# killerwhile/kafka-assignment-optimizer

Measured on AMD Instinct MI355X. Metric: candidate assignments/sec (+ time_to_optimal_s), 10k-partition reassign, higher is better.
Workload: dtype int32

## Files before the change

### include/kao.h

```cpp
#ifndef KAO_H
#define KAO_H

#include <stdint.h>

#ifdef __cplusplus
extern "C" {
#endif

#define KAO_VERSION 103
#define KAO_NONE 0xFFFFu
#define KAO_MAX_RF 8
#define KAO_MAX_RACKS 255

enum {
    KAO_OK = 0,
    KAO_ERR_INVALID = -1,
    KAO_ERR_UNSUPPORTED = -2,
    KAO_ERR_NO_DEVICE = -3,
    KAO_ERR_HIP = -4,
    KAO_ERR_NOMEM = -5,
    KAO_ERR_NOT_INIT = -6
};

enum {
    KAO_STATUS_OPTIMAL_PROVEN = 0,
    KAO_STATUS_FEASIBLE_BOUND_GAP = 1,
    KAO_STATUS_NO_FEASIBLE = 2,
    KAO_STATUS_TIME_LIMIT = 3,
    KAO_STATUS_INFEASIBLE_PROVEN = 4
};

typedef struct kao_topic {
    int32_t n_brokers;
    int32_t n_racks;
    int32_t n_partitions;
    int32_t rf;
    int32_t rf_cur;
    const uint8_t *rack_of;
    const uint16_t *current;
    int32_t w[2][2];
    int32_t rep_lo, rep_hi;
    int32_t lead_lo, lead_hi;
    int32_t rack_lo, rack_hi;
    int32_t prack_lo, prack_hi;
    const int32_t *broker_w;
    const int32_t *broker_wl;
} kao_topic;

typedef struct kao_opts {
    uint64_t seed;
    double time_limit_s;
    int32_t restarts;
    int32_t iters_per_launch;
    int32_t max_launches;
    int32_t obj_scale;
    int32_t lam_min, lam_max;
    int32_t period_log2;
    int32_t stop_at_bound;
    int32_t profile;
    int32_t dual_iters;
    int32_t elite_period;
    int32_t use_prices;
    int32_t use_cycles;
    int32_t islands;
    int32_t schedule;
    int32_t team;
    const int64_t *target_objective;
} kao_opts;

typedef struct kao_result {
    int32_t status;
    int32_t best_restart;
    int64_t objective;
    int64_t upper_bound;
    int32_t violations[8];
    double seconds_to_best;
    uint16_t *assignment;
} kao_result;

typedef struct kao_stats {
    uint64_t launches;
    uint64_t delta_candidates;
    uint64_t full_candidates;
    double ms_search;
    double ms_eval;
    uint64_t search_bytes_algo;
    uint64_t eval_bytes_algo;
    int32_t n_restarts_total;
    int32_t lds_bytes_search;
    int32_t blocks_search;
    int32_t drift;
    int32_t launch_groups;
    int32_t search_rf3_launches;
} kao_stats;

typedef struct kao_session kao_session;
typedef struct kao_eval_plan kao_eval_plan;

int kao_init(int device);
void kao_shutdown(void);
int kao_version(void);
const char *kao_strerror(int code);
const char *kao_last_error(void);
int kao_device_name(char *buf, int len);

int kao_derive_bounds(const kao_topic *t, int32_t out[8]);
int kao_upper_bound(const kao_topic *t, int64_t *ub);
int kao_check_infeasible(const kao_topic *t, char *why, int why_len);
int kao_canonicalize(const kao_topic *t, uint16_t *assignment);

int kao_evaluate(const kao_topic *t, const uint16_t *assignment, int64_t *objective, int32_t violations[8]);
int kao_evaluate_batch(const kao_topic *t, const uint16_t *candidates, int64_t n, int32_t *objective,
                       int32_t *violations);
int kao_eval_plan_create(const kao_topic *t, kao_eval_plan **out);
int kao_eval_plan_run(kao_eval_plan *p, const void *d_candidates, int64_t n, void *d_objective ,
                      void *d_violations , void *d_best_key );
int kao_eval_plan_sync(kao_eval_plan *p, double *ms_last );
void kao_eval_plan_destroy(kao_eval_plan *p);

int kao_session_create(const kao_topic *topics, int32_t n_topics, const kao_opts *opts, kao_session **out);
int kao_session_step(kao_session *s);
int kao_session_sync(kao_session *s);
int kao_session_new_generation(kao_session *s);
int kao_session_best(kao_session *s, kao_result *results);
int kao_session_best_keys(kao_session *s, uint64_t *keys);
int kao_session_device_keys(kao_session *s, void **d_keys);
int kao_session_stats(kao_session *s, kao_stats *out);
int kao_session_small_launches(kao_session *s, int64_t *out);
int kao_session_bound_step(kao_session *s, const int64_t *target, int32_t iters);
int kao_session_set_prices(kao_session *s, int32_t topic, const int32_t *a, const int32_t *l, const int32_t *g);
int kao_session_adopt_prices(kao_session *s);
int kao_session_prices(kao_session *s, int32_t topic, int32_t *a, int32_t *l, int32_t *g);
int kao_session_bound_busy(kao_session *s);
int kao_session_bounds(kao_session *s, int64_t *upper_bound, int32_t *flags, int32_t *iters);
int kao_session_dual_state(kao_session *s, int32_t topic, int32_t *a, int32_t *l, int32_t *g, int64_t *best_dual);
int kao_session_set_dual_state(kao_session *s, int32_t topic, const int32_t *a, const int32_t *l, const int32_t *g);
int kao_lp_bound(const kao_topic *t, double tol, int32_t max_iters, int64_t *bound, int64_t *best_dual, int32_t *multipliers, double stats[8]);
int kao_lp_trace(const kao_topic *t, double tol, int32_t max_iters, double *trace, double stats[8], int32_t *multipliers);
int kao_lp_round(const kao_topic *t, double pert, uint32_t salt, double tol, int32_t max_iters, int32_t use_fallback, uint16_t *assignment,
                 int64_t *objective, int32_t violations[8], double stats[8]);
int kao_lp_round_host(const kao_topic *t, const uint8_t *q, const int32_t *zq, int32_t use_fallback, uint16_t *assignment, int32_t rep[4]);
int kao_dense_spd_test(const double *A, int32_t n, const double *rhs, double *factor, double *linv, double *x, double ms[2]);
int kao_search_band_row(int32_t lo, int32_t hi, int32_t c, int32_t force_plain, int32_t *fits);
int kao_search_rack_delta(int32_t lo, int32_t hi, int32_t c, int32_t dec);
int kao_lp_sharded_test(const kao_topic *t, const int32_t *devices, int32_t n_dev, double pert, uint32_t salt, double tol, int32_t max_iters,
                        int64_t *bound, uint16_t *assignment, int64_t *objective, int32_t violations[8], double stats[8]);
int kao_dual_bound(const kao_topic *t, int64_t target, int32_t iters, int32_t launches, int64_t *bound,
                   int64_t *best_dual, int32_t *iters_done, int32_t *flags, int32_t *multipliers);
int kao_session_restart_state(kao_session *s, int32_t topic, int32_t restart, uint16_t *final_state,
                              uint16_t *best_state, int32_t info[4]);
void kao_session_destroy(kao_session *s);

int kao_solve(const kao_topic *topics, int32_t n_topics, const kao_opts *opts, kao_result *results);
int kao_solve_multi(const kao_topic *topics, int32_t n_topics, const int32_t *devices, int32_t n_dev, const kao_opts *opts,
                    kao_result *results);
int kao_solve_capped(const kao_topic *topics, int32_t n_topics, const int32_t *replica_cap, const int32_t *devices, int32_t n_dev,
                     const kao_opts *opts, int32_t max_rounds, kao_result *results, int64_t *lagrangian_bound);
int kao_improve_cycles(const kao_topic *t, uint16_t *assignment, int32_t max_rounds, int64_t *objective, int32_t stats[8]);
int kao_cycle_matrices(const kao_topic *t, const uint16_t *assignment, int32_t layer, int32_t level, int32_t *dist, int32_t *mid,
                       uint32_t *slot);
int kao_cycle_square_plan(int32_t n, int32_t out[3]);
int kao_cycle_seeds(const kao_topic *t, const uint16_t *assignment, int32_t *table, int32_t *n_cfg);
int kao_cycle_pair_edges(const kao_topic *t, const uint16_t *assignment, int32_t gmin, int32_t *cost, int64_t stats[4]);

int kao_plan_waves(int32_t n_brokers, int32_t n_partitions, int32_t width, const uint16_t *current, const uint16_t *target,
                   int32_t max_per_broker, uint64_t seed, int32_t *wave , int32_t *n_waves, int32_t *lower_bound);

int kao_plan_waves_sized(int32_t n_brokers, int32_t n_partitions, int32_t width, const uint16_t *current, const uint16_t *target,
                         const uint64_t *size , uint64_t max_bytes_per_broker, int32_t max_per_broker,
                         uint64_t seed, int32_t *wave , int32_t *n_waves, int32_t *lower_bound);

int kao_balance_leaders(const kao_topic *t, uint16_t *assignment , int32_t *n_changed,
                        int64_t *objective ,
                        int32_t *status, int32_t stats[8] );

#define KAO_FAILOVER_MAX_BROKERS 8000
int kao_failover_order(int32_t n_brokers, int32_t n_racks, const uint8_t *rack_of ,
                       int32_t n_partitions, int32_t width, uint16_t *rows ,
                       int32_t scope , int32_t dry_run,
                       int32_t *scen , int32_t *n_reordered, int32_t stats[8] );

int kao_balance_leaders_cluster(int32_t n_brokers, int32_t n_partitions, int32_t width,
                                uint16_t *rows ,
                                const int32_t *topic_of , int32_t n_topics,
                                const int32_t *topic_lo, const int32_t *topic_hi ,
                                int32_t cluster_lo, int32_t cluster_hi , int32_t dry_run,
                                int32_t *n_changed, int32_t *peak_before, int32_t *peak_after, int32_t *status,
                                int32_t stats[8] );

int kao_balance_leaders_weighted(int32_t n_brokers, int32_t n_partitions, int32_t width,
                                 uint16_t *rows , const uint64_t *weight ,
                                 uint64_t min_gain, int32_t max_rounds , int32_t dry_run,
                                 int32_t *n_changed, uint64_t *peak_before, uint64_t *peak_after, uint64_t *lower_bound,
                                 int32_t *status, int64_t stats[8] );
int kao_wleaders_test_path(int32_t path);

int kao_failover_order_weighted(int32_t n_brokers, int32_t n_racks, const uint8_t *rack_of, int32_t n_partitions, int32_t width,
                                uint16_t *rows , const uint64_t *weight ,
                                int32_t scope, uint64_t min_gain, int32_t max_rounds , int32_t dry_run,
                                uint64_t *scen , int32_t *n_reordered, int32_t *status,
                                int64_t stats[8] );

#define KAO_DISK_MAX_BROKERS 8000
int kao_balance_disk(int32_t n_brokers, int32_t n_racks, const uint8_t *rack_of, int32_t n_partitions, int32_t width,
                     uint16_t *rows , const uint64_t *size ,
                     int32_t max_per_rack , int32_t move_leaders, uint64_t min_gain,
                     int32_t max_rounds , int32_t dry_run, int32_t *n_moved, uint64_t *bytes_moved,
                     uint64_t *peak_before, uint64_t *peak_after, uint64_t *lower_bound, int32_t *status,
                     int64_t stats[8] );

int kao_balance_disk_budget(int32_t n_brokers, int32_t n_racks, const uint8_t *rack_of, int32_t n_partitions, int32_t width,
                            uint16_t *rows , const uint64_t *size ,
                            int32_t max_per_rack , int32_t move_leaders, uint64_t min_gain,
                            uint64_t max_bytes , int32_t max_rounds , int32_t dry_run,
                            int32_t *n_moved, uint64_t *bytes_moved, uint64_t *peak_before, uint64_t *peak_after,
                            uint64_t *lower_bound, int32_t *status, int64_t stats[10] );

#define KAO_LOGDIRS_MAX_DIRS 64
int kao_balance_logdirs(int32_t n_brokers, const int32_t *dir_start , const uint64_t *base ,
                        int32_t n_replicas, int32_t *dir , const uint64_t *size ,
                        uint64_t min_gain, int32_t max_rounds , int32_t dry_run,
                        int32_t *n_moved, uint64_t *bytes_moved, uint64_t *peak_before, uint64_t *peak_after,
                        uint64_t *per_broker , int32_t *status, int64_t stats[8] );

int kao_rccl_selftest(const int32_t *devices, int32_t n_dev);
int kao_rccl_loopback_counts(uint64_t out[2]);
int kao_last_solve_timing(double out[16]);
int kao_last_solve_lp(double out[8]);
int kao_last_solve_profile(double out[8]);

#ifdef __cplusplus
}
#endif
#endif
```

### kafka_assignment_optimizer_amd/__init__.py

```python
from .model import DEFAULT_WEIGHTS, NONE, Topic, assignment_to_json, topics_from_json
from .solver import (EvalPlan, KaoError, Result, Session, canonicalize, check_infeasible, derive_bounds, device_name, dual_bound, evaluate,
                     cycle_matrices, cycle_pair_edges, cycle_seeds, cycle_square_plan, dense_spd_test, evaluate_batch, improve_cycles, init, last_solve_lp, last_solve_profile, last_solve_timing, library_path, lp_bound, lp_repair_host, lp_round, lp_round_host, lp_sharded, lp_trace, rccl_loopback_counts, rccl_selftest, solve, solve_capped, solve_multi, upper_bound)

__version__ = "0.1.0"
```

### kafka_assignment_optimizer_amd/_ffi.py

```python
from __future__ import annotations

import ctypes as C
import os

_HERE = os.path.dirname(os.path.abspath(__file__))
LIB_PATH = os.path.join(_HERE, "libkao.so")


class KaoTopic(C.Structure):
    _fields_ = [("n_brokers", C.c_int32), ("n_racks", C.c_int32), ("n_partitions", C.c_int32),
                ("rf", C.c_int32), ("rf_cur", C.c_int32),
                ("rack_of", C.POINTER(C.c_uint8)), ("current", C.POINTER(C.c_uint16)),
                ("w", (C.c_int32 * 2) * 2),
                ("rep_lo", C.c_int32), ("rep_hi", C.c_int32), ("lead_lo", C.c_int32), ("lead_hi", C.c_int32),
                ("rack_lo", C.c_int32), ("rack_hi", C.c_int32), ("prack_lo", C.c_int32), ("prack_hi", C.c_int32),
                ("broker_w", C.POINTER(C.c_int32)), ("broker_wl", C.POINTER(C.c_int32))]


class KaoOpts(C.Structure):
    _fields_ = [("seed", C.c_uint64), ("time_limit_s", C.c_double), ("restarts", C.c_int32),
                ("iters_per_launch", C.c_int32), ("max_launches", C.c_int32), ("obj_scale", C.c_int32),
                ("lam_min", C.c_int32), ("lam_max", C.c_int32), ("period_log2", C.c_int32),
                ("stop_at_bound", C.c_int32), ("profile", C.c_int32), ("dual_iters", C.c_int32),
                ("elite_period", C.c_int32), ("use_prices", C.c_int32), ("use_cycles", C.c_int32), ("islands", C.c_int32),
                ("schedule", C.c_int32), ("team", C.c_int32),
                ("target_objective", C.POINTER(C.c_int64))]


class KaoResult(C.Structure):
    _fields_ = [("status", C.c_int32), ("best_restart", C.c_int32), ("objective", C.c_int64),
                ("upper_bound", C.c_int64), ("violations", C.c_int32 * 8), ("seconds_to_best", C.c_double),
                ("assignment", C.POINTER(C.c_uint16))]


class KaoStats(C.Structure):
    _fields_ = [("launches", C.c_uint64), ("delta_candidates", C.c_uint64), ("full_candidates", C.c_uint64),
                ("ms_search", C.c_double), ("ms_eval", C.c_double), ("search_bytes_algo", C.c_uint64),
                ("eval_bytes_algo", C.c_uint64), ("n_restarts_total", C.c_int32), ("lds_bytes_search", C.c_int32),
                ("blocks_search", C.c_int32), ("drift", C.c_int32), ("launch_groups", C.c_int32),
                ("search_rf3_launches", C.c_int32)]


_P = C.POINTER
SIGNATURES = {
    "kao_init": (C.c_int, [C.c_int]),
    "kao_shutdown": (None, []),
    "kao_version": (C.c_int, []),
    "kao_strerror": (C.c_char_p, [C.c_int]),
    "kao_last_error": (C.c_char_p, []),
    "kao_device_name": (C.c_int, [C.c_char_p, C.c_int]),
    "kao_derive_bounds": (C.c_int, [_P(KaoTopic), _P(C.c_int32)]),
    "kao_upper_bound": (C.c_int, [_P(KaoTopic), _P(C.c_int64)]),
    "kao_canonicalize": (C.c_int, [_P(KaoTopic), _P(C.c_uint16)]),
    "kao_check_infeasible": (C.c_int, [_P(KaoTopic), C.c_char_p, C.c_int]),
    "kao_evaluate": (C.c_int, [_P(KaoTopic), _P(C.c_uint16), _P(C.c_int64), _P(C.c_int32)]),
    "kao_evaluate_batch": (C.c_int, [_P(KaoTopic), _P(C.c_uint16), C.c_int64, _P(C.c_int32), _P(C.c_int32)]),
    "kao_eval_plan_create": (C.c_int, [_P(KaoTopic), _P(C.c_void_p)]),
    "kao_eval_plan_run": (C.c_int, [C.c_void_p, C.c_void_p, C.c_int64, C.c_void_p, C.c_void_p, C.c_void_p]),
    "kao_eval_plan_sync": (C.c_int, [C.c_void_p, _P(C.c_double)]),
    "kao_eval_plan_destroy": (None, [C.c_void_p]),
    "kao_session_create": (C.c_int, [_P(KaoTopic), C.c_int32, _P(KaoOpts), _P(C.c_void_p)]),
    "kao_session_step": (C.c_int, [C.c_void_p]),
    "kao_session_sync": (C.c_int, [C.c_void_p]),
    "kao_session_new_generation": (C.c_int, [C.c_void_p]),
    "kao_session_best": (C.c_int, [C.c_void_p, _P(KaoResult)]),
    "kao_session_best_keys": (C.c_int, [C.c_void_p, _P(C.c_uint64)]),
    "kao_session_device_keys": (C.c_int, [C.c_void_p, _P(C.c_void_p)]),
    "kao_session_stats": (C.c_int, [C.c_void_p, _P(KaoStats)]),
    "kao_session_small_launches": (C.c_int, [C.c_void_p, _P(C.c_int64)]),
    "kao_session_restart_state": (C.c_int, [C.c_void_p, C.c_int32, C.c_int32, _P(C.c_uint16), _P(C.c_uint16),
                                            _P(C.c_int32)]),
    "kao_session_bound_step": (C.c_int, [C.c_void_p, _P(C.c_int64), C.c_int32]),
    "kao_session_set_prices": (C.c_int, [C.c_void_p, C.c_int32, _P(C.c_int32), _P(C.c_int32), _P(C.c_int32)]),
    "kao_session_adopt_prices": (C.c_int, [C.c_void_p]),
    "kao_session_prices": (C.c_int, [C.c_void_p, C.c_int32, _P(C.c_int32), _P(C.c_int32), _P(C.c_int32)]),
    "kao_session_bound_busy": (C.c_int, [C.c_void_p]),
    "kao_session_bounds": (C.c_int, [C.c_void_p, _P(C.c_int64), _P(C.c_int32), _P(C.c_int32)]),
    "kao_session_dual_state": (C.c_int, [C.c_void_p, C.c_int32, _P(C.c_int32), _P(C.c_int32), _P(C.c_int32), _P(C.c_int64)]),
    "kao_session_set_dual_state": (C.c_int, [C.c_void_p, C.c_int32, _P(C.c_int32), _P(C.c_int32), _P(C.c_int32)]),
    "kao_lp_bound": (C.c_int, [_P(KaoTopic), C.c_double, C.c_int32, _P(C.c_int64), _P(C.c_int64), _P(C.c_int32), _P(C.c_double)]),
    "kao_lp_round": (C.c_int, [_P(KaoTopic), C.c_double, C.c_uint32, C.c_double, C.c_int32, C.c_int32, _P(C.c_uint16), _P(C.c_int64), _P(C.c_int32), _P(C.c_double)]),
    "kao_lp_round_host": (C.c_int, [_P(KaoTopic), _P(C.c_uint8), _P(C.c_int32), C.c_int32, _P(C.c_uint16), _P(C.c_int32)]),
    "kao_dense_spd_test": (C.c_int, [_P(C.c_double), C.c_int32, _P(C.c_double), _P(C.c_double), _P(C.c_double), _P(C.c_double), _P(C.c_double)]),
    "kao_search_band_row": (C.c_int, [C.c_int32, C.c_int32, C.c_int32, C.c_int32, _P(C.c_int32)]),
    "kao_search_rack_delta": (C.c_int, [C.c_int32, C.c_int32, C.c_int32, C.c_int32]),
    "kao_lp_sharded_test": (C.c_int, [_P(KaoTopic), _P(C.c_int32), C.c_int32, C.c_double, C.c_uint32, C.c_double, C.c_int32, _P(C.c_int64), _P(C.c_uint16),
                                      _P(C.c_int64), _P(C.c_int32), _P(C.c_double)]),
    "kao_lp_trace": (C.c_int, [_P(KaoTopic), C.c_double, C.c_int32, _P(C.c_double), _P(C.c_double), _P(C.c_int32)]),
    "kao_dual_bound": (C.c_int, [_P(KaoTopic), C.c_int64, C.c_int32, C.c_int32, _P(C.c_int64), _P(C.c_int64), _P(C.c_int32),
                                 _P(C.c_int32), _P(C.c_int32)]),
    "kao_session_destroy": (None, [C.c_void_p]),
    "kao_solve": (C.c_int, [_P(KaoTopic), C.c_int32, _P(KaoOpts), _P(KaoResult)]),
    "kao_solve_multi": (C.c_int, [_P(KaoTopic), C.c_int32, _P(C.c_int32), C.c_int32, _P(KaoOpts), _P(KaoResult)]),
    "kao_solve_capped": (C.c_int, [_P(KaoTopic), C.c_int32, _P(C.c_int32), _P(C.c_int32), C.c_int32, _P(KaoOpts), C.c_int32,
                                  _P(KaoResult), _P(C.c_int64)]),
    "kao_rccl_selftest": (C.c_int, [_P(C.c_int32), C.c_int32]),
    "kao_rccl_loopback_counts": (C.c_int, [_P(C.c_uint64)]),
    "kao_improve_cycles": (C.c_int, [_P(KaoTopic), _P(C.c_uint16), C.c_int32, _P(C.c_int64), _P(C.c_int32)]),
    "kao_cycle_matrices": (C.c_int, [_P(KaoTopic), _P(C.c_uint16), C.c_int32, C.c_int32, _P(C.c_int32), _P(C.c_int32), _P(C.c_uint32)]),
    "kao_cycle_square_plan": (C.c_int, [C.c_int32, _P(C.c_int32)]),
    "kao_cycle_seeds": (C.c_int, [_P(KaoTopic), _P(C.c_uint16), _P(C.c_int32), _P(C.c_int32)]),
    "kao_cycle_pair_edges": (C.c_int, [_P(KaoTopic), _P(C.c_uint16), C.c_int32, _P(C.c_int32), _P(C.c_int64)]),
    "kao_plan_waves": (C.c_int, [C.c_int32, C.c_int32, C.c_int32, _P(C.c_uint16), _P(C.c_uint16), C.c_int32, C.c_uint64,
                                 _P(C.c_int32), _P(C.c_int32), _P(C.c_int32)]),
    "kao_plan_waves_sized": (C.c_int, [C.c_int32, C.c_int32, C.c_int32, _P(C.c_uint16), _P(C.c_uint16), _P(C.c_uint64), C.c_uint64,
                                       C.c_int32, C.c_uint64, _P(C.c_int32), _P(C.c_int32), _P(C.c_int32)]),
    "kao_balance_leaders": (C.c_int, [_P(KaoTopic), _P(C.c_uint16), _P(C.c_int32), _P(C.c_int64), _P(C.c_int32), _P(C.c_int32)]),
    "kao_failover_order": (C.c_int, [C.c_int32, C.c_int32, _P(C.c_uint8), C.c_int32, C.c_int32, _P(C.c_uint16), C.c_int32, C.c_int32,
                                     _P(C.c_int32), _P(C.c_int32), _P(C.c_int32)]),
    "kao_balance_leaders_cluster": (C.c_int, [C.c_int32, C.c_int32, C.c_int32, _P(C.c_uint16), _P(C.c_int32), C.c_int32, _P(C.c_int32),
                                              _P(C.c_int32), C.c_int32, C.c_int32, C.c_int32, _P(C.c_int32), _P(C.c_int32), _P(C.c_int32),
                                              _P(C.c_int32), _P(C.c_int32)]),
    "kao_balance_leaders_weighted": (C.c_int, [C.c_int32, C.c_int32, C.c_int32, _P(C.c_uint16), _P(C.c_uint64), C.c_uint64, C.c_int32, C.c_int32,
                                               _P(C.c_int32), _P(C.c_uint64), _P(C.c_uint64), _P(C.c_uint64), _P(C.c_int32), _P(C.c_int64)]),
    "kao_wleaders_test_path": (C.c_int, [C.c_int32]),
    "kao_failover_order_weighted": (C.c_int, [C.c_int32, C.c_int32, _P(C.c_uint8), C.c_int32, C.c_int32, _P(C.c_uint16), _P(C.c_uint64), C.c_int32,
                                              C.c_uint64, C.c_int32, C.c_int32, _P(C.c_uint64), _P(C.c_int32), _P(C.c_int32), _P(C.c_int64)]),
    "kao_balance_disk": (C.c_int, [C.c_int32, C.c_int32, _P(C.c_uint8), C.c_int32, C.c_int32, _P(C.c_uint16), _P(C.c_uint64), C.c_int32, C.c_int32,
                                   C.c_uint64, C.c_int32, C.c_int32, _P(C.c_int32), _P(C.c_uint64), _P(C.c_uint64), _P(C.c_uint64), _P(C.c_uint64),
                                   _P(C.c_int32), _P(C.c_int64)]),
    "kao_balance_disk_budget": (C.c_int, [C.c_int32, C.c_int32, _P(C.c_uint8), C.c_int32, C.c_int32, _P(C.c_uint16), _P(C.c_uint64), C.c_int32,
                                          C.c_int32, C.c_uint64, C.c_uint64, C.c_int32, C.c_int32, _P(C.c_int32), _P(C.c_uint64), _P(C.c_uint64),
                                          _P(C.c_uint64), _P(C.c_uint64), _P(C.c_int32), _P(C.c_int64)]),
    "kao_balance_logdirs": (C.c_int, [C.c_int32, _P(C.c_int32), _P(C.c_uint64), C.c_int32, _P(C.c_int32), _P(C.c_uint64), C.c_uint64, C.c_int32, C.c_int32,
                                      _P(C.c_int32), _P(C.c_uint64), _P(C.c_uint64), _P(C.c_uint64), _P(C.c_uint64), _P(C.c_int32), _P(C.c_int64)]),
    "kao_last_solve_timing":(C.c_int, [_P(C.c_double)]),
    "kao_last_solve_profile": (C.c_int, [_P(C.c_double)]),
    "kao_last_solve_lp": (C.c_int, [_P(C.c_double)]),
}

_lib = None


def load():
    global _lib
    if _lib is None:
        if not os.path.exists(LIB_PATH):
            raise OSError(f"{LIB_PATH} not built: the HIP library is required (no CPU fallback); "
                          "run `make -C kafka_assignment_optimizer_amd/csrc`")
        lib = C.CDLL(LIB_PATH)
        for name, (res, args) in SIGNATURES.items():
            fn = getattr(lib, name)
            fn.restype = res
            fn.argtypes = args
        _lib = lib
    return _lib
```

### kafka_assignment_optimizer_amd/csrc/kao_host.h

```cpp
#pragma once
#include <hip/hip_runtime.h>

#include <algorithm>
#include <cstdint>
#include <cstdlib>
#include <memory>
#include <string>
#include <vector>

#include "../../include/kao.h"
#include "kao_internal.h"

namespace kao {

int fail(int code, const std::string &msg);
#define HIP_TRY(expr)                                                                          \
    do {                                                                                       \
        hipError_t e_ = (expr);                                                                \
        if (e_ != hipSuccess)                                                                  \
            return ::kao::fail(KAO_ERR_HIP, std::string(#expr) + ": " + hipGetErrorString(e_)); \
    } while (0)
double now_s();
int cur_device();
constexpr int kMaxDevices = 64;
int num_cu(int device);
int require_init();
bool is_init();
extern thread_local int t_device;
struct DeviceScope {
    const int saved = t_device;
    int rc = KAO_OK;
    DeviceScope() = default;
    explicit DeviceScope(int device) { to(device); }
    DeviceScope(const DeviceScope &) = delete;
    DeviceScope &operator=(const DeviceScope &) = delete;
    int to(int device);
    ~DeviceScope();
};
struct SolveTiming {
    double session_ready, time_to_best, results_read_back, returned, launches, delta_candidates, bound_launches, elite_exchanges,
           bound_iters, cx_calls, cx_gains, search_iters, generations, cx_further_starts, lp_solves, lp_iters;
};
struct SolveLp { double solves, iterations, rounded, adopted, fractional_partitions; };
struct SolveProfile {
    double ms_search, ms_eval, search_launches, restarts, search_bytes_algo, delta_candidates, lds_bytes_search, blocks_search;
};
struct SolveCounters { SolveTiming timing; SolveLp lp; SolveProfile profile; };
extern thread_local SolveCounters g_last;
inline const char *env_str(const char *name) { const char *e = std::getenv(name); return e && *e ? e : nullptr; }
inline int64_t env_int(const char *name, int64_t dflt) { const char *e = env_str(name); return e ? (int64_t)std::atoll(e) : dflt; }
inline double env_real(const char *name, double dflt) { const char *e = env_str(name); return e ? std::atof(e) : dflt; }
int arena_get(size_t bytes, void **out, size_t *cap);
void arena_put(void *p, size_t bytes, int device);
int stream_get(hipStream_t *out);
void stream_put(hipStream_t st, int device);
void arena_drop_all();
inline size_t align_up(size_t x, size_t a = 256) { return (x + a - 1) / a * a; }
inline uint32_t replica_word(uint16_t x, int m) { return x == KAO_NONE ? kNoneW : ((uint32_t)x | ((uint32_t)(x / m) << 16)); }

struct CallBufs {
    void *arena = nullptr;
    size_t cap = 0;
    hipStream_t stream = nullptr;
    CallBufs() = default;
    CallBufs(const CallBufs &) = delete;
    CallBufs &operator=(const CallBufs &) = delete;
    int open(size_t bytes);
    template <class T> T *at(size_t off) const { return reinterpret_cast<T *>(static_cast<unsigned char *>(arena) + off); }
    ~CallBufs();
};
struct Carve {
    size_t next = 0;
    template <class T> size_t take(size_t count) { const size_t o = next; next += align_up(count * sizeof(T)); return o; }
    size_t end() const { return next; }
};
inline unsigned grid_for(int64_t n, int threads) { return (unsigned)((std::max<int64_t>(n, 1) + threads - 1) / threads); }
int check_dims(const std::string &fn, int32_t B, int32_t P, int32_t W, int32_t R = 1);
int check_slot_cap(const std::string &fn, int32_t P, int32_t W);
int check_row(const std::string &fn, int32_t B, int32_t W, int64_t p, const uint16_t *row);
int check_rows(const std::string &fn, int32_t B, int32_t P, int32_t W, const uint16_t *rows);
int check_weight_sum(const std::string &fn, int32_t P, const uint64_t *weight);
constexpr int kSettleBatch = 8;
template <class Launch>
int settle_rounds(const char *fn, hipStream_t st, int N, int32_t *d_flags, int32_t &rounds, int32_t &launches, Launch launch) {
    int32_t flags[kSettleBatch];
    for (int r = 0, settled = 0; !settled;) {
        if (r > N + kSettleBatch) return fail(KAO_ERR_HIP, std::string(fn) + "relaxation did not settle");
        if (r) { HIP_TRY(hipMemsetAsync(d_flags, 0, sizeof flags, st)); }
        for (int i = 0; i < kSettleBatch; ++i, ++r) launch(r, d_flags + i);
        launches += kSettleBatch;
        HIP_TRY(hipGetLastError());
        HIP_TRY(hipMemcpyAsync(flags, d_flags, sizeof flags, hipMemcpyDeviceToHost, st));
        HIP_TRY(hipStreamSynchronize(st));
        for (int i = 0; i < kSettleBatch && !settled; ++i) {
            ++rounds;
            settled = flags[i] == 0;
        }
    }
    return KAO_OK;
}

int validate(const kao_topic *t);
void derive_bounds(const kao_topic *t, int32_t o[8]);
struct PreparedTopic {
    TopicDev d{};
    std::vector<uint16_t> int_of;
    std::vector<uint16_t> ext_of;
    std::vector<int32_t> rack_size;
    std::vector<uint16_t> cur_int;
    std::vector<uint8_t> rack_of;
    std::vector<uint16_t> cur_dense;
    std::vector<uint32_t> bw_int, bw_dense;
};
int prepare(const kao_topic *t, uint64_t seed, PreparedTopic &pt);
std::string infeasible_reason(const kao_topic *t);
int64_t upper_bound(const kao_topic *t);
int64_t upper_bound_w(const kao_topic *t);
uint64_t neighbours_in_range(uint32_t it0, uint32_t iters, int rf, int n_brokers, int n_partitions, int scan2_max = kScanTwoSlots);
int auto_period_log2(int P, int RF);
bool dual_supported(const kao_topic *t, bool session_bw = false);

}

using namespace kao;

struct kao_eval_plan {
    PreparedTopic pt;
    TopicDev *d_topic = nullptr;
    uint8_t *d_rackof = nullptr;
    uint16_t *d_curd = nullptr;
    int4 *d_map = nullptr;
    uint32_t *d_bwd = nullptr;
    int32_t *d_overflow = nullptr;
    int64_t map_n = -1;
    int map_blocks = 0;
    hipStream_t stream = nullptr;
    hipEvent_t ev0 = nullptr, ev1 = nullptr;
    bool timed = false;
    int cands_per_block = 32;
    bool cur_in_lds = true;
    bool coop = false;
    int device = 0;
};

struct kao_session {
    int device = 0;
    int n_topics = 0;
    kao_opts opts{};
    std::vector<PreparedTopic> pts;
    std::vector<kao_topic> topics;
    std::vector<int64_t> ub;
    std::vector<char> topic_global;
    std::vector<char> topic_curg;
    std::vector<char> topic_infeasible;
    std::vector<char> dual_ok;
    std::vector<int64_t> h_dual_target;
    std::vector<int32_t> h_dual_ids;
    bool multi_off = false;
    std::vector<int2> h_wide_map;
    uint64_t wide_ctl_i32 = 0, wide_map_i32 = 0;
    std::vector<int32_t> dual_flags, dual_iters;
    int total_restarts = 0;
    struct LaunchGroup {
        int maxP = 0, maxBx = 0, maxB = 0, maxR = 0;
        bool wide = false;
        int waves = kWaves;
        int nw = kRFP;
        int rf_uniform = -1;
        int w_abs_max = 0;
        bool band_tabs = true;
        bool rf3 = true;
        bool global_a = false;
        bool cur_global = false;
        int team = 0;
        bool cur_in_lds = true;
        bool eval_coop = false;
        int smap_off = 0, smap_n = 0, emap_off = 0, emap_n = 0;
    };
    std::vector<LaunchGroup> groups;
    int blocks_search = 0, blocks_eval = 0;
    void *arena_ro = nullptr, *arena_rw = nullptr;
    size_t arena_ro_bytes = 0, arena_rw_bytes = 0;
    TopicDev *d_topics = nullptr;
    int2 *d_smap = nullptr;
    int4 *d_emap = nullptr;
    uint32_t *d_cur = nullptr;
    uint16_t *d_ext = nullptr;
    int32_t *d_rsz = nullptr;
    uint8_t *d_rackof = nullptr;
    uint16_t *d_curd = nullptr;
    unsigned char *d_state = nullptr;
    uint16_t *d_best = nullptr;
    int32_t *d_info = nullptr;
    int32_t *d_obj = nullptr;
    int32_t *d_viol = nullptr;
    unsigned char *d_readback = nullptr;
    size_t readback_bytes = 0, rb_viol_off = 0, rb_assign_off = 0;
    int32_t *d_dual = nullptr;
    int32_t *d_price = nullptr;
    size_t price_half_i32 = 0;
    int price_read = 0;
    int price_write_last = -1;
    bool priced = false;
    bool any_bw = false;
    uint16_t *d_int = nullptr;
    uint32_t *d_bw = nullptr, *d_bwd = nullptr;
    long long *d_dual_target = nullptr;
    int32_t *d_dual_ids = nullptr;
    unsigned char *d_dual_rb = nullptr;
    size_t dual_rb_bytes = 0;
    uint64_t bound_launches = 0;
    bool dual_state_init = false;
    size_t dual_bytes = 0;
    hipStream_t stream_bound = nullptr;
    hipEvent_t ev_bound0 = nullptr, ev_bound1 = nullptr, ev_search = nullptr;
    bool bound_inflight = false;
    bool bound_no_wait = false;
    int bound_iters_last = 0;
    double bound_ms_last = 0;
    unsigned long long *d_keys = nullptr;
    unsigned long long *d_keys_glob = nullptr;
    int32_t *d_drift = nullptr;
    int32_t *d_win_viol = nullptr;
    uint16_t *d_win_assign = nullptr;
    std::vector<unsigned char> h_readback;
    hipStream_t stream = nullptr;
    uint32_t launch = 0;
    uint32_t gen = 0;
    bool reinit = false;
    size_t best_bytes = 0;
    std::vector<hipEvent_t> ev;
    int ev_pending = 0;
    double ms_search = 0, ms_eval = 0;
    uint64_t eval_bytes_per_launch = 0;
    uint64_t delta_total = 0, search_bytes_total = 0;
    uint64_t search_rf3_launches = 0;
    uint64_t search_small_launches = 0;
    bool small_on = true;
};

namespace kao {
constexpr int64_t kDualNone = 0x7F7F7F7F7F7F7F7Fll;
inline int64_t dual_floor(int64_t best_dual) { return best_dual >= 0 ? best_dual / kDualScale : -((-best_dual + kDualScale - 1) / kDualScale); }
inline int64_t dual_bound_value(int32_t flags, int32_t iters, int64_t best_dual) { return (flags & 4) || iters == 0 ? INT64_MAX : dual_floor(best_dual); }
struct SessionDeleter { void operator()(kao_session *s) const { kao_session_destroy(s); } };
using SessionPtr = std::unique_ptr<kao_session, SessionDeleter>;
int bound_only_session(const kao_topic *t, SessionPtr &out);
int session_topic_best(kao_session *s, int i, uint16_t *out);
int session_restart_objs(kao_session *s, int i, std::vector<int32_t> &objs);
int session_restart_best(kao_session *s, int i, int restart, uint16_t *out);
int session_adopt_external(kao_session *s, int i, const uint16_t *assign, int64_t objective, uint64_t *key_out);
}
```

### kafka_assignment_optimizer_amd/csrc/kao_internal.h

```cpp
#pragma once
#include <stdint.h>

#include <unordered_map>

#include "../../include/kao.h"

namespace kao {

constexpr int kRFP = 4;
constexpr int kMaxRF = 8;
constexpr int kWaves = 4;
constexpr int kTeamMax = 8;
constexpr int kMaxRacks = 255;
constexpr int kLdsLimit = 160 * 1024;
constexpr int kRackTab = 256;
constexpr uint32_t kNoneW = 0xFFFFFFFFu;
constexpr uint32_t kKeyNull = 0xFFFFFFFFu;
constexpr int kDBias = 32768;
constexpr int kDualLog2 = 16;
constexpr int kDualScale = 1 << kDualLog2;
constexpr int kDualStage = 100;
constexpr int kDualDeflP = 2048;
constexpr int kScanTwoSlots = 24576;
constexpr int kDualClamp = 1 << 26;
constexpr int kDualQuarterLog2 = kDualLog2 - 2;
constexpr int kDualProbes = 2;
constexpr uint32_t kExternalRestart = 0xFFFFFu;
constexpr uint32_t kObjCap = 0xFFFFFFu;

struct TopicDev {
    int32_t P, RF, R, m, Bx;
    uint32_t magic;
    int32_t rep_lo, rep_hi, lead_lo, lead_hi, rack_lo, rack_hi, prack_lo, prack_hi;
    int32_t w00, w01, w10, w11;
    uint32_t seed_lo, seed_hi;
    int32_t n_restarts;
    int32_t restart_base;
    uint32_t cur_off;
    uint32_t ext_off;
    uint32_t rsz_off;
    uint64_t state_off;
    uint64_t best_off;
    int32_t B, rf_cur;
    uint32_t rackof_off;
    uint32_t curd_off;
    uint32_t win_off;
    uint32_t dual_off;
    int32_t period_log2;
    uint32_t price_off;
    uint32_t int_off;
    int32_t nw;
    int32_t has_bw;
    uint32_t bw_off;
    uint32_t bwd_off;
    uint32_t cnt_off;
    uint32_t hole_off;
    int32_t pad_[1];
};

struct SearchParams {
    int32_t obj_scale, lam_min, lam_max;
    int32_t maxR;
    int32_t wide;
    uint32_t launch;
    uint32_t iters;
    int32_t init;
    int32_t maxP, maxBx;
    int32_t bw;
    uint32_t gen;
    int32_t scan2_max;
    int32_t cur_global;
    int32_t elite;
};

struct SearchPools {
    const TopicDev *topics;
    const int2 *block_map;
    const uint32_t *cur_pool;
    const uint16_t *ext_pool;
    const int32_t *rsz_pool;
    unsigned char *state_pool;
    uint16_t *best_pool;
    int32_t *restart_info;
    int32_t *drift;
    const int32_t *price_pool;
    const uint32_t *bw_pool;
    const uint16_t *int_pool;
    const uint16_t *elite_assign;
    const unsigned long long *elite_key;
};

struct EvalPools {
    const TopicDev *topics;
    const int4 *block_map;
    const uint8_t *rackof_pool;
    const uint16_t *curd_pool;
    const uint16_t *cand;
    int32_t *objective;
    int32_t *violations;
    unsigned long long *best_key;
    int32_t maxP, maxB;
    int32_t cur_in_lds;
    int32_t coop;
    const uint32_t *bwd_pool;
    int32_t *overflow;
    int32_t rf_uniform;
};

struct BoundPools {
    const TopicDev *topics;
    const int32_t *ids;
    const uint8_t *rackof_pool;
    const uint16_t *curd_pool;
    const uint16_t *ext_pool;
    const int32_t *rsz_pool;
    int32_t *dual_pool;
    const long long *target;
    long long *best_L;
    int32_t *info;
    int32_t iters;
    int32_t maxB, maxP, maxR;
    int32_t cur_in_lds;
    int32_t *price_pool;
    int32_t export_prices;
    int32_t ne;
    const uint32_t *bwd_pool;
};

struct BoundWide {
    const int2 *map;
    int32_t *cnt_pool;
    long long *ctl;
    int32_t chunk;
};

constexpr int search_rack_tab(int maxR) { return ((maxR < 1 ? 1 : maxR) + 1 + 63) & ~63; }
size_t search_lds_bytes(int maxP, int maxBx, int waves, bool global_a, bool priced = false, int nw = 4, bool bw = false, int maxR = kRackTab - 1, int team = 0, bool cur_global = false);
size_t eval_lds_bytes(int maxP, int maxB, bool cur_in_lds, int ne = 4);
bool search_rf3_eligible(bool global_a, bool cur_global, bool priced, int nw, int team);
constexpr int kSmallCostMax = 16384;
bool search_small_cost(int lam_min, int lam_max, int obj_scale, int w_abs_max, bool priced);
bool search_band_tabs(int rep_lo, int rep_hi, int lead_lo, int lead_hi);
void launch_search(const SearchPools &pools, const SearchParams &prm, int n_blocks, int waves, bool global_a, bool priced, int nw, void *stream, int team = 0, int rft = 0, bool small = false);
bool launch_init(const SearchPools &pools, const SearchParams &prm, int n_blocks, int per_block, bool priced, int nw, int waves, void *stream);
void launch_eval(const EvalPools &pools, int n_blocks, int ne, void *stream);
void launch_gather(const TopicDev *topics, int n_topics, const unsigned long long *keys, const uint16_t *best_pool,
                   const int32_t *viol, uint16_t *win_assign, int32_t *win_viol, void *stream);

void launch_adopt_global(unsigned long long *keys, const unsigned long long *glob, int n, void *stream);

size_t bound_lds_bytes(int maxB, int maxP, int maxR, bool cur_in_lds, int ne = 4, bool hbw = false, bool dirs = false);
void launch_bound_center(const BoundPools &pools, int n_topics, void *stream);
void launch_bound(const BoundPools &pools, int n_blocks, int waves, void *stream);
void launch_bound_wide(const BoundPools &pools, const BoundWide &wide, int n_topics, int n_blocks, int waves, void *stream);
bool launch_bound_multi(const BoundPools &pools, const BoundWide &wide, int n_topics, int n_blocks, int waves, void *stream);

size_t canon_lds_bytes(int maxBx);
void launch_canon(const TopicDev *topic, const uint32_t *cur_words, const uint16_t *ext, const int32_t *rsz, uint32_t *A, int maxBx,
                  int nw, int32_t *status, void *stream);


struct LpCtx;
struct LpColl {
    virtual int allreduce(int rank, double *buf, size_t n, bool is_min, void *stream) = 0;
    virtual ~LpColl() {}
};
struct LpShard { int p0, p1, rank; LpColl *coll; };
struct LpFan {
    virtual int begin(double tol, int maxit, double pert, uint32_t salt) = 0;
    virtual int enqueue_mark(int k, int slot) = 0;
    virtual int poll_mark(int slot, int *status, int *iterations, double deadline) = 0;
    virtual int finish(int32_t *multipliers, double stats[8], double *trace) = 0;
    virtual int primal(uint8_t *q, int32_t *zq) = 0;
    virtual void abort() = 0;
    virtual void close() = 0;
    virtual ~LpFan() {}
};
extern thread_local bool t_lp_inner;
void lp_set_fan(LpCtx *c, LpFan *fan);
int lp_open_fan(const kao_topic *t, const int *devices, int n_dev, LpCtx **out);
int lp_open(const kao_topic *t, LpCtx **out, const LpShard *shard = nullptr);
int lp_solve(LpCtx *c, double tol, int maxit, int32_t *multipliers, double stats[8], double *trace, double pert = 0.0, uint32_t salt = 0);
int lp_begin(LpCtx *c, double tol, int maxit, double pert = 0.0, uint32_t salt = 0);
int lp_enqueue(LpCtx *c, int k);
int lp_poll(LpCtx *c, int *status, int *iterations);
int lp_enqueue_mark(LpCtx *c, int k, int slot);
int lp_poll_mark(LpCtx *c, int slot, int *status, int *iterations, double deadline = 0);
int lp_finish(LpCtx *c, int32_t *multipliers, double stats[8], double *trace);
inline double lp_default_pert(const kao_topic *t) { const double e = 100.0 / ((double)t->n_partitions * t->rf); return e < 1e-2 ? e : 1e-2; }
int lp_primal(LpCtx *c, uint8_t *q, int32_t *zq);
int lp_round_assignment(const kao_topic *t, const uint8_t *q, const int32_t *zq, const uint16_t *fallback, uint16_t *out, int32_t rep[4], int max_free = 1 << 30);
void lp_abort(LpCtx *c);
void lp_close(LpCtx *c);
void chol_enqueue(void *stream, const double *stop, double *S, int n, const double *diag0, double *Linv);
void trsv_enqueue(void *stream, double *stop, const double *gate, const double *S, int n, double *r, const double *Linv, double *xz);

bool cycle_supported(const kao_topic *t);
int cycle_improve(const kao_topic *t, uint16_t *assign, int32_t max_rounds, double deadline, int64_t *objective, int32_t stats[8]);
struct CycleCtx;
CycleCtx *cycle_open(const kao_topic *t, int *rc_out);
int cycle_run(CycleCtx *c, uint16_t *assign, int32_t max_rounds, double deadline, int64_t *objective, int32_t stats[8],
              int (*poll)(void *) = nullptr, void *poll_arg = nullptr, bool pairs = true);
void cycle_close(CycleCtx *c);
struct PairEdge { int32_t cost; int32_t set; int32_t p, q; uint16_t rowp[8], rowq[8]; };
int pair_edges(const kao_topic *t, const uint16_t *assignment, int gmin, std::unordered_map<uint32_t, PairEdge> &edges, int64_t stats[4]);
int api_fail(int code, const char *msg);
int api_require_init();
double api_now_s();

}
```

### kafka_assignment_optimizer_amd/csrc/kao_search.hip

```cpp
#include "kao_search_dev.h"

namespace kao {

template <bool kGlobalA, bool kPriced, int NW, bool kWide, bool kTeam, bool kCurG = false, int RFT = 0, bool kSmall = false>
__device__ __forceinline__ void search_body(unsigned char *smem, const SearchPools &pl, const SearchParams &prm) {
    static_assert(!kTeam || kGlobalA, "teams run topics that live in global memory");
    static_assert(!kCurG || !kGlobalA, "kCurG: the working assignment is in LDS");
    static_assert(RFT == 0 || (RFT == 3 && NW == 4 && !kGlobalA && !kTeam), "RFT = 3: LDS-resident topics of four words per partition");
    static_assert(!kSmall || (RFT == 3 && !kPriced && !kCurG), "kSmall: the unpriced RF-3 instantiation");
    constexpr int NS = RFT ? RFT : NW;
    const int lane = threadIdx.x & 63;
    const int wave = __builtin_amdgcn_readfirstlane(threadIdx.x >> 6);
    const int n_waves = kTeam ? __builtin_amdgcn_readfirstlane((int)(blockDim.x >> 6)) : 1;
    const int tid = kTeam ? (int)threadIdx.x : lane, nthr = kTeam ? (int)blockDim.x : 64;
    const int2 bm = pl.block_map[blockIdx.x];
    const TopicDev *TD = pl.topics + bm.x;

    TopicRegs T = topic_regs<RFT>(TD);
    {
        uint32_t v0 = T.c7_inc, v1 = T.c7_dec;
        asm volatile("" : "+v"(v0), "+v"(v1));
        T.c7_inc = (uint32_t)__builtin_amdgcn_readfirstlane((int)v0); T.c7_dec = (uint32_t)__builtin_amdgcn_readfirstlane((int)v1);
    }
    constexpr bool kBandTabs = kSmall;
    int bq_r0 = kBandTabs ? band_tab_bias(T.rep_lo) : T.rep_lo, bq_r1 = kBandTabs ? (int)band_tab(T.rep_lo, T.rep_hi) : T.rep_hi;
    int bq_l0 = kBandTabs ? band_tab_bias(T.lead_lo) : T.lead_lo, bq_l1 = kBandTabs ? (int)band_tab(T.lead_lo, T.lead_hi) : T.lead_hi;
    asm volatile("" : "+v"(bq_r0), "+v"(bq_r1), "+v"(bq_l0), "+v"(bq_l1));

    const int a_bytes = kGlobalA ? 0 : prm.maxP * NW * 4;
    const int cur_bytes = (kGlobalA || kCurG) ? 0 : prm.maxP * NW * 4;
    const int bx64 = (prm.maxBx + 63) & ~63;
    const int c_bytes = bx64 * 4;
    const int krt = search_rack_tab(prm.maxR);
    int *RSZ = reinterpret_cast<int *>(smem + cur_bytes);
    uint8_t *XR = smem + cur_bytes + krt * 4;
    const uint32_t inv = (uint32_t)krt - 1u;
    uint32_t *PR = reinterpret_cast<uint32_t *>(smem + cur_bytes + krt * 4 + bx64);
    const bool hbw = kPriced && prm.bw != 0;
    const int pr_bytes = kPriced ? (hbw ? 2 : 1) * c_bytes + krt * 4 : 0;
    int *PG = reinterpret_cast<int *>(smem + cur_bytes + krt * 4 + bx64 + c_bytes);
    uint32_t *BW = reinterpret_cast<uint32_t *>(smem + cur_bytes + krt * 4 + bx64 + c_bytes + krt * 4);
    unsigned char *wb = smem + cur_bytes + krt * 4 + bx64 + pr_bytes + (kTeam ? 0 : wave * (a_bytes + c_bytes + c_bytes / 2 + krt * 8));
    const Part<NW> *cur_words = reinterpret_cast<const Part<NW> *>(pl.cur_pool + TD->cur_off);
    const Part<NW> *CUR;
    if (kGlobalA || kCurG) CUR = cur_words; else CUR = reinterpret_cast<const Part<NW> *>(smem);
    WaveLds<NW> L;
    L.C = reinterpret_cast<uint32_t *>(wb + a_bytes);
    L.W = reinterpret_cast<uint16_t *>(wb + a_bytes + c_bytes);
    L.K = reinterpret_cast<int *>(wb + a_bytes + c_bytes + c_bytes / 2);
    L.RT = L.K + krt + (kTeam ? wave * krt : 0);
    int *TR = L.K + krt + n_waves * krt;
    int *TS = TR + 2 * 16 * kTeamRec;

    if (!kGlobalA && !kCurG) {
        Part<NW> *cur_lds = reinterpret_cast<Part<NW> *>(smem);
        for (int p = threadIdx.x; p < T.P; p += blockDim.x) cur_lds[p] = cur_words[p];
    }
    for (int r = threadIdx.x; r < krt; r += blockDim.x) {
        RSZ[r] = r < T.R ? pl.rsz_pool[TD->rsz_off + r] : 0;
        if (kPriced) PG[r] = r < T.R ? price_units(pl.price_pool[TD->price_off + 2 * TD->B + r], prm.obj_scale) : 0;
    }
    __syncthreads();
    for (int x = threadIdx.x; x < ((T.Bx + 63) & ~63); x += blockDim.x) {
        const uint32_t r = mulhi((uint32_t)x, T.magic);
        const bool valid = x < T.Bx && (int)((uint32_t)x - r * (uint32_t)T.m) < RSZ[r < (uint32_t)krt ? r : 0];
        XR[x] = valid ? (uint8_t)r : (uint8_t)inv;
        if (kPriced) {
            uint32_t pr = 0;
            if (valid) {
                const int32_t *pp = pl.price_pool + TD->price_off;
                const int b = pl.ext_pool[TD->ext_off + x];
                pr = ((uint32_t)price_units(pp[b], prm.obj_scale) & 0xFFFFu) | ((uint32_t)price_units(pp[TD->B + b], prm.obj_scale) << 16);
            }
            PR[x] = pr;
            if (hbw) BW[x] = (valid && TD->has_bw) ? pl.bw_pool[TD->bw_off + x] : 0u;
        }
    }
    __syncthreads();

    const int rho = bm.y + (kTeam ? 0 : wave);
    if (rho >= TD->n_restarts) return;
    const int g = TD->restart_base + rho;
    unsigned char *state_packed = pl.state_pool + TD->state_off + (uint64_t)rho * T.P * (NW * 2);
    if (kGlobalA) L.A = reinterpret_cast<Part<NW> *>(pl.state_pool + TD->state_off) + (uint64_t)rho * T.P;
    else L.A = reinterpret_cast<Part<NW> *>(wb);
    uint16_t *best = pl.best_pool + TD->best_off + (uint64_t)rho * T.P * T.RF;
    const uint16_t *ext = pl.ext_pool + TD->ext_off;
    const uint32_t slo = TD->seed_lo, shi = TD->seed_hi;
    const int S = prm.obj_scale;

    int best_obj, accepted;
    if (prm.init) {
        if (prm.init == 1)
        for (int p = tid; p < T.P; p += nthr) {
            Part<NW> c = CUR[p];
#pragma unroll
            for (int k = 1; k < NW; ++k)
                if (k >= T.RF) c.w[k] = kNoneW;
            L.A[p] = c;
        }
        best_obj = -1; accepted = 0;
    } else {
        best_obj = pl.restart_info[g * 4 + 0];
        accepted = pl.restart_info[g * 4 + 3];
        bool reseed = false;
        if (prm.elite) {
            const unsigned long long ek = pl.elite_key[bm.x];
            const int e_obj = (int)kObjCap - (int)((ek >> 20) & 0xFFFFFFull);
            reseed = ek != ~0ull && (ek >> 44) == 0 && (int)(ek & 0xFFFFFull) != rho && best_obj < e_obj &&
                     (fmix32(slo ^ ((uint32_t)rho * 0x9E3779B1u) ^ (prm.launch * 0x85EBCA77u) ^ 0xE117Eu) & 1u);
        }
        if (reseed) {
            const uint16_t *ea = pl.elite_assign + TD->win_off;
            const uint16_t *io = pl.int_pool + TD->int_off;
            for (int p = tid; p < T.P; p += nthr) {
                Part<NW> w;
#pragma unroll
                for (int k = 0; k < NW; ++k) w.w[k] = k < T.RF ? to_word(T, io[ea[p * T.RF + k]]) : kNoneW;
                L.A[p] = w;
            }
        } else if (!kGlobalA) {
            for (int p = lane; p < T.P; p += 64) L.A[p] = load_packed<NW>(T, state_packed, p);
        }
    }
    if (kGlobalA) __builtin_amdgcn_fence(__ATOMIC_SEQ_CST, "workgroup");
    if (kTeam) __syncthreads();
    recount(T, L, tid, nthr, krt);
    if (kTeam) __syncthreads();

    rebuild_band_state(T, L, XR, inv, tid, nthr);
    if (lane == 0) L.RT[krt - 1] = 0;
    if (kTeam) __syncthreads();

    if (prm.init == 1) {
        constexpr bool kFillWeights = RFT != 3;
        const uint32_t *HL = pl.cur_pool + TD->hole_off;
        const FillTabs F{L.W, XR, L.K, L.RT, PR, PG, hbw ? BW : nullptr};
        if (!kTeam || wave == 0)
        for (int pass = 0; pass < 2; ++pass) {
            const uint32_t n_holes = HL[pass], *hl = HL + 2 + (pass ? HL[0] : 0u);
            int p_n = n_holes ? (int)hl[0] : 0;
            Part<NW> a_n = L.A[p_n], c_n = CUR[p_n];
            for (uint32_t hi = 0; hi < n_holes; ++hi) {
                const int p = p_n;
                Part<NW> a = a_n;
                const Part<NW> c = c_n;
                if (hi + 1 < n_holes) { p_n = (int)hl[hi + 1]; a_n = L.A[p_n]; c_n = CUR[p_n]; }
                fill_mark<NS>(L.W, a, lane);
#pragma nounroll
                for (int k = pass; k < (pass ? T.RF : 1); ++k) {
                    if ((uint32_t)__builtin_amdgcn_readfirstlane((int)sel_slot<NS>(a, k)) != kNoneW) continue;
                    const uint32_t hmix = slo ^ fmix32(shi + (uint32_t)rho * 0x9E3779B1u + (uint32_t)(p * NW + k) * 0x27D4EB2Fu + 0x5BD1E995u + prm.gen * 0x632BE5ABu);
                    const uint32_t xw_win = fill_hole<NS, kPriced, !kSmall, kFillWeights>(T, F, a, c, k == 0, hmix, prm.lam_max, S, lane);
                    if (xw_win == kNoneW) continue;
                    set_slot(a, k, xw_win);
                    if (lane == 0) {
                        const uint32_t xs = xw_win & 0xFFFFu;
                        reinterpret_cast<uint32_t *>(&L.A[p])[k] = xw_win;
                        const uint32_t cx = L.C[xs] + ((k == 0) ? 0x10001u : 1u);
                        L.C[xs] = cx;
                        L.K[xw_win >> 16] += 1;
                        uint32_t wx = band_row<kBandTabs>((int)(cx & 0xFFFFu), bq_r0, bq_r1);
                        if (k == 0) wx |= band_row<kBandTabs>((int)(cx >> 16), bq_l0, bq_l1) << 6;
                        else wx |= L.W[xs] & kWRowL;
                        L.W[xs] = (uint16_t)(wx | kWNoCand);
                    }
                }
                fill_unmark<NS>(L.W, a, lane);
            }
        }
        if (kGlobalA) __builtin_amdgcn_fence(__ATOMIC_SEQ_CST, "workgroup");
        if (kTeam) __syncthreads();
    }

    int V, obj;
    full_cost<NW, kTeam>(T, L, CUR, RSZ, tid, nthr, V, obj, hbw ? BW : nullptr, TS, wave, n_waves);
    if (V == 0 && obj > best_obj) { best_obj = obj; snapshot(T, L, ext, best, tid, nthr); }
    if (kTeam) __syncthreads();

    uint32_t rng = fmix32(slo ^ fmix32(shi + (uint32_t)rho * 0x9E3779B1u + prm.launch * 0x85EBCA77u + (uint32_t)tid * 0xC2B2AE3Du));

    const int plog = TD->period_log2 + (rho & 3);
    const uint32_t pmask = (1u << plog) - 1u;
    const uint32_t lrange = (uint32_t)(prm.lam_max - prm.lam_min + 1);
    const uint32_t RF8 = (uint32_t)T.RF << 8, R8 = (uint32_t)T.R << 8, m8 = (uint32_t)T.m << 8;

    const int T_tour = min(64, max(4, (T.P * T.RF) >> 2));
    uint32_t tour_off = lane < T_tour ? 0u : kKeyNull;
    asm volatile("" : "+v"(tour_off));
    const int GA = min(16, max(1, (T.P * T.RF) >> 8));
    const int x_rounds_full = (T.P + 63) >> 6;
    const bool x_windowed = x_rounds_full > 8;

    int lam_lo = prm.lam_min, lam_hi = prm.lam_max;
    uint32_t n_iters = prm.iters, it_base = prm.launch * prm.iters;
    constexpr uint32_t kLpScanTwo = 1u << 29;
    uint32_t loop_pack = TD->P * TD->RF <= prm.scan2_max ? kLpScanTwo : 0u;
    if (kSmall) loop_pack |= ((uint32_t)prm.lam_min & 0xFFFu) | (((uint32_t)prm.lam_max & 0xFFFu) << 12) | (((uint32_t)plog & 31u) << 24);
    {
        uint32_t v0 = (uint32_t)lam_lo, v1 = (uint32_t)lam_hi, v2 = n_iters, v3 = it_base, v4 = loop_pack;
        asm volatile("" : "+v"(v2), "+v"(v3), "+v"(v4));
        if constexpr (!kSmall) {
            asm volatile("" : "+v"(v0), "+v"(v1));
            lam_lo = (int)__builtin_amdgcn_readfirstlane(v0); lam_hi = (int)__builtin_amdgcn_readfirstlane(v1);
        }
        n_iters = __builtin_amdgcn_readfirstlane(v2); it_base = __builtin_amdgcn_readfirstlane(v3);
        loop_pack = __builtin_amdgcn_readfirstlane(v4);
    }
    auto loop_flag = [&](uint32_t bit) { uint32_t lp = loop_pack; asm volatile("" : "+s"(lp)); return (lp & bit) != 0u; };
    constexpr bool kFuse = !kGlobalA && !kTeam && !kPriced;
    const bool fuse_ok = kFuse && T.Bx <= 16384;
    uint32_t jmp_a = 1u, jmp_c = 0u;
    if (fuse_ok)
        for (int n = (T.Bx + 63) >> 6; n > 0; --n) { jmp_a = (jmp_a * 0x6D2B79u) & 0xFFFFFFu; jmp_c = (jmp_c * 0x6D2B79u + 0x3C6EF3u) & 0xFFFFFFu; }
    best_obj = __builtin_amdgcn_readfirstlane(best_obj);
    for (uint32_t i = 0; i < n_iters; ++i) {
        const uint32_t it = it_base + i;
        const int type = (int)((0x1210u >> ((it & 7u) * 2u)) & 3u);
        int lam;
        if constexpr (kSmall) {
            uint32_t lp = loop_pack;
            asm volatile("" : "+s"(lp));
            const uint32_t plg = (lp >> 24) & 31u;
            const int lo_ = (int)(lp & 0xFFFu), hi_ = (int)((lp >> 12) & 0xFFFu);
            const uint32_t ph = it & ((1u << plg) - 1u);
            lam = best_obj < 0 ? hi_ : min(hi_, lo_ + (int)((2u * ph * (uint32_t)(hi_ - lo_ + 1)) >> plg));
        } else {
            const uint32_t ph = it & pmask;
            lam = best_obj < 0 ? lam_hi : min(lam_hi, lam_lo + (int)((2u * ph * lrange) >> plog));
        }
        const bool sampled = (type == 2) || (type == 0 && ((it >> 3) & 1u));

        auto finish = [&](auto ty, auto uni, uint32_t kmin, int win, int p, int k, int q, int j, uint32_t uw, uint32_t vw, int dV, int dObj) {
            constexpr int TY = decltype(ty)::value;
            auto of_win = [&](int v) { return decltype(uni)::value ? v : __builtin_amdgcn_readlane(v, win); };
            if (!kTeam) {
                if (kmin == kKeyNull) return;
                if ((int)(kmin >> 8) - kDBias > 0) return;
            }
            bool mine = true;
            int *rec = TR + ((i & 1u) * 16 + (uint32_t)wave) * kTeamRec;
            if (kTeam) {
                const bool ok = kmin != kKeyNull && (int)(kmin >> 8) - kDBias <= 0;
                if (lane == win) {
                    const uint32_t ro_ = uw >> 16, rn_ = vw >> 16;
                    const bool racks = ok && TY == 0 && ro_ != rn_;
                    rec[0] = ok ? 1 : 0; rec[1] = p; rec[2] = TY == 1 ? q : p;
                    rec[3] = (int)(uw & 0xFFFFu); rec[4] = (int)(vw & 0xFFFFu);
                    rec[5] = racks ? (int)ro_ : 0xFFFF; rec[6] = racks ? (int)rn_ : 0xFFFF;
                    rec[7] = dV; rec[8] = dObj;
                }
                __syncthreads();
                bool clash = false;
                if (lane < wave) {
                    const int *o = TR + ((i & 1u) * 16 + (uint32_t)lane) * kTeamRec;
                    if (o[0]) {
                        const int mp = rec[1], mq = rec[2], mb0 = rec[3], mb1 = rec[4], mr0 = rec[5], mr1 = rec[6];
                        clash = (o[1] == mp) | (o[1] == mq) | (o[2] == mp) | (o[2] == mq) | (o[3] == mb0) | (o[3] == mb1) | (o[4] == mb0) | (o[4] == mb1);
                        if (o[5] != 0xFFFF && mr0 != 0xFFFF) clash |= (o[5] == mr0) | (o[5] == mr1) | (o[6] == mr0) | (o[6] == mr1);
                    }
                }
                mine = ok && __ballot(clash) == 0ull;
            }

            constexpr bool kOneTrip = !kTeam && kSmall;
            if constexpr (kOneTrip) {
                if (lane == win) {
                    uint32_t *ap = reinterpret_cast<uint32_t *>(&L.A[p]);
                    if (TY == 0) ap[k] = vw;
                    else if (TY == 1) { ap[k] = vw; reinterpret_cast<uint32_t *>(&L.A[q])[j] = uw; }
                    else { ap[0] = vw; ap[k] = uw; }
                }
                const int kw = of_win(k);
                int rows;
                if (TY == 0) rows = 1 | (kw == 0 ? 2 : 0);
                else if (TY == 1) rows = (kw == 0 ? 2 : 0) ^ (of_win(j) == 0 ? 2 : 0);
                else rows = 2;
                if (rows != 0) {
                    const uint32_t uws = (uint32_t)of_win((int)uw);
                    const uint32_t vws = decltype(uni)::value ? (uint32_t)__builtin_amdgcn_readfirstlane((int)vw) : (uint32_t)of_win((int)vw);
                    const uint32_t xo = uws & 0xFFFFu, xn = vws & 0xFFFFu;
                    uint32_t xx = xo;
                    asm("v_writelane_b32 %0, %1, 1" : "+v"(xx) : "s"(xn));
                    uint32_t xi = xx;
                    const uint32_t d0 = TY == 0 ? (kw == 0 ? 0x10001u : 1u) : (TY == 1 ? (kw == 0 ? 0x10000u : 0u - 0x10000u) : 0x10000u);
                    int n_own = 2;
                    if (TY == 0) {
                        const uint32_t ro_ = uws >> 16, rn_ = vws >> 16;
                        asm("v_writelane_b32 %0, %1, 2\n\tv_writelane_b32 %0, %2, 3" : "+v"(xi) : "s"(ro_), "s"(rn_));
                        n_own = ro_ != rn_ ? 4 : 2;
                    }
                    int lane_w = lane;
                    asm volatile("" : "+v"(lane_w));
                    if (lane_w < n_own) {
                        uint32_t *cp = (lane_w < 2 ? L.C : reinterpret_cast<uint32_t *>(L.K)) + xi;
                        const uint32_t c_old = *cp;
                        const uint32_t w_old = L.W[xx];
                        const uint32_t dl = lane_w < 2 ? d0 : 1u;
                        const uint32_t cx = (lane_w & 1) ? c_old + dl : c_old - dl;
                        *cp = cx;
                        if (lane_w < 2) {
                            uint32_t wx;
                            if (rows == 3) wx = band_row<kBandTabs>((int)(cx & 0xFFFFu), bq_r0, bq_r1) | (band_row<kBandTabs>((int)(cx >> 16), bq_l0, bq_l1) << 6);
                            else if (rows == 1) wx = (w_old & ~kWRowR) | band_row<kBandTabs>((int)(cx & 0xFFFFu), bq_r0, bq_r1);
                            else wx = (w_old & ~kWRowL) | (band_row<kBandTabs>((int)(cx >> 16), bq_l0, bq_l1) << 6);
                            L.W[xx] = (uint16_t)wx;
                        }
                    }
                }
            } else {
            if (lane == win && mine) {
                uint32_t *ap = reinterpret_cast<uint32_t *>(&L.A[p]);
                if (TY == 0) {
                    const uint32_t d = (k == 0) ? 0x10001u : 1u;
                    L.C[uw & 0xFFFFu] -= d;
                    L.C[vw & 0xFFFFu] += d;
                    if (!kTeam || (uw >> 16) != (vw >> 16)) {
                        L.K[uw >> 16] -= 1;
                        L.K[vw >> 16] += 1;
                    }
                    ap[k] = vw;
                } else if (TY == 1) {
                    uint32_t *bp = reinterpret_cast<uint32_t *>(&L.A[q]);
                    if ((k == 0) != (j == 0)) {
                        const uint32_t lose = (k == 0) ? uw : vw, gain = (k == 0) ? vw : uw;
                        L.C[lose & 0xFFFFu] -= 0x10000u;
                        L.C[gain & 0xFFFFu] += 0x10000u;
                    }
                    ap[k] = vw;
                    bp[j] = uw;
                } else {
                    L.C[uw & 0xFFFFu] -= 0x10000u;
                    L.C[vw & 0xFFFFu] += 0x10000u;
                    ap[0] = vw;
                    ap[k] = uw;
                }
            }
            if (mine) {
                int rows;
                if (TY == 0) rows = 1 | (of_win(k) == 0 ? 2 : 0);
                else if (TY == 1) rows = (of_win(k) == 0 ? 2 : 0) ^ (of_win(j) == 0 ? 2 : 0);
                else rows = 2;
                if (rows != 0) {
                    const uint32_t xo = (uint32_t)of_win((int)uw) & 0xFFFFu, xn = decltype(uni)::value ? (uint32_t)__builtin_amdgcn_readfirstlane((int)(vw & 0xFFFFu)) : (uint32_t)of_win((int)vw) & 0xFFFFu;
                    uint32_t xx = xo;
                    asm("v_writelane_b32 %0, %1, 1" : "+v"(xx) : "s"(xn));
                    int lane_w = lane;
                    asm volatile("" : "+v"(lane_w));
                    if (lane_w < 2) {
                        const uint32_t cx = L.C[xx];
                        uint32_t wx;
                        if (rows == 3) wx = band_row<kBandTabs>((int)(cx & 0xFFFFu), bq_r0, bq_r1) | (band_row<kBandTabs>((int)(cx >> 16), bq_l0, bq_l1) << 6);
                        else if (rows == 1) wx = (L.W[xx] & ~kWRowR) | band_row<kBandTabs>((int)(cx & 0xFFFFu), bq_r0, bq_r1);
                        else wx = (L.W[xx] & ~kWRowL) | (band_row<kBandTabs>((int)(cx >> 16), bq_l0, bq_l1) << 6);
                        L.W[xx] = (uint16_t)wx;
                    }
                }
            }
            }
            if (kGlobalA) __builtin_amdgcn_fence(__ATOMIC_SEQ_CST, "workgroup");
            if (kTeam) {
                if (lane == 0) rec[9] = mine ? 1 : 0;
                __syncthreads();
                int dVs = 0, dOs = 0, na = 0;
                if (lane < n_waves) {
                    const int *o = TR + ((i & 1u) * 16 + (uint32_t)lane) * kTeamRec;
                    if (o[9]) { dVs = o[7]; dOs = o[8]; na = 1; }
                }
                V += wave_sum(dVs);
                obj += wave_sum(dOs);
                accepted += wave_sum(na);
            } else {
                V += of_win(dV);
                obj += of_win(dObj);
                accepted++;
            }
        };
        constexpr std::integral_constant<int, 0> kReplace{};
        constexpr std::integral_constant<int, 1> kExchange{};
        constexpr std::integral_constant<int, 2> kLeaderSwap{};

        if (sampled) {
            const int p = (int)rnd24_wide(rng, (uint32_t)T.P);
            const Part<NW> a = L.A[p];
            const Part<NW> c = CUR[p];
            uint32_t key = kKeyNull, vw = 0;
            int dV = 0, dObj = 0;
            if (type == 0) {
                const int k = (int)rnd24(rng, RF8);
                const uint32_t uw = sel_slot<NS>(a, k);
                const uint32_t ro = uw >> 16;
                const bool lead = k == 0;
                const uint32_t lw = lead ? 2u : 0u;
                const int wl = lead ? T.w00 : T.w01, wf = lead ? T.w10 : T.w11;
                const int g_old = role_w2<NS>(c, uw, wl, wf) + (hbw ? bw_of(BW[uw & 0xFFFFu], lead) : 0);
                const uint32_t wo = L.W[uw & 0xFFFFu];
                const int dV_old = wfld(wo, kWDecR) + wfldw(wo, kWDecL, lw);
                const int dV_rack_old = ddec(L.K[ro], T.rack_lo, T.rack_hi) + c7_delta(T.c7_dec, cnt4x2<NS>(a, ro));
                const int rsz_ro = RSZ[ro];
                int dP_old = 0, dP_rack_old = 0;
                if (kPriced) {
                    const uint32_t pro = PR[uw & 0xFFFFu];
                    dP_old = -(wflag(wo, kWPoutR) & price_rep(pro));
                    if (lead) dP_old -= wflag(wo, kWPoutL) & price_lead(pro);
                    dP_rack_old = p_out(L.K[ro], T.rack_lo, T.rack_hi, PG[ro]);
                }
                const int base_s = kSmall ? mad24s(S, g_old, kDBias) : 0;
#pragma unroll
                for (int g = 0; g < 4; ++g) {
                    uint32_t r, jj;
                    bool okg;
                    if (g < 2) {
                        r = rnd24(rng, R8);
                        jj = rnd24(rng, m8);
                        okg = (int)jj < RSZ[r];
                    } else {
                        r = ro;
                        jj = rnd24(rng, (uint32_t)rsz_ro << 8);
                        okg = true;
                    }
                    const uint32_t x = __umul24(r, (uint32_t)T.m) + jj;
                    const uint32_t xw = x | (r << 16);
                    okg = okg && !in4<NS>(a, xw);
                    const uint32_t wn = L.W[x];
                    int dVg = dV_old + wfld(wn, kWIncR) + wfldw(wn, kWIncL, lw);
                    if (g < 2) {
                        if (r != ro)
                            dVg += dV_rack_old + dinc(L.K[r], T.rack_lo, T.rack_hi) + c7_delta(T.c7_inc, cnt4x2<NS>(a, r));
                    }
                    const int dObjg = role_w2<NS>(c, xw, wl, wf) + (hbw ? bw_of(BW[x], lead) : 0) - (kSmall ? 0 : g_old);
                    uint32_t keyg;
                    if constexpr (kSmall) keyg = okg ? key_small(mad24s(-S, dObjg, mad24s(lam, dVg, base_s)), (uint32_t)lane) : kKeyNull;
                    else if (kPriced) {
                        const uint32_t prx = PR[x];
                        int dPg = dP_old + (wflag(wn, kWPinR) & price_rep(prx));
                        if (lead) dPg += wflag(wn, kWPinL) & price_lead(prx);
                        if (g < 2 && r != ro) dPg += dP_rack_old + p_in(L.K[r], T.rack_lo, T.rack_hi, PG[r]);
                        keyg = okg ? make_key_p(lam, S, dVg, dObjg, dPg, lane) : kKeyNull;
                    }
                    else keyg = okg ? make_key(lam, S, dVg, dObjg, lane) : kKeyNull;
                    if (keyg < key) { key = keyg; vw = xw; dV = dVg; dObj = dObjg; }
                }
                if constexpr (kSmall) dObj -= g_old;
                const uint32_t kmin = wave_umin(key);
                finish(kReplace, std::false_type{}, kmin, (int)(kmin & 63u), p, k, 0, 0, uw, vw, dV, dObj);
            } else {
                const uint32_t uw = a.w[0];
                int k = 0;
                const int u_lead = role_w2<NS>(c, uw, T.w00, T.w10), u_fol = role_w2<NS>(c, uw, T.w01, T.w11);
                const uint32_t wu = L.W[uw & 0xFFFFu];
                const int dV_u = wfld(wu, kWDecL);
                const int dP_u = kPriced ? -(wflag(wu, kWPoutL) & price_lead(PR[uw & 0xFFFFu])) : 0;
#pragma unroll
                for (int kk = 1; kk < NS; ++kk) {
                    if (!RFT && kk >= T.RF) break;
                    const uint32_t xw = a.w[kk];
                    const int dObjg = role_w2<NS>(c, xw, T.w00, T.w10) + u_fol - u_lead - role_w2<NS>(c, xw, T.w01, T.w11) +
                                      (hbw ? (int)(BW[xw & 0xFFFFu] >> 16) - (int)(BW[uw & 0xFFFFu] >> 16) : 0);
                    const uint32_t wx = L.W[xw & 0xFFFFu];
                    const int dVg = dV_u + wfld(wx, kWIncL);
                    uint32_t keyg;
                    if constexpr (kSmall) keyg = key_small(mad24s(lam, dVg, mad24s(-S, dObjg, kDBias)), (uint32_t)lane);
                    else if (kPriced) keyg = make_key_p(lam, S, dVg, dObjg, dP_u + (wflag(wx, kWPinL) & price_lead(PR[xw & 0xFFFFu])), lane);
                    else keyg = make_key(lam, S, dVg, dObjg, lane);
                    if (keyg < key) { key = keyg; vw = xw; k = kk; dV = dVg; dObj = dObjg; }
                }
                const uint32_t kmin = wave_umin(key);
                finish(kLeaderSwap, std::false_type{}, kmin, (int)(kmin & 63u), p, k, 0, 0, uw, vw, dV, dObj);
            }
        } else {
            uint32_t keyA, oldw_l;
            int pl_, kl_, g_old_l, dvo_l = 0, dvr_l = 0;
            auto score_words = [&](auto ty, uint32_t &key_o, const Part<NW> &al, const Part<NW> &cl, int k_o, uint32_t &oldw_o, int &g_o, int &dvo_o, int &dvr_o) {
                constexpr int TY = decltype(ty)::value;
                oldw_o = sel_slot<NS>(al, k_o);
                const uint32_t rol = oldw_o >> 16;
                const bool leadl = k_o == 0;
                g_o = role_w2<NS>(cl, oldw_o, leadl ? T.w00 : T.w01, leadl ? T.w10 : T.w11);
                if (hbw && TY == 0) g_o += bw_of(BW[oldw_o & 0xFFFFu], leadl);
                const uint32_t wo = L.W[oldw_o & 0xFFFFu];
                const int dv7 = c7_delta(T.c7_dec, cnt4x2<NS>(al, rol));
                int sc;
                if (TY == 0) {
                    dvo_o = wfld(wo, kWDecR) + wfldw(wo, kWDecL, leadl ? 2u : 0u);
                    dvr_o = ddec(L.K[rol], T.rack_lo, T.rack_hi) + dv7;
                    sc = dvo_o + min(dvr_o, 0);
                } else {
                    const int dvl = wfld(wo, leadl ? kWDecL : kWIncL);
                    sc = min(dv7, 0) + min(dvl, 0);
                }
                if constexpr (kSmall) key_o = key_small(mad24s(lam, sc, mad24s(S, g_o, kDBias)), (uint32_t)lane) | tour_off;
                else if (kPriced) {
                    int dPs = 0;
                    if (TY == 0) {
                        const uint32_t pro = PR[oldw_o & 0xFFFFu];
                        dPs = -(wflag(wo, kWPoutR) & price_rep(pro));
                        dPs -= wflagw(wo, kWPoutL, leadl ? 1u : 0u) & price_lead(pro);
                    }
// ... 174 lines not shown
                const int n_rd = (T.Bx + 63) >> 6;
                int rd = 0, base = 0;
                while (rd < n_rd) {
                    int nxt = n_rd;
#pragma unroll
                    for (int i2 = 0; i2 < 2 * NW; ++i2)
                        if (mr[i2] >= rd) nxt = min(nxt, mr[i2]);
                    uint32_t k1a, k2a, k1b, k2b;
                    for (; rd + 1 < nxt; rd += 2, base += 128) {
                        const int wa = Ws[base + lane], wb = Ws[base + 64 + lane];
                        const uint32_t ra = XR[base + lane], rb = XR[base + 64 + lane];
                        const int rta = L.RT[ra], rtb = L.RT[rb];
                        scan_round2(std::false_type{}, base, rd, wa, rta, k1a, k2a);
                        scan_round2(std::false_type{}, base + 64, rd + 1, wb, rtb, k1b, k2b);
                        best1 = min(best1, min(k1a, k1b));
                        best2 = min(best2, min(k2a, k2b));
                    }
                    if (rd < nxt) { const int wa = Ws[base + lane]; scan_round2(std::false_type{}, base, rd, wa, L.RT[XR[base + lane]], k1a, k2a); best1 = min(best1, k1a); best2 = min(best2, k2a); ++rd; base += 64; }
                    if (rd < n_rd) { const int wa = Ws[base + lane]; scan_round2(std::true_type{}, base, rd, wa, L.RT[XR[base + lane]], k1a, k2a); best1 = min(best1, k1a); best2 = min(best2, k2a); ++rd; base += 64; }
                }
                asm("v_mad_u32_u24 %0, %0, %1, %2" : "+v"(rng) : "s"(jmp_a), "v"(jc));
                if (holds) L.W[ai & 0xFFFFu] = (uint16_t)w_keep;
                const uint32_t kw = wave_umin(min(((best1 >> 1) & ~127u) | (uint32_t)lane, ((best2 >> 1) & ~127u) | 64u | (uint32_t)lane));
                const bool two = (kw & 64u) != 0u;
                const uint32_t kmin = kw >> 7;
                const int win = (int)(kw & 63u);
                const int p = two ? ps[1] : ps[0], k = two ? ks[1] : ks[0];
                const uint32_t uw = two ? us[1] : us[0];
                if ((int)(kmin >> 8) - kDBias <= 0) {
                    const bool lead = k == 0;
                    const uint32_t bw_ = (uint32_t)__builtin_amdgcn_readlane((int)(two ? best2 : best1), win);
                    const uint32_t xs = ((bw_ & 255u) << 6) + (uint32_t)win;
                    const uint32_t rs = XR[xs];
                    const uint32_t ws = L.W[xs];
                    const int rts = L.RT[rs];
                    const uint32_t vw = xs | (rs << 16);
                    const int dV = wfld(ws, kWIncR) + wfldw(ws, kWIncL, lead ? 2u : 0u) + (two ? dvos[1] : dvos[0]) + ((two != kSmall) ? (rts >> 16) : wfldw(rts, 0, 16u));
                    int mx1 = -1, mx2 = -1;
#pragma unroll
                    for (int i2 = 0; i2 < NW; ++i2) { mx1 = max(mx1, mr[i2]); mx2 = max(mx2, mr[NW + i2]); }
                    const bool has_missing = (two ? mx2 : mx1) >= 0;
                    const int dObj = -(two ? gs[1] : gs[0]) + (has_missing ? (two ? role_w2<NS>(c2, vw, wl2, wf2) : role_w2<NS>(c1, vw, wl1, wf1)) : 0);
                    finish(kReplace, std::true_type{}, kmin, win, p, k, 0, 0, uw, vw, dV, dObj);
                }
            } else {
            auto slot_of = [&](int wA, int &p, int &k, uint32_t &uw, int &g_old, int &dV_old, int &dV_rack_old, Part<NW> &a, Part<NW> &c) {
                p = __builtin_amdgcn_readlane(pl_, wA);
                k = __builtin_amdgcn_readlane(kl_, wA);
                uw = (uint32_t)__builtin_amdgcn_readlane((int)oldw_l, wA);
                g_old = __builtin_amdgcn_readlane(g_old_l, wA);
                dV_old = __builtin_amdgcn_readlane(dvo_l, wA);
                dV_rack_old = __builtin_amdgcn_readlane(dvr_l, wA);
                if constexpr (kGlobalA) {
#pragma unroll
                    for (int i2 = 0; i2 < NW; ++i2) { a.w[i2] = (uint32_t)__builtin_amdgcn_readlane((int)a_l.w[i2], wA); c.w[i2] = (uint32_t)__builtin_amdgcn_readlane((int)c_l.w[i2], wA); }
                } else {
                    a = L.A[p];
                    c = CUR[p];
                }
            };
            if (type == 0) {
            uint32_t b_kmin = kKeyNull, b_uw = 0, b_vw = 0;
            int b_win = 0, b_p = 0, b_k = 0, b_dV = 0, b_dObj = 0;
#pragma nounroll
            for (int si = 0; si < (wA2 >= 0 ? 2 : 1); ++si) {
                int p, k, g_old, dV_old, dV_rack_old;
                uint32_t uw;
                Part<NW> a, c;
                slot_of(si == 0 ? wA1 : wA2, p, k, uw, g_old, dV_old, dV_rack_old, a, c);
                const bool lead = k == 0;
                const uint32_t ro = uw >> 16;
                uint32_t vw = 0;
                int dV = 0, dObj = 0;
                {
                    const int dP_rack_old = kPriced ? p_out(L.K[ro], T.rack_lo, T.rack_hi, PG[ro]) : 0;
                    for (int r = lane; r < T.R; r += 64) {
                        int v = ((uint32_t)r != ro) ? dV_rack_old + dinc(L.K[r], T.rack_lo, T.rack_hi) + c7_delta(T.c7_inc, cnt4x2<NS>(a, (uint32_t)r)) : 0;
                        if (kPriced)
                            v = (v & 0xFF) | ((((uint32_t)r != ro) ? dP_rack_old + p_in(L.K[r], T.rack_lo, T.rack_hi, PG[r]) : 0) * 256);
                        L.RT[r] = v;
                    }
                }
                const int wl = lead ? T.w00 : T.w01, wf = lead ? T.w10 : T.w11;
                const int li = lane & (NW - 1);
                const uint32_t ai = sel_slot<NS>(a, li), ci = sel_slot<NS>(c, li);
                const bool holds = (lane < NS) & (ai != kNoneW);
                uint32_t w_keep = 0;
                if (!kTeam && holds) {
                    w_keep = L.W[ai & 0xFFFFu];
                    L.W[ai & 0xFFFFu] = (uint16_t)(w_keep | kWNoCand);
                }
                int ar[NS];
                {
                    const int ar_l = (kTeam && holds) ? (int)((ai & 0xFFFFu) >> 6) : -1;
#pragma unroll
                    for (int i2 = 0; i2 < NS; ++i2) ar[i2] = __builtin_amdgcn_readlane(ar_l, i2);
                }
                const bool hm_l = (lane < NS) & (ci != kNoneW) & !in4<NS>(a, ci);
                const int mr_l = hm_l ? (int)((ci & 0xFFFFu) >> 6) : -1;
                int mr[NS];
#pragma unroll
                for (int i2 = 0; i2 < NS; ++i2) mr[i2] = __builtin_amdgcn_readlane(mr_l, i2);
                bool has_missing = false;
#pragma unroll
                for (int i2 = 0; i2 < NS; ++i2) has_missing |= mr[i2] >= 0;
                int K0 = __mul24(S, g_old) + kDBias + __mul24(lam, dV_old);
                if (kPriced) {
                    const uint32_t pro = PR[uw & 0xFFFFu];
                    const uint32_t wo = L.W[uw & 0xFFFFu];
                    K0 -= wflag(wo, kWPoutR) & price_rep(pro);
                    if (lead) K0 -= wflag(wo, kWPoutL) & price_lead(pro);
                }
                const uint32_t lw = lead ? 2u : 0u, lf = lead ? 1u : 0u;
                uint32_t bestA = kKeyNull;
                int chunkA = 0;
                const short *Ws = reinterpret_cast<const short *>(L.W);
                auto scan_round_on = [&](auto with_w, int base, int rd, int w, int rt) -> uint32_t {
                    const uint32_t st = lcg24(rng);
                    int dsc;
                    if (kPriced) {
                        const uint32_t prx = PR[base + lane];
                        const int dVx = wfld(w, kWIncR) + wfldw(w, kWIncL, lw) + (int)(signed char)(rt & 0xFF);
                        dsc = __mul24(lam, dVx) + K0 + (rt >> 8) + (wflag(w, kWPinR) & price_rep(prx)) + (wflagw(w, kWPinL, lf) & price_lead(prx));
                        if (hbw) dsc -= __mul24(S, bw_of(BW[base + lane], lead));
                    } else {
                        const int dVx = wfld(w, kWIncR) + wfldw(w, kWIncL, lw) + rt;
                        dsc = __mul24(lam, dVx) + K0;
                    }
                    uint32_t member = 0;
                    if (decltype(with_w)::value) {
                        const uint32_t x = (uint32_t)(base + lane);
                        const uint32_t xw = x | ((uint32_t)XR[x] << 16);
                        dsc -= __mul24(S, role_w2<NS>(c, xw, wl, wf));
                        if (kTeam && in4<NS>(a, xw)) member = 0xFFFF0000u;
                    }
                    dsc = min(max(dsc, 0), 2 * kDBias - 2);
                    return ((uint32_t)dsc << 16) | (st & 0xFF00u) | (uint32_t)rd | ((uint32_t)w & 0xFFFF0000u) | member;
                };
                auto scan_round = [&](auto with_w, int base, int rd) -> uint32_t {
                    const int w = Ws[base + lane];
                    return scan_round_on(with_w, base, rd, w, L.RT[XR[base + lane]]);
                };
                auto scan_pair = [&](int base, int rd) -> uint32_t {
                    const int wa = Ws[base + lane], wb = Ws[base + 64 + lane];
                    const uint32_t ra = XR[base + lane], rb = XR[base + 64 + lane];
                    const int rta = L.RT[ra], rtb = L.RT[rb];
                    const uint32_t k0 = scan_round_on(std::false_type{}, base, rd, wa, rta);
                    const uint32_t k1 = scan_round_on(std::false_type{}, base + 64, rd + 1, wb, rtb);
                    return min(k0, k1);
                };
                auto is_weighted = [&](int rdg) {
                    bool wgt = false;
#pragma unroll
                    for (int i2 = 0; i2 < NS; ++i2) wgt |= (mr[i2] == rdg) | (kTeam && ar[i2] == rdg);
                    return wgt;
                };
                for (int cb = 0; cb < T.Bx; cb += 16384) {
                    uint32_t bestc = kKeyNull;
                    const int cend = min(T.Bx, cb + 16384);
                    int rd = 0, base = cb;
                    if (kWide) {
                        for (; base + 64 < cend; base += 128, rd += 2) {
                            const int rdg = (cb >> 6) + rd;
                            if (is_weighted(rdg) || is_weighted(rdg + 1)) {
                                bestc = min(bestc, is_weighted(rdg) ? scan_round(std::true_type{}, base, rd) : scan_round(std::false_type{}, base, rd));
                                bestc = min(bestc, is_weighted(rdg + 1) ? scan_round(std::true_type{}, base + 64, rd + 1) : scan_round(std::false_type{}, base + 64, rd + 1));
                            } else bestc = min(bestc, scan_pair(base, rd));
                        }
                    }
                    if (kWide || kTeam) {
                        for (; base < cend; base += 64, ++rd)
                            bestc = min(bestc, is_weighted((cb >> 6) + rd) ? scan_round(std::true_type{}, base, rd) : scan_round(std::false_type{}, base, rd));
                    } else {
                        const int n_rd = (cend - cb + 63) >> 6, rd0 = cb >> 6;
                        while (rd < n_rd) {
                            int nxt = n_rd;
#pragma unroll
                            for (int i2 = 0; i2 < NS; ++i2) {
                                const int m = mr[i2] - rd0;
                                if (m >= rd) nxt = min(nxt, m);
                            }
                            for (; rd + 1 < nxt; rd += 2, base += 128) bestc = min(bestc, scan_pair(base, rd));
                            if (rd < nxt) { bestc = min(bestc, scan_round(std::false_type{}, base, rd)); ++rd; base += 64; }
                            if (rd < n_rd) { bestc = min(bestc, scan_round(std::true_type{}, base, rd)); ++rd; base += 64; }
                        }
                    }
                    if ((bestc >> 8) < (bestA >> 8)) { bestA = bestc; chunkA = cb; }
                }
                if (!kTeam && holds) L.W[ai & 0xFFFFu] = (uint16_t)w_keep;
                const uint32_t key = bestA >> 8;
                const uint32_t kmin = wave_umin(key);
                const unsigned long long bal = __ballot(key == kmin);
                const int win = __ffsll((long long)bal) - 1;
                if ((int)(kmin >> 8) - kDBias <= 0) {
                    const uint32_t bw_ = (uint32_t)__builtin_amdgcn_readlane((int)bestA, win);
                    const uint32_t xs = (uint32_t)__builtin_amdgcn_readlane(chunkA, win) + ((bw_ & 255u) << 6) + (uint32_t)win;
                    const uint32_t rs = XR[xs];
                    const uint32_t ws = L.W[xs];
                    const int rts = L.RT[rs];
                    vw = xs | (rs << 16);
                    dV = wfld(ws, kWIncR) + wfldw(ws, kWIncL, lw) + dV_old + (kPriced ? (int)(signed char)(rts & 0xFF) : rts);
                    dObj = -g_old + (has_missing ? role_w2<NS>(c, vw, wl, wf) : 0) + (hbw ? bw_of(BW[xs], lead) : 0);
                }
                if (si == 0 || kmin < b_kmin) { b_kmin = kmin; b_win = win; b_p = p; b_k = k; b_uw = uw; b_vw = vw; b_dV = dV; b_dObj = dObj; }
            }
            finish(kReplace, std::true_type{}, b_kmin, b_win, b_p, b_k, 0, 0, b_uw, b_vw, b_dV, b_dObj);
            } else {
                int p, k, g_old, dV_old, dV_rack_old;
                uint32_t uw;
                Part<NW> a, c;
                slot_of(wA1, p, k, uw, g_old, dV_old, dV_rack_old, a, c);
                const bool lead = k == 0;
                const uint32_t ro = uw >> 16;
                uint32_t key = kKeyNull, vw = 0;
                int dV = 0, dObj = 0, q = 0, j = 0;
                const int nrp = lead ? 0 : 1;
                const int cnt_a_ru2 = cnt4x2<NS>(a, ro);
                const uint32_t wu = L.W[uw & 0xFFFFu];
                const int pl_u = kPriced ? price_lead(PR[uw & 0xFFFFu]) : 0;
                const int bwl_u = hbw ? (int)(BW[uw & 0xFFFFu] >> 16) : 0;
                if (!kGlobalA) {
                    const int q_draw = (int)rnd24_wide(rng, (uint32_t)T.P);
                    q0 = x_windowed ? __builtin_amdgcn_readfirstlane(q_draw) : 0;
                }
                const int x_rounds = x_windowed ? 8 : x_rounds_full;
                auto x_round = [&](int rd, const Part<NW> &b, const Part<NW> &cb) {
                    const uint32_t tie0 = lcg24(rng) >> 8;
                    int qq; bool okq;
                    x_partner(rd, qq, okq);
                    okq = okq & (qq != p);
                    const bool u_in_b = in4<NS>(b, uw);
                    const int u_in_q_lead = role_w2<NS>(cb, uw, T.w00, T.w10), u_in_q_fol = role_w2<NS>(cb, uw, T.w01, T.w11);
                    const int dv_ro = c7_delta(T.c7_dec, cnt_a_ru2) + c7_delta(T.c7_inc, cnt4x2<NS>(b, ro));
                    int cnt_b_rv[3] = {0, 0, 0};
                    if constexpr (RFT == 3) {
                        const int e01 = (int)((b.w[0] >> 16) == (b.w[1] >> 16)), e02 = (int)((b.w[0] >> 16) == (b.w[2] >> 16)), e12 = (int)((b.w[1] >> 16) == (b.w[2] >> 16));
                        cnt_b_rv[0] = (1 + e01 + e02) << 1; cnt_b_rv[1] = (1 + e01 + e12) << 1; cnt_b_rv[2] = (1 + e02 + e12) << 1;
                    }
#pragma unroll
                    for (int jj = 0; jj < NS; ++jj) {
                        if (!RFT && jj >= T.RF) break;
                        const uint32_t v = b.w[jj];
                        const bool ok = okq & (v != uw) & !in4<NS>(a, v) & !u_in_b;
                        const int nrq = jj != 0;
                        int dObjx = role_w<NS>(T, c, v, nrp) + (jj == 0 ? u_in_q_lead : u_in_q_fol) - g_old - role_w<NS>(T, cb, v, nrq);
                        int dVx = 0, dPx = 0;
                        if (lead != (jj == 0)) {
                            const uint32_t wv = L.W[v & 0xFFFFu];
                            dVx += lead ? (wfld(wu, kWDecL) + wfld(wv, kWIncL)) : (wfld(wv, kWDecL) + wfld(wu, kWIncL));
                            if (kPriced) {
                                if (hbw) { const int dbl = (int)(BW[v & 0xFFFFu] >> 16) - bwl_u; dObjx += lead ? dbl : -dbl; }
                                const int plv = price_lead(PR[v & 0xFFFFu]);
                                dPx = lead ? ((wflag(wv, kWPinL) & plv) - (wflag(wu, kWPoutL) & pl_u))
                                           : ((wflag(wu, kWPinL) & pl_u) - (wflag(wv, kWPoutL) & plv));
                            }
                        }
                        const uint32_t rv = v >> 16;
                        if (rv != ro)
                            dVx += dv_ro + c7_delta(T.c7_inc, cnt4x2<NS>(a, rv)) + c7_delta(T.c7_dec, RFT == 3 ? cnt_b_rv[jj < 3 ? jj : 0] : cnt4x2<NS>(b, rv));
                        uint32_t keyx;
                        if constexpr (kSmall) keyx = ok ? key_small(mad24s(lam, dVx, mad24s(-S, dObjx, kDBias)), (tie0 + (uint32_t)jj * 0x55u) & 0xFFu) : kKeyNull;
                        else if (kPriced) keyx = ok ? make_key_tie_p(lam, S, dVx, dObjx, dPx, tie0 + (uint32_t)jj * 0x55u) : kKeyNull;
                        else keyx = ok ? make_key_tie(lam, S, dVx, dObjx, tie0 + (uint32_t)jj * 0x55u) : kKeyNull;
                        if (keyx < key) { key = keyx; vw = v; q = qq; j = jj; dV = dVx; dObj = dObjx; }
                    }
                };
                if constexpr (kGlobalA) {
#pragma unroll
                    for (int r2 = 0; r2 < XB; ++r2)
                        if (r2 < x_rounds) x_round(r2, xb[r2], xcb[r2]);
                    for (int rb = XB; rb < x_rounds; rb += XB) {
                        Part<NW> yb[XB], ycb[XB];
#pragma unroll
                        for (int r2 = 0; r2 < XB; ++r2) { int qq; bool okq; const int qc = x_partner(rb + r2, qq, okq); yb[r2] = L.A[qc]; ycb[r2] = CUR[qc]; }
#pragma unroll
                        for (int r2 = 0; r2 < XB; ++r2)
                            if (rb + r2 < x_rounds) x_round(rb + r2, yb[r2], ycb[r2]);
                    }
                } else {
                    for (int rd = 0; rd < x_rounds; ++rd) {
                        int qq; bool okq;
                        const int qc = x_partner(rd, qq, okq);
                        const Part<NW> b = L.A[qc];
                        const Part<NW> cb = CUR[qc];
                        x_round(rd, b, cb);
                    }
                }
                const uint32_t kmin = wave_umin(key);
                const unsigned long long bal = __ballot(key == kmin);
                const int win = __ffsll((long long)bal) - 1;
                finish(kExchange, std::false_type{}, kmin, win, p, k, q, j, uw, vw, dV, dObj);
            }
            }
        }
        if (V == 0 && obj > best_obj) { best_obj = obj; snapshot(T, L, ext, best, tid, nthr); }
    }

    if (kTeam) __syncthreads();
    recount(T, L, tid, nthr, krt);
    if (kTeam) __syncthreads();
    int V2, obj2;
    T = topic_regs<RFT>(TD);
    full_cost<NW, kTeam>(T, L, CUR, RSZ, tid, nthr, V2, obj2, hbw ? BW : nullptr, TS, wave, n_waves);
    if ((V2 != V || obj2 != obj) && tid == 0) atomicAdd(pl.drift, 1);
    if (!kGlobalA)
        for (int p = lane; p < T.P; p += 64) store_packed<NW>(state_packed, p, L.A[p]);
    if (tid == 0) {
        pl.restart_info[g * 4 + 0] = best_obj;
        pl.restart_info[g * 4 + 1] = V2;
        pl.restart_info[g * 4 + 2] = obj2;
        pl.restart_info[g * 4 + 3] = accepted;
    }
}

#ifndef KAO_WPE_SMALL
#define KAO_WPE_SMALL 6
#endif
#ifndef KAO_WPE_WIDE
#define KAO_WPE_WIDE 6
#endif
template <bool kGlobalA, bool kPriced, int NW, bool kWide> constexpr int search_min_waves() { return kGlobalA ? 1 : (kWide ? KAO_WPE_WIDE : KAO_WPE_SMALL); }
template <bool kGlobalA, bool kPriced, int NW, bool kWide, int RFT = 0, bool kSmall = false>
__global__ __launch_bounds__(256) __attribute__((amdgpu_waves_per_eu(search_min_waves<kGlobalA, kPriced, NW, kWide>(), 8))) void k_search(SearchPools pl, SearchParams prm) {
    extern __shared__ __attribute__((aligned(16))) unsigned char smem[];
    search_body<kGlobalA, kPriced, NW, kWide, false, false, RFT, kSmall>(smem, pl, prm);
}
template <bool kPriced, int NW>
__global__ __launch_bounds__(256) void k_search_curg(SearchPools pl, SearchParams prm) {
    extern __shared__ __attribute__((aligned(16))) unsigned char smem[];
    search_body<false, kPriced, NW, true, false, true>(smem, pl, prm);
}
template <bool kPriced, int NW>
__global__ __launch_bounds__(NW == 8 ? 256 : 512) void k_team(SearchPools pl, SearchParams prm) {
    extern __shared__ __attribute__((aligned(16))) unsigned char smem[];
    search_body<true, kPriced, NW, true, true>(smem, pl, prm);
}

constexpr int kInitWaves = 16;
constexpr size_t init_lds_total(size_t maxBx, int maxR, bool priced, bool bw) {
    const size_t bx64 = (maxBx + 63) & ~(size_t)63, krt = (size_t)search_rack_tab(maxR);
    return krt * 4 + bx64 + (priced ? (bw ? 2 : 1) * bx64 * 4 + krt * 4 : 0) + bx64 * 4 + krt * 4 + (size_t)kInitWaves * krt * 4 + 3 * 8;
}
size_t init_lds_bytes(int maxBx, int maxR, bool priced, bool bw) { return init_lds_total((size_t)maxBx, maxR, priced, bw); }
static_assert(init_lds_total(500, 255, false, false) == 21016 && init_lds_total(500, 255, true, true) == 26136, "init_lds_total no longer sums the LDS carve of k_init");
template <bool kPriced, int NW>
__global__ __launch_bounds__(64 * kInitWaves) void k_init(SearchPools pl, SearchParams prm, int per_block) {
    extern __shared__ __attribute__((aligned(16))) unsigned char smem[];
    const int lane = threadIdx.x & 63;
    const int wave = __builtin_amdgcn_readfirstlane(threadIdx.x >> 6);
    const int n_waves = __builtin_amdgcn_readfirstlane((int)(blockDim.x >> 6));
    const int tid = (int)threadIdx.x, nthr = (int)blockDim.x;
    const int2 bm = pl.block_map[blockIdx.x / (unsigned)per_block];
    const TopicDev *TD = pl.topics + bm.x;
    const int rho = bm.y + (int)(blockIdx.x % (unsigned)per_block);
    if (rho >= TD->n_restarts) return;

    const TopicRegs T = topic_regs(TD);

    const int bx64 = (prm.maxBx + 63) & ~63, krt = search_rack_tab(prm.maxR);
    const bool hbw = kPriced && prm.bw != 0;
    const uint32_t inv = (uint32_t)krt - 1u;
    unsigned char *q = smem;
    int *RSZ = reinterpret_cast<int *>(q); q += krt * 4;
    uint8_t *XR = q; q += bx64;
    uint32_t *PR = reinterpret_cast<uint32_t *>(q); if (kPriced) q += bx64 * 4;
    int *PG = reinterpret_cast<int *>(q); if (kPriced) q += krt * 4;
    uint32_t *BW = reinterpret_cast<uint32_t *>(q); if (hbw) q += bx64 * 4;
    WaveLds<NW> L;
    L.C = reinterpret_cast<uint32_t *>(q); q += bx64 * 4;
    L.K = reinterpret_cast<int *>(q); q += krt * 4;
    L.W = nullptr; L.RT = nullptr;
    int *KW = reinterpret_cast<int *>(q); q += kInitWaves * krt * 4;
    unsigned long long *BEST = reinterpret_cast<unsigned long long *>(q);

    for (int r = tid; r < krt; r += nthr) {
        RSZ[r] = r < T.R ? pl.rsz_pool[TD->rsz_off + r] : 0;
        if (kPriced) PG[r] = r < T.R ? price_units(pl.price_pool[TD->price_off + 2 * TD->B + r], prm.obj_scale) : 0;
    }
    __syncthreads();
    for (int x = tid; x < ((T.Bx + 63) & ~63); x += nthr) {
        const uint32_t r = mulhi((uint32_t)x, T.magic);
        const bool valid = x < T.Bx && (int)((uint32_t)x - r * (uint32_t)T.m) < RSZ[r < (uint32_t)krt ? r : 0];
        XR[x] = valid ? (uint8_t)r : (uint8_t)inv;
        if (kPriced) {
            uint32_t pr = 0;
            if (valid) {
                const int32_t *pp = pl.price_pool + TD->price_off;
                const int b = pl.ext_pool[TD->ext_off + x];
                pr = ((uint32_t)price_units(pp[b], prm.obj_scale) & 0xFFFFu) | ((uint32_t)price_units(pp[TD->B + b], prm.obj_scale) << 16);
            }
            PR[x] = pr;
            if (hbw) BW[x] = (valid && TD->has_bw) ? pl.bw_pool[TD->bw_off + x] : 0u;
        }
    }
    const Part<NW> *CUR = reinterpret_cast<const Part<NW> *>(pl.cur_pool + TD->cur_off);
    L.A = reinterpret_cast<Part<NW> *>(pl.state_pool + TD->state_off) + (uint64_t)rho * T.P;
    const uint32_t slo = TD->seed_lo, shi = TD->seed_hi;
    const int S = prm.obj_scale;
    for (int p = tid; p < T.P; p += nthr) {
        Part<NW> c = CUR[p];
#pragma unroll
        for (int k = 1; k < NW; ++k)
            if (k >= T.RF) c.w[k] = kNoneW;
        L.A[p] = c;
    }
    __builtin_amdgcn_fence(__ATOMIC_SEQ_CST, "workgroup");
    __syncthreads();
    recount(T, L, tid, nthr, krt);
    __syncthreads();
    if (n_waves > 1) {
        for (int r = lane; r < krt; r += 64) KW[wave * krt + r] = L.K[r];
        L.K = KW + wave * krt;
        if (tid < 3) BEST[tid] = ~0ull;
        __syncthreads();
    }

    const uint32_t *HL = pl.cur_pool + TD->hole_off;
    const int n_rounds = (T.Bx + 63) >> 6;
    int par = 0;
    for (int pass = 0; pass < 2; ++pass) {
        const uint32_t n_holes = HL[pass], *hl = HL + 2 + (pass ? HL[0] : 0u);
        for (uint32_t h0 = 0; h0 < n_holes; h0 += 64) {
          const uint32_t nb = min(64u, n_holes - h0);
          const uint32_t p_l = hl[h0 + ((uint32_t)lane < nb ? (uint32_t)lane : 0u)];
          const Part<NW> a_l = L.A[p_l], c_l = CUR[p_l];
          for (uint32_t hi = 0; hi < nb; ++hi) {
            const int p = __builtin_amdgcn_readlane((int)p_l, (int)hi);
            Part<NW> a, c;
#pragma unroll
            for (int w = 0; w < NW; ++w) {
                a.w[w] = (uint32_t)__builtin_amdgcn_readlane((int)a_l.w[w], (int)hi);
                c.w[w] = (uint32_t)__builtin_amdgcn_readlane((int)c_l.w[w], (int)hi);
            }
#pragma unroll
            for (int k = 0; k < NW; ++k) {
                if (k >= T.RF) break;
                if ((k == 0) != (pass == 0)) continue;
                if (a.w[k] != kNoneW) continue;
                const uint32_t hmix = slo ^ fmix32(shi + (uint32_t)rho * 0x9E3779B1u + (uint32_t)(p * NW + k) * 0x27D4EB2Fu + 0x5BD1E995u + prm.gen * 0x632BE5ABu);
                const int wl = k == 0 ? T.w00 : T.w01, wf = k == 0 ? T.w10 : T.w11;
                uint32_t key = kKeyNull, xw_l = kNoneW;
                for (int j = wave; j < n_rounds; j += n_waves) {
                    const uint32_t x = (uint32_t)(j * 64 + lane);
                    const uint32_t r = XR[x];
                    const uint32_t xw = x | (r << 16);
                    const bool okx = (r != inv) & !in4(a, xw);
                    const uint32_t cn = L.C[x];
                    int dV = dinc((int)(cn & 0xFFFFu), T.rep_lo, T.rep_hi) + dinc(L.K[r], T.rack_lo, T.rack_hi) +
                             dinc(cnt4(a, r), T.prack_lo, T.prack_hi);
                    if (k == 0) dV += dinc((int)(cn >> 16), T.lead_lo, T.lead_hi);
                    const uint32_t tie = fmix32(hmix + x * 0x165667B1u) >> 24;
                    uint32_t keyx;
                    if (kPriced) {
                        const uint32_t prx = PR[x];
                        int dP = p_in((int)(cn & 0xFFFFu), T.rep_lo, T.rep_hi, price_rep(prx)) + p_in(L.K[r], T.rack_lo, T.rack_hi, PG[r]);
                        if (k == 0) dP += p_in((int)(cn >> 16), T.lead_lo, T.lead_hi, price_lead(prx));
                        keyx = okx ? make_key_tie_p(prm.lam_max, S, dV, role_w2(c, xw, wl, wf) + (hbw ? bw_of(BW[x], k == 0) : 0), dP, tie) : kKeyNull;
                    }
                    else keyx = okx ? make_key_tie(prm.lam_max, S, dV, role_w2(c, xw, wl, wf), tie) : kKeyNull;
                    if (keyx < key) { key = keyx; xw_l = xw; }
                }
                uint32_t kmin = wave_umin(key);
                const unsigned long long bal = __ballot(key == kmin);
                const int l_win = __ffsll((long long)bal) - 1;
                uint32_t xw_win = (uint32_t)__builtin_amdgcn_readlane((int)xw_l, l_win);
                if (n_waves > 1) {
                    if (lane == 0) atomicMin(&BEST[par], ((unsigned long long)kmin << 32) | ((unsigned long long)l_win << 24) | ((unsigned long long)((xw_win & 0xFFFFu) >> 6) << 8) | (xw_win >> 16 & 0xFFu));
                    asm volatile("s_waitcnt lgkmcnt(0)\n\ts_barrier" ::: "memory");
                    const unsigned long long bw = BEST[par];
                    const int nxt = par == 2 ? 0 : par + 1;
                    if (tid == 0) BEST[nxt == 2 ? 0 : nxt + 1] = ~0ull;
                    par = nxt;
                    const uint32_t lo = (uint32_t)bw;
                    xw_win = (((lo >> 8) & 0xFFFFu) << 6 | (lo >> 24)) | ((lo & 0xFFu) << 16);
                }
                a.w[k] = xw_win;
                if (lane == 0) {
                    const int owner = (int)(((xw_win & 0xFFFFu) >> 6) & (uint32_t)(n_waves - 1));
                    if (wave == owner) {
                        reinterpret_cast<uint32_t *>(&L.A[p])[k] = xw_win;
                        L.C[xw_win & 0xFFFFu] += (k == 0) ? 0x10001u : 1u;
                    }
                    L.K[xw_win >> 16] += 1;
                }
            }
          }
        }
        __builtin_amdgcn_fence(__ATOMIC_SEQ_CST, "workgroup");
        __syncthreads();
    }
}

constexpr size_t search_lds_total(size_t maxP, size_t maxBx, size_t waves, bool global_a, bool priced, size_t nw, bool bw, int maxR, size_t team, bool cur_global) {
    const size_t a = global_a ? 0 : maxP * 4 * nw, bx64 = (maxBx + 63) & ~(size_t)63, krt = (size_t)search_rack_tab(maxR);
    const size_t shared = (cur_global ? 0 : a) + krt * 4 + bx64 + (priced ? (bw ? 2 : 1) * bx64 * 4 + krt * 4 : 0);
    if (team > 0)
        return shared + bx64 * 6 + krt * 4 + team * krt * 4 + 2 * 16 * kTeamRec * 4 + 16 * 2 * 4;
    return shared + waves * (a + bx64 * 6 + krt * 8);
}
size_t search_lds_bytes(int maxP, int maxBx, int waves, bool global_a, bool priced, int nw, bool bw, int maxR, int team, bool cur_global) {
    return search_lds_total((size_t)maxP, (size_t)maxBx, (size_t)waves, global_a, priced, (size_t)nw, bw, maxR, (size_t)team, cur_global);
}
static_assert(search_lds_total(50, 500, 4, false, false, 4, false, 10, 0, false) == 19104 && search_lds_total(50, 500, 4, false, false, 8, false, 10, 0, false) == 23104 &&
              search_lds_total(50, 500, 4, false, true, 4, false, 10, 0, false) == 21408 && search_lds_total(50, 500, 4, false, true, 4, true, 10, 0, false) == 23456 &&
              search_lds_total(9800, 500, 1, false, false, 4, false, 10, 0, true) == 161152 && search_lds_total(100000, 500, 1, true, false, 4, false, 10, 8, false) == 7808,
              "search_lds_total no longer sums the LDS carve of search_body");

bool search_rf3_eligible(bool global_a, bool cur_global, bool priced, int nw, int team) { return !global_a && !cur_global && !priced && nw == 4 && team == 0; }

bool search_band_tabs(int rep_lo, int rep_hi, int lead_lo, int lead_hi) { return band_tab_fits(rep_lo, rep_hi) && band_tab_fits(lead_lo, lead_hi); }
bool search_small_cost(int lam_min, int lam_max, int obj_scale, int w_abs_max, bool priced) {
    if (priced || lam_min < 0 || lam_max < lam_min || obj_scale < 1 || w_abs_max < 0) return false;
    return 8 * (int64_t)lam_max + 4 * (int64_t)obj_scale * (int64_t)w_abs_max <= (int64_t)kSmallCostMax;
}

void launch_search(const SearchPools &pools, const SearchParams &prm, int n_blocks, int waves, bool global_a, bool priced, int nw, void *stream, int team, int rft, bool small) {
    const bool curg = prm.cur_global != 0 && !global_a, wide = prm.wide != 0;
    const size_t lds = search_lds_bytes(prm.maxP, prm.maxBx, waves, global_a, priced, nw, prm.bw != 0, prm.maxR, team, curg);
    hipStream_t st = static_cast<hipStream_t>(stream);
    const dim3 grid(n_blocks), block(64 * (team > 0 && !curg ? team : waves));
    if (rft == 3 && search_rf3_eligible(global_a, curg, priced, nw, team)) {
        if (small) {
            if (wide) launch_lds<k_search<false, false, 4, true, 3, true>>(grid, block, lds, st, pools, prm);
            else launch_lds<k_search<false, false, 4, false, 3, true>>(grid, block, lds, st, pools, prm);
        }
        else if (wide) launch_lds<k_search<false, false, 4, true, 3>>(grid, block, lds, st, pools, prm);
        else launch_lds<k_search<false, false, 4, false, 3>>(grid, block, lds, st, pools, prm);
        return;
    }
    with_flags(priced, nw == 8, [&](auto p, auto k8) {
        constexpr bool kPriced = decltype(p)::value;
        constexpr int NW = decltype(k8)::value ? 8 : 4;
        if (curg) launch_lds<k_search_curg<kPriced, NW>>(grid, block, lds, st, pools, prm);
        else if (team > 0) launch_lds<k_team<kPriced, NW>>(grid, block, lds, st, pools, prm);
        else if (global_a) launch_lds<k_search<true, kPriced, NW, true>>(grid, block, lds, st, pools, prm);
        else if (wide) launch_lds<k_search<false, kPriced, NW, true>>(grid, block, lds, st, pools, prm);
        else launch_lds<k_search<false, kPriced, NW, false>>(grid, block, lds, st, pools, prm);
    });
}

bool launch_init(const SearchPools &pools, const SearchParams &prm, int n_blocks, int per_block, bool priced, int nw, int waves, void *stream) {
    const size_t lds = init_lds_bytes(prm.maxBx, prm.maxR, priced, prm.bw != 0);
    if (lds > 160 * 1024) return false;
    waves = waves > 0 ? std::min(kInitWaves, waves) : std::min(8, std::max(1, (prm.maxBx + 63) / 64));
    while (waves & (waves - 1)) waves &= waves - 1;
    const dim3 grid((unsigned)(n_blocks * per_block)), block((unsigned)(64 * waves));
    with_flags(priced, nw == 8, [&](auto p, auto k8) {
        launch_lds<k_init<decltype(p)::value, decltype(k8)::value ? 8 : 4>>(grid, block, lds, static_cast<hipStream_t>(stream), pools, prm, per_block);
    });
    return true;
}

}

extern "C" int kao_search_band_row(int32_t lo, int32_t hi, int32_t c, int32_t force_plain, int32_t *fits) {
    using namespace kao;
    const bool tab = band_tab_fits(lo, hi);
    if (fits) *fits = tab ? 1 : 0;
    if (tab && !force_plain) return (int)band_lookup_plain(c, band_tab_bias(lo), band_tab(lo, hi));
    const int a = std::min(std::max(c - lo, -1), 1), b = std::min(std::max(c - hi, -1), 1);
    return (int)((kBandTab >> (uint32_t)(6 * (3 * a + b) + 24)) & 63u);
}
extern "C" int kao_search_rack_delta(int32_t lo, int32_t hi, int32_t c, int32_t dec) {
    const uint32_t tab = kao::c7_tab(dec != 0, lo, hi);
    const uint32_t f = (tab >> ((2u * (uint32_t)c) & 31u)) & 3u;
    return (int)(f ^ 2u) - 2;
}
```

### kafka_assignment_optimizer_amd/csrc/kao_session.cpp

```cpp
#include <cstring>

#include "kao_host.h"

namespace {

constexpr int kEvRing = 32;

template <typename Item>
std::vector<Item> xcd_order(const std::vector<Item> &items, const std::vector<int> &topic_of) {
    const size_t n = items.size();
    std::vector<std::vector<size_t>> q(8);
    for (size_t i = 0; i < n; ++i) q[(size_t)topic_of[i] % 8].push_back(i);
    std::vector<size_t> head(8, 0);
    std::vector<Item> out;
    out.reserve(n);
    for (size_t b = 0; b < n; ++b) {
        size_t x = b % 8;
        if (head[x] >= q[x].size()) {
            size_t bestx = 0, bestlen = 0;
            for (size_t y = 0; y < 8; ++y)
                if (q[y].size() - head[y] > bestlen) { bestlen = q[y].size() - head[y]; bestx = y; }
            x = bestx;
            out.push_back(items[q[x].back()]);
            q[x].pop_back();
            continue;
        }
        out.push_back(items[q[x][head[x]++]]);
    }
    return out;
}

int session_drain_events(kao_session *s) {
    for (int i = 0; i < s->ev_pending; ++i) {
        float a = 0, b = 0;
        HIP_TRY(hipEventSynchronize(s->ev[i * 3 + 2]));
        HIP_TRY(hipEventElapsedTime(&a, s->ev[i * 3 + 0], s->ev[i * 3 + 1]));
        HIP_TRY(hipEventElapsedTime(&b, s->ev[i * 3 + 1], s->ev[i * 3 + 2]));
        s->ms_search += a;
        s->ms_eval += b;
    }
    s->ev_pending = 0;
    return KAO_OK;
}

int resolve_opts(const kao_topic *topics, int n_topics, const kao_opts *opts_in, int n_cu, uint64_t device_bytes, kao_opts &o) {
    o = opts_in ? *opts_in : kao_opts{};
    if (o.team < 0 || o.team > kTeamMax || o.schedule < 0 || o.schedule > 1) return fail(KAO_ERR_INVALID, "kao_opts: team must be 0..8, schedule 0 or 1");
    if (o.iters_per_launch <= 0) o.iters_per_launch = 512;
    if (o.obj_scale <= 0) o.obj_scale = 4;
    if (o.lam_min <= 0) o.lam_min = 1;
    if (o.lam_max <= 0) o.lam_max = 40;
    if (o.lam_max < o.lam_min) o.lam_max = o.lam_min;
    if (o.period_log2 < 0) o.period_log2 = 0;
    if (o.period_log2 > 20) o.period_log2 = 20;
    if (o.time_limit_s <= 0) o.time_limit_s = 10.0;
    if (o.elite_period < 0) o.elite_period = 0;
    if (o.restarts <= 0) {
        const int want = n_cu * 32;
        int r = want / n_topics;
        r = (r / kWaves) * kWaves;
        o.restarts = std::min(std::max(r, 8), 8192);
        int64_t slots = 1;
        for (int t = 0; t < n_topics; ++t) slots = std::max<int64_t>(slots, (int64_t)topics[t].n_partitions * std::max(topics[t].rf, 1));
        const int floor_r = slots >= 32768 ? 4 * n_cu : n_cu;
        const int cap = (int)std::max<int64_t>(floor_r, (((int64_t)1 << 22) / slots) / kWaves * kWaves);
        o.restarts = std::min(o.restarts, cap);
        if (n_topics == 1 && o.restarts > n_cu && o.restarts <= n_cu + n_cu / 4 && o.team <= 1) {
            const kao_topic &t0 = topics[0];
            std::vector<int> rs((size_t)std::max(t0.n_racks, 1), 0);
            for (int b = 0; b < t0.n_brokers; ++b) if (t0.rack_of[b] < rs.size()) rs[t0.rack_of[b]]++;
            const int bx = *std::max_element(rs.begin(), rs.end()) * t0.n_racks, nw0 = (t0.rf > kRFP || t0.rf_cur > kRFP) ? 2 * kRFP : kRFP;
            const bool hbw = t0.broker_w || t0.broker_wl;
            if (search_lds_bytes(t0.n_partitions, bx, 1, false, true, nw0, hbw, t0.n_racks) > kLdsLimit &&
                search_lds_bytes(t0.n_partitions, bx, 1, false, true, nw0, hbw, t0.n_racks, 0, true) <= kLdsLimit)
                o.restarts = n_cu / kWaves * kWaves;
        }
    }
    if (o.restarts > (1 << 20) - 2) o.restarts = (1 << 20) - 2;
    uint64_t per_restart = 0;
    for (int t = 0; t < n_topics; ++t) per_restart += (uint64_t)topics[t].n_partitions * (32 + 2 * (uint64_t)std::max(topics[t].rf, 1));
    uint64_t budget = 8ull << 30;
    if (device_bytes > 0) budget = std::min<uint64_t>(budget, std::max<uint64_t>(device_bytes / 8, 256ull << 20));
    const uint64_t cap = budget / std::max<uint64_t>(per_restart, 1);
    if ((uint64_t)o.restarts > cap) o.restarts = (int)std::max<uint64_t>(cap / kWaves * kWaves, kWaves);
    return KAO_OK;
}

struct SessionPlan {
    std::vector<TopicDev> tds;
    std::vector<int2> smap;
    std::vector<int4> emap;
    std::vector<uint32_t> cur_pool, bw_pool, bwd_pool; std::vector<uint16_t> ext_pool, curd_pool, int_pool; std::vector<int32_t> rsz_pool;
    std::vector<uint8_t> rackof_pool;
    uint64_t state_bytes = 0, best_u16 = 0, win_u16 = 0, dual_i32 = 0, price_i32 = 0, wide_slices = 0;
};
template <typename T>
uint32_t append(std::vector<T> &pool, const std::vector<T> &v) { pool.insert(pool.end(), v.begin(), v.end()); return (uint32_t)(pool.size() - v.size()); }

void plan_topic(kao_session &s, int t, bool curg_on, int n_cu, SessionPlan &pl) {
    const kao_opts &o = s.opts;
    const PreparedTopic &pt = s.pts[(size_t)t];
    TopicDev &d = s.pts[(size_t)t].d;
    d.n_restarts = o.restarts;
    d.period_log2 = o.period_log2 > 0 ? o.period_log2 : auto_period_log2(d.P, d.RF);
    d.restart_base = t * o.restarts;
    std::vector<uint32_t> &cur_pool = pl.cur_pool;
    while (cur_pool.size() % 4) cur_pool.push_back(kNoneW);
    d.cur_off = (uint32_t)cur_pool.size();
    for (size_t i = 0; i < (size_t)d.P * d.nw; ++i) cur_pool.push_back(replica_word(pt.cur_int[i], d.m));
    {
        d.hole_off = (uint32_t)cur_pool.size();
        const size_t w0 = (size_t)d.cur_off;
        std::vector<uint32_t> lead, foll;
        for (int p = 0; p < d.P; ++p) {
            bool fh = false;
            for (int k = 1; k < d.RF; ++k) fh |= cur_pool[w0 + (size_t)p * d.nw + k] == kNoneW;
            if (cur_pool[w0 + (size_t)p * d.nw] == kNoneW) lead.push_back((uint32_t)p);
            if (fh) foll.push_back((uint32_t)p);
        }
        cur_pool.push_back((uint32_t)lead.size()); cur_pool.push_back((uint32_t)foll.size());
        append(cur_pool, lead);
        append(cur_pool, foll);
    }
    const bool both_fit = search_lds_bytes(d.P, d.Bx, 1, false, true, d.nw, s.any_bw, d.R) <= kLdsLimit;
    const bool curg = !both_fit && curg_on && o.team <= 1 && o.restarts <= n_cu &&
                      search_lds_bytes(d.P, d.Bx, 1, false, true, d.nw, s.any_bw, d.R, 0, true) <= kLdsLimit;
    const bool global_a = !both_fit && !curg;
    s.topic_global[(size_t)t] = global_a;
    s.topic_curg[(size_t)t] = curg;
    d.ext_off = append(pl.ext_pool, pt.ext_of);
    d.rsz_off = append(pl.rsz_pool, pt.rack_size);
    d.state_off = pl.state_bytes;
    pl.state_bytes += align_up((uint64_t)o.restarts * d.P * d.nw * (global_a ? 4 : 2));
    d.best_off = pl.best_u16;
    pl.best_u16 += (uint64_t)o.restarts * d.P * d.RF;
    d.win_off = (uint32_t)pl.win_u16;
    pl.win_u16 += (uint64_t)d.P * d.RF;
    d.rackof_off = append(pl.rackof_pool, pt.rack_of);
    d.curd_off = append(pl.curd_pool, pt.cur_dense);
    if (d.has_bw) {
        d.bw_off = append(pl.bw_pool, pt.bw_int);
        d.bwd_off = append(pl.bwd_pool, pt.bw_dense);
        s.priced = true;
        s.any_bw = true;
    }
    d.int_off = append(pl.int_pool, pt.int_of);
    d.price_off = (uint32_t)pl.price_i32;
    pl.price_i32 += 2 * (uint64_t)d.B + kRackTab;
    pl.dual_i32 = (pl.dual_i32 + 1) & ~(uint64_t)1;
    d.dual_off = (uint32_t)pl.dual_i32;
    pl.dual_i32 += 6 * (uint64_t)d.B + 3 * kRackTab + 8;
    d.cnt_off = (uint32_t)pl.dual_i32;
    pl.dual_i32 += 3 * (2 * (uint64_t)d.B + kRackTab) + 4 * (uint64_t)d.B + 2 * kRackTab;
    pl.wide_slices += (uint64_t)(d.P + 63) / 64;
    s.eval_bytes_per_launch += (uint64_t)o.restarts * (uint64_t)(2 * d.RF * d.P + 2 * d.rf_cur * d.P + d.B);
}

int plan_groups(kao_session &s, int n_cu, SessionPlan &pl) {
    const kao_opts &o = s.opts;
    const bool rft_on = env_int("KAO_SEARCH_RFT", 1) != 0;
    s.small_on = env_int("KAO_SEARCH_SMALL", 1) != 0;
    std::vector<int> order((size_t)s.n_topics);
    for (int t = 0; t < s.n_topics; ++t) order[(size_t)t] = t;
    auto need1 = [&](int t) {
        const TopicDev &d = s.pts[(size_t)t].d;
        const bool ga = s.topic_global[(size_t)t] != 0;
        const bool cg = s.topic_curg[(size_t)t] != 0;
        return (ga ? ((size_t)1 << 40) : 0) + (cg ? ((size_t)1 << 39) : 0) + (d.nw > kRFP ? ((size_t)1 << 41) : 0) + search_lds_bytes(d.P, d.Bx, 1, ga, true, d.nw, s.any_bw, d.R, 0, cg);
    };
    std::stable_sort(order.begin(), order.end(), [&](int x, int y) { return need1(x) < need1(y); });
    std::vector<std::vector<int>> members;
    size_t group_base = 0;
    auto kind = [&](int t) { return (s.topic_global[(size_t)t] ? 1 : 0) | (s.pts[(size_t)t].d.nw > kRFP ? 2 : 0) | (s.topic_curg[(size_t)t] ? 4 : 0); };
    int lds_groups = 0, group_kind = -1;
    for (int t : order) {
        const bool new_kind = members.empty() || kind(t) != group_kind;
        if (new_kind || (need1(t) > 2 * group_base && lds_groups < 8)) {
            members.emplace_back(); group_base = need1(t); group_kind = kind(t);
            if (new_kind) lds_groups = 1; else ++lds_groups;
        }
        members.back().push_back(t);
    }
    for (const std::vector<int> &mem : members) {
        kao_session::LaunchGroup g;
        int64_t n_cand = 0;
        for (int t : mem) n_cand += s.pts[(size_t)t].d.n_restarts;
        const int64_t fill = 4 * (int64_t)std::max(n_cu, 1);
        int cpb = 32;
        if (n_cand < fill * 32) cpb = (int)std::min<int64_t>(32, std::max<int64_t>(kWaves, ((n_cand + fill - 1) / fill + kWaves - 1) / kWaves * kWaves));
        for (int t : mem) {
            const TopicDev &d = s.pts[(size_t)t].d;
            g.rf_uniform = g.rf_uniform < 0 ? d.RF : (g.rf_uniform == d.RF ? d.RF : 0);
            for (const int w : {d.w00, d.w01, d.w10, d.w11}) g.w_abs_max = std::max(g.w_abs_max, w < 0 ? (w == INT32_MIN ? INT32_MAX : -w) : w);
            g.band_tabs = g.band_tabs && search_band_tabs(d.rep_lo, d.rep_hi, d.lead_lo, d.lead_hi);
            g.rf3 = g.rf3 && d.RF == 3 && d.rf_cur <= 3;
            g.maxP = std::max(g.maxP, d.P); g.maxBx = std::max(g.maxBx, d.Bx); g.maxB = std::max(g.maxB, d.B); g.maxR = std::max(g.maxR, d.R); g.wide = g.wide || (int64_t)d.P * d.RF >= 512;
        }
        g.rf3 = g.rf3 && rft_on;
        g.global_a = s.topic_global[(size_t)mem[0]] != 0;
        g.cur_global = s.topic_curg[(size_t)mem[0]] != 0;
        g.nw = s.pts[(size_t)mem[0]].d.nw;
        g.eval_coop = n_cand <= fill && g.maxP >= 1024;
        if (g.eval_coop) cpb = 1;
        if (g.global_a) {
            const int tmax = g.nw > kRFP ? kTeamMax / 2 : kTeamMax;
            const int want = o.team == 0 ? 1 : o.team;
            g.team = want <= 1 ? 0 : std::min(want, tmax);
            if (g.team > 0) g.waves = 1;
        }
        auto search_lds = [&] { return search_lds_bytes(g.maxP, g.maxBx, g.waves, g.global_a, true, g.nw, s.any_bw, g.maxR, g.team, g.cur_global); };
        while (g.waves > 1 && search_lds() > kLdsLimit) g.waves /= 2;
        g.cur_in_lds = eval_lds_bytes(g.maxP, g.maxB, true, g.nw) <= kLdsLimit;
        if (search_lds() > kLdsLimit || eval_lds_bytes(g.maxP, g.maxB, g.cur_in_lds, g.nw) > kLdsLimit)
            return fail(KAO_ERR_UNSUPPORTED, "broker tables exceed 160 KiB of LDS (about 30,000 padded brokers)");
        std::vector<int2> gs; std::vector<int> gs_topic;
        std::vector<int4> ge; std::vector<int> ge_topic;
        for (int t : mem) {
            const TopicDev &d = s.pts[(size_t)t].d;
            for (int r = 0; r < d.n_restarts; r += g.waves) { gs.push_back(make_int2(t, r)); gs_topic.push_back(t); }
            for (int r = 0; r < d.n_restarts; r += cpb) {
                ge.push_back(make_int4(t, r, std::min(cpb, d.n_restarts - r), d.restart_base + r));
                ge_topic.push_back(t);
            }
        }
        gs = xcd_order(gs, gs_topic);
        ge = xcd_order(ge, ge_topic);
        g.smap_off = (int)pl.smap.size(); g.smap_n = (int)gs.size();
        g.emap_off = (int)pl.emap.size(); g.emap_n = (int)ge.size();
        pl.smap.insert(pl.smap.end(), gs.begin(), gs.end());
        pl.emap.insert(pl.emap.end(), ge.begin(), ge.end());
        s.groups.push_back(g);
    }
    s.blocks_search = (int)pl.smap.size();
    s.blocks_eval = (int)pl.emap.size();
    return KAO_OK;
}

int plan_session(kao_session &s, const kao_topic *topics, int n_cu, SessionPlan &pl) {
    const int n_topics = s.n_topics;
    s.pts.resize((size_t)n_topics);
    s.topics.assign(topics, topics + n_topics);
    s.ub.resize((size_t)n_topics);
    s.topic_global.assign((size_t)n_topics, 0);
    s.topic_curg.assign((size_t)n_topics, 0);
    for (int t = 0; t < n_topics; ++t) s.any_bw |= topics[t].broker_w || topics[t].broker_wl;
    const bool curg_on = env_int("KAO_CUR_GLOBAL", 1) != 0;
    for (int t = 0; t < n_topics; ++t) {
        const uint64_t seed = s.opts.seed ^ ((uint64_t)(t + 1) * 0x9E3779B97F4A7C15ull);
        const int rc = prepare(&topics[t], seed, s.pts[(size_t)t]);
        if (rc) return rc;
        s.ub[(size_t)t] = upper_bound_w(&topics[t]);
        s.topic_infeasible.push_back(infeasible_reason(&topics[t]).empty() ? 0 : 1);
        plan_topic(s, t, curg_on, n_cu, pl);
        s.dual_ok.push_back(dual_supported(&topics[t], s.any_bw) ? 1 : 0);
    }
    s.dual_flags.assign((size_t)n_topics, 0);
    s.dual_iters.assign((size_t)n_topics, 0);
    for (int t = 0; t < n_topics; ++t) if (!s.dual_ok[(size_t)t]) s.dual_flags[(size_t)t] = 8;
    s.total_restarts = n_topics * s.opts.restarts;
    const int rc = plan_groups(s, n_cu, pl);
    for (const PreparedTopic &pt : s.pts) pl.tds.push_back(pt.d);
    return rc;
}

struct ArenaLayout {
    struct Sec { void *slot; size_t off, bytes; const void *src; };
    std::vector<Sec> secs;
    size_t total = 0;
    template <typename T>
    void add(T *&dev_ptr, size_t bytes, const void *src = nullptr) {
        secs.push_back({&dev_ptr, total, bytes, src});
        total += align_up(bytes);
    }
    template <typename T, typename V>
    void add(T *&dev_ptr, const std::vector<V> &image) { add(dev_ptr, image.size() * sizeof(V), image.data()); }
    void stage(unsigned char *host) const {
        for (const Sec &sec : secs) if (sec.bytes && sec.src) std::memcpy(host + sec.off, sec.src, sec.bytes);
    }
    void bind(void *base) const {
        for (const Sec &sec : secs) { unsigned char *p = static_cast<unsigned char *>(base) + sec.off; std::memcpy(sec.slot, &p, sizeof p); }
    }
};

ArenaLayout layout_ro(kao_session &s, const SessionPlan &pl) {
    ArenaLayout a;
    a.add(s.d_topics, pl.tds);
    a.add(s.d_smap, pl.smap);
    a.add(s.d_emap, pl.emap);
    a.add(s.d_cur, pl.cur_pool);
    a.add(s.d_ext, pl.ext_pool);
    a.add(s.d_rsz, pl.rsz_pool);
    a.add(s.d_rackof, pl.rackof_pool);
    a.add(s.d_curd, pl.curd_pool);
    a.add(s.d_int, pl.int_pool);
    a.add(s.d_bw, pl.bw_pool);
    a.add(s.d_bwd, pl.bwd_pool);
    return a;
}

ArenaLayout layout_rw(kao_session &s, const SessionPlan &pl) {
    const size_t n_topics = (size_t)s.n_topics, n_restarts = (size_t)s.total_restarts;
    s.rb_viol_off = align_up(n_topics * 8 + 16, 16);
    s.rb_assign_off = s.rb_viol_off + n_topics * 32;
    s.readback_bytes = s.rb_assign_off + pl.win_u16 * 2;
    uint64_t dual_i32 = (pl.dual_i32 + 1) & ~(uint64_t)1;
    s.wide_ctl_i32 = dual_i32; dual_i32 += 32 * (uint64_t)n_topics;
    s.wide_map_i32 = dual_i32; dual_i32 += 2 * pl.wide_slices;
    s.dual_bytes = align_up(dual_i32 * 4);
    s.dual_rb_bytes = n_topics * 24;
    s.price_half_i32 = align_up(pl.price_i32 * 4) / 4;
    s.best_bytes = pl.best_u16 * 2 ? pl.best_u16 * 2 : 2;
    ArenaLayout a;
    a.add(s.d_state, pl.state_bytes);
    a.add(s.d_best, pl.best_u16 * 2);
    a.add(s.d_info, n_restarts * 16);
    a.add(s.d_obj, n_restarts * 4);
    a.add(s.d_viol, n_restarts * 32);
    a.add(s.d_readback, s.readback_bytes);
    a.add(s.d_dual, s.dual_bytes);
    a.add(s.d_dual_target, n_topics * 8);
    a.add(s.d_dual_ids, n_topics * 4);
    a.add(s.d_dual_rb, s.dual_rb_bytes);
    a.add(s.d_price, 2 * s.price_half_i32 * 4);
    a.add(s.d_keys_glob, n_topics * 8);
    return a;
}

}

extern "C" {

void kao_session_destroy(kao_session *s) {
    if (!s) return;
    (void)hipSetDevice(s->device);
    if (s->stream) (void)hipStreamSynchronize(s->stream);
    if (s->stream_bound) (void)hipStreamSynchronize(s->stream_bound);
    if (s->ev_bound0) (void)hipEventDestroy(s->ev_bound0);
    if (s->ev_bound1) (void)hipEventDestroy(s->ev_bound1);
    if (s->ev_search) (void)hipEventDestroy(s->ev_search);
    if (s->stream_bound) (void)hipStreamDestroy(s->stream_bound);
    arena_put(s->arena_ro, s->arena_ro_bytes, s->device);
    arena_put(s->arena_rw, s->arena_rw_bytes, s->device);
    for (hipEvent_t e : s->ev) (void)hipEventDestroy(e);
    stream_put(s->stream, s->device);
    delete s;
}

int kao_session_create(const kao_topic *topics, int32_t n_topics, const kao_opts *opts_in, kao_session **out) {
    if (!out) return fail(KAO_ERR_INVALID, "null out");
    *out = nullptr;
    if (!topics || n_topics < 1) return fail(KAO_ERR_INVALID, "no topics");
    int rc = require_init();
    if (rc) return rc;
    SessionPtr s(new kao_session());
    s->device = cur_device();
    s->n_topics = n_topics;
    const int n_cu = num_cu(s->device);
    size_t free_b = 0, total_b = 0;
    if (hipMemGetInfo(&free_b, &total_b) != hipSuccess) total_b = 0;
    if ((rc = resolve_opts(topics, n_topics, opts_in, n_cu, total_b, s->opts))) return rc;
    SessionPlan pl;
    if ((rc = plan_session(*s, topics, n_cu, pl))) return rc;

    const ArenaLayout ro = layout_ro(*s, pl), rw = layout_rw(*s, pl);
    if ((rc = arena_get(ro.total, &s->arena_ro, &s->arena_ro_bytes))) return rc;
    if ((rc = arena_get(rw.total, &s->arena_rw, &s->arena_rw_bytes))) return rc;
    ro.bind(s->arena_ro);
    rw.bind(s->arena_rw);
    s->d_keys = reinterpret_cast<unsigned long long *>(s->d_readback);
    s->d_drift = reinterpret_cast<int32_t *>(s->d_readback + (size_t)n_topics * 8);
    s->d_win_viol = reinterpret_cast<int32_t *>(s->d_readback + s->rb_viol_off);
    s->d_win_assign = reinterpret_cast<uint16_t *>(s->d_readback + s->rb_assign_off);
    s->h_readback.assign(s->readback_bytes, 0);
    std::vector<unsigned char> stage(ro.total);
    ro.stage(stage.data());

    if ((rc = stream_get(&s->stream))) return rc;
    const size_t price_b = 2 * s->price_half_i32 * 4;
    hipError_t e1 = hipMemcpyAsync(s->arena_ro, stage.data(), ro.total, hipMemcpyHostToDevice, s->stream);
    hipError_t e2 = hipMemsetAsync(s->d_best, 0xFF, s->best_bytes, s->stream);
    hipError_t e3 = hipMemsetAsync(s->d_readback, 0xFF, (size_t)n_topics * 8, s->stream);
    hipError_t e4 = hipMemsetAsync(s->d_drift, 0, 16, s->stream);
    if (e4 == hipSuccess) e4 = hipMemsetAsync(s->d_price, 0, price_b ? price_b : 4, s->stream);
    hipError_t e5 = hipStreamSynchronize(s->stream);
    if (e1 != hipSuccess || e2 != hipSuccess || e3 != hipSuccess || e4 != hipSuccess || e5 != hipSuccess) return fail(KAO_ERR_HIP, "session upload failed");
    if (s->opts.profile) {
        s->ev.resize(kEvRing * 3);
        for (auto &e : s->ev) if (hipEventCreate(&e) != hipSuccess) return fail(KAO_ERR_HIP, "hipEventCreate");
    }
    *out = s.release();
    return KAO_OK;
}

int kao_session_step(kao_session *s) {
    if (!s) return fail(KAO_ERR_INVALID, "null session");
    HIP_TRY(hipSetDevice(s->device));
    const bool prof = s->opts.profile != 0;
    if (prof && s->ev_pending == kEvRing) {
        int rc = session_drain_events(s);
        if (rc) return rc;
    }
    SearchPools sp{};
    sp.topics = s->d_topics; sp.block_map = s->d_smap; sp.cur_pool = s->d_cur; sp.ext_pool = s->d_ext; sp.rsz_pool = s->d_rsz;
    sp.state_pool = s->d_state; sp.best_pool = s->d_best; sp.restart_info = s->d_info; sp.drift = s->d_drift;
    SearchParams prm{};
    prm.obj_scale = s->opts.obj_scale; prm.lam_min = s->opts.lam_min; prm.lam_max = s->opts.lam_max;
    prm.launch = s->launch; prm.iters = (uint32_t)s->opts.iters_per_launch; prm.init = (s->launch == 0 || s->reinit) ? 1 : 0;
    prm.gen = s->gen;
    s->reinit = false;
    const int eper = s->opts.elite_period;
    prm.bw = s->any_bw ? 1 : 0;
    prm.scan2_max = kScanTwoSlots;
    prm.elite = (eper > 0 && s->launch > 0 && s->launch % (uint32_t)eper == 0) ? 1 : 0;
    sp.price_pool = s->d_price + (size_t)s->price_read * s->price_half_i32;
    sp.int_pool = s->d_int; sp.elite_assign = s->d_win_assign; sp.elite_key = s->d_keys; sp.bw_pool = s->d_bw;
    EvalPools ep{};
    ep.topics = s->d_topics; ep.rackof_pool = s->d_rackof; ep.curd_pool = s->d_curd;
    ep.cand = s->d_best; ep.objective = s->d_obj; ep.violations = s->d_viol; ep.best_key = s->d_keys; ep.bwd_pool = s->d_bwd;
    hipEvent_t *e = prof ? &s->ev[(size_t)s->ev_pending * 3] : nullptr;
    if (prof) HIP_TRY(hipEventRecord(e[0], s->stream));
    for (const kao_session::LaunchGroup &g : s->groups) {
        sp.block_map = s->d_smap + g.smap_off;
        prm.maxP = g.maxP; prm.maxBx = g.maxBx; prm.maxR = g.maxR; prm.wide = g.wide ? 1 : 0; prm.cur_global = g.cur_global ? 1 : 0;
        SearchParams gp = prm;
        if (gp.init && g.global_a) {
            const int init_waves = (int)env_int("KAO_INIT_WAVES", -1);
            if (init_waves != 0 && launch_init(sp, gp, g.smap_n, g.team > 0 ? 1 : g.waves, s->priced, g.nw, std::max(init_waves, 0), s->stream)) gp.init = 2;
            HIP_TRY(hipGetLastError());
        }
        const int rft = g.rf3 ? 3 : 0;
        const bool rf3_runs = rft && search_rf3_eligible(g.global_a, g.cur_global, s->priced, g.nw, g.team);
        const bool small = rf3_runs && s->small_on && g.band_tabs && search_small_cost(gp.lam_min, gp.lam_max, gp.obj_scale, g.w_abs_max, s->priced);
        launch_search(sp, gp, g.smap_n, g.waves, g.global_a, s->priced, g.nw, s->stream, g.team, rft, small);
        if (rf3_runs) s->search_rf3_launches++;
        if (small) s->search_small_launches++;
        HIP_TRY(hipGetLastError());
    }
    if (prof) HIP_TRY(hipEventRecord(e[1], s->stream));
    for (const kao_session::LaunchGroup &g : s->groups) {
        ep.block_map = s->d_emap + g.emap_off;
        ep.maxP = g.maxP; ep.maxB = g.maxB; ep.cur_in_lds = g.cur_in_lds ? 1 : 0; ep.coop = g.eval_coop ? 1 : 0; ep.rf_uniform = std::max(g.rf_uniform, 0);
        launch_eval(ep, g.emap_n, g.nw, s->stream);
        HIP_TRY(hipGetLastError());
    }
    if (prof) { HIP_TRY(hipEventRecord(e[2], s->stream)); s->ev_pending++; }
    if (eper > 0 && (s->launch + 1) % (uint32_t)eper == 0) {
        launch_gather(s->d_topics, s->n_topics, s->d_keys, s->d_best, s->d_viol, s->d_win_assign, s->d_win_viol, s->stream);
        HIP_TRY(hipGetLastError());
    }
    for (const PreparedTopic &pt : s->pts) {
        const uint64_t n = neighbours_in_range(prm.launch * prm.iters, prm.iters, pt.d.RF, pt.d.B, pt.d.P, prm.scan2_max) * (uint64_t)pt.d.n_restarts;
        s->delta_total += n;
        s->search_bytes_total += n * (uint64_t)(8 * pt.d.RF + 10);
    }
    s->launch++;
    return KAO_OK;
}

int kao_session_new_generation(kao_session *s) {
    if (!s) return fail(KAO_ERR_INVALID, "null session");
    HIP_TRY(hipSetDevice(s->device));
    HIP_TRY(hipMemsetAsync(s->d_best, 0xFF, s->best_bytes, s->stream));
    HIP_TRY(hipMemsetAsync(s->d_readback, 0xFF, (size_t)s->n_topics * 8, s->stream));
    s->gen++;
    s->reinit = true;
    return KAO_OK;
}

int kao_session_sync(kao_session *s) {
    if (!s) return fail(KAO_ERR_INVALID, "null session");
    HIP_TRY(hipSetDevice(s->device));
    HIP_TRY(hipStreamSynchronize(s->stream));
    if (s->opts.profile) return session_drain_events(s);
    return KAO_OK;
}

int kao_session_best_keys(kao_session *s, uint64_t *keys) {
    if (!s || !keys) return fail(KAO_ERR_INVALID, "null argument");
    HIP_TRY(hipSetDevice(s->device));
    HIP_TRY(hipMemcpyAsync(keys, s->d_keys, (size_t)s->n_topics * 8, hipMemcpyDeviceToHost, s->stream));
    HIP_TRY(hipStreamSynchronize(s->stream));
    return KAO_OK;
}

int kao_session_device_keys(kao_session *s, void **d_keys) {
    if (!s || !d_keys) return fail(KAO_ERR_INVALID, "null argument");
    *d_keys = s->d_keys;
    return KAO_OK;
}

int kao_session_best(kao_session *s, kao_result *results) {
    if (!s || !results) return fail(KAO_ERR_INVALID, "null argument");
    HIP_TRY(hipSetDevice(s->device));
    launch_gather(s->d_topics, s->n_topics, s->d_keys, s->d_best, s->d_viol, s->d_win_assign, s->d_win_viol, s->stream);
    HIP_TRY(hipGetLastError());
    HIP_TRY(hipMemcpyAsync(s->h_readback.data(), s->d_readback, s->readback_bytes, hipMemcpyDeviceToHost, s->stream));
    int rc = kao_session_sync(s);
    if (rc) return rc;
    const uint64_t *keys = reinterpret_cast<const uint64_t *>(s->h_readback.data());
    const int32_t *wv = reinterpret_cast<const int32_t *>(s->h_readback.data() + s->rb_viol_off);
    const uint16_t *wa = reinterpret_cast<const uint16_t *>(s->h_readback.data() + s->rb_assign_off);
    for (int t = 0; t < s->n_topics; ++t) {
        const TopicDev &d = s->pts[(size_t)t].d;
        kao_result &r = results[t];
        r.upper_bound = s->ub[(size_t)t];
        const uint64_t key = keys[t];
        if (key == ~0ull) {
            r.status = s->topic_infeasible[(size_t)t] ? KAO_STATUS_INFEASIBLE_PROVEN : KAO_STATUS_NO_FEASIBLE; r.best_restart = -1; r.objective = -1;
            std::memset(r.violations, 0, sizeof r.violations);
            continue;
        }
        r.best_restart = (key & 0xFFFFF) == kExternalRestart ? -1 : (int)(key & 0xFFFFF);
        r.objective = (int64_t)kObjCap - (int64_t)((key >> 20) & 0xFFFFFF);
        std::memcpy(r.violations, wv + (size_t)t * 8, 32);
        if (r.assignment) std::memcpy(r.assignment, wa + d.win_off, (size_t)d.P * d.RF * 2);
        if (r.violations[0] != 0) { r.status = s->topic_infeasible[(size_t)t] ? KAO_STATUS_INFEASIBLE_PROVEN : KAO_STATUS_NO_FEASIBLE; r.objective = -1; }
        else r.status = r.objective >= r.upper_bound ? KAO_STATUS_OPTIMAL_PROVEN : KAO_STATUS_FEASIBLE_BOUND_GAP;
    }
    return KAO_OK;
}

int kao_session_stats(kao_session *s, kao_stats *out) {
    if (!s || !out) return fail(KAO_ERR_INVALID, "null argument");
    int rc = kao_session_sync(s);
    if (rc) return rc;
    std::memset(out, 0, sizeof *out);
    out->launches = s->launch;
    out->delta_candidates = s->delta_total;
    out->full_candidates = (uint64_t)s->launch * (uint64_t)s->total_restarts;
    out->ms_search = s->ms_search; out->ms_eval = s->ms_eval;
    out->search_bytes_algo = s->search_bytes_total;
    out->eval_bytes_algo = s->eval_bytes_per_launch * s->launch;
    out->n_restarts_total = s->total_restarts;
    for (const kao_session::LaunchGroup &g : s->groups)
        out->lds_bytes_search = std::max(out->lds_bytes_search, (int32_t)search_lds_bytes(g.maxP, g.maxBx, g.waves, g.global_a, s->priced, g.nw, s->any_bw, g.maxR, g.team, g.cur_global));
    out->launch_groups = (int32_t)s->groups.size();
    out->blocks_search = s->blocks_search;
    out->search_rf3_launches = (int32_t)std::min<uint64_t>(s->search_rf3_launches, (uint64_t)INT32_MAX);
    HIP_TRY(hipMemcpy(&out->drift, s->d_drift, 4, hipMemcpyDeviceToHost));
    return KAO_OK;
}

int kao_session_small_launches(kao_session *s, int64_t *out) {
    if (!s || !out) return fail(KAO_ERR_INVALID, "null argument");
    *out = (int64_t)s->search_small_launches;
    return KAO_OK;
}

int kao_session_restart_state(kao_session *s, int32_t topic, int32_t restart, uint16_t *final_state, uint16_t *best_state,
                              int32_t info[4]) {
    if (!s || topic < 0 || topic >= s->n_topics) return fail(KAO_ERR_INVALID, "bad topic");
    const PreparedTopic &pt = s->pts[(size_t)topic];
    const TopicDev &d = pt.d;
    if (restart < 0 || restart >= d.n_restarts) return fail(KAO_ERR_INVALID, "bad restart");
    HIP_TRY(hipSetDevice(s->device));
    int rc = kao_session_sync(s);
    if (rc) return rc;
    if (final_state) {
        const bool ga = s->topic_global[(size_t)topic] != 0;
        const int nw = d.nw;
        std::vector<uint16_t> raw((size_t)d.P * nw * (ga ? 2 : 1));
        HIP_TRY(hipMemcpy(raw.data(), s->d_state + d.state_off + (uint64_t)restart * d.P * nw * (ga ? 4 : 2), raw.size() * 2, hipMemcpyDeviceToHost));
        for (int p = 0; p < d.P; ++p)
            for (int k = 0; k < d.RF; ++k) {
                const uint16_t x = ga ? raw[((size_t)p * nw + k) * 2] : raw[(size_t)p * nw + k];
                final_state[(size_t)p * d.RF + k] = x < pt.ext_of.size() ? pt.ext_of[x] : (uint16_t)KAO_NONE;
            }
    }
    if (best_state)
        HIP_TRY(hipMemcpy(best_state, s->d_best + d.best_off + (uint64_t)restart * d.P * d.RF, (size_t)d.P * d.RF * 2, hipMemcpyDeviceToHost));
    if (info) HIP_TRY(hipMemcpy(info, s->d_info + (size_t)(d.restart_base + restart) * 4, 16, hipMemcpyDeviceToHost));
    return KAO_OK;
}

}

namespace kao {

int session_topic_best(kao_session *s, int i, uint16_t *out) {
    HIP_TRY(hipSetDevice(s->device));
    launch_gather(s->d_topics, s->n_topics, s->d_keys, s->d_best, s->d_viol, s->d_win_assign, s->d_win_viol, s->stream);
    HIP_TRY(hipGetLastError());
    const TopicDev &d = s->pts[(size_t)i].d;
    HIP_TRY(hipMemcpyAsync(out, s->d_win_assign + d.win_off, (size_t)d.P * d.RF * 2, hipMemcpyDeviceToHost, s->stream));
    HIP_TRY(hipStreamSynchronize(s->stream));
    return KAO_OK;
}
int session_restart_objs(kao_session *s, int i, std::vector<int32_t> &objs) {
    HIP_TRY(hipSetDevice(s->device));
    const TopicDev &d = s->pts[(size_t)i].d;
    std::vector<int32_t> info((size_t)d.n_restarts * 4);
    HIP_TRY(hipMemcpyAsync(info.data(), s->d_info + (size_t)d.restart_base * 4, info.size() * 4, hipMemcpyDeviceToHost, s->stream));
    HIP_TRY(hipStreamSynchronize(s->stream));
    objs.resize((size_t)d.n_restarts);
    for (int r = 0; r < d.n_restarts; ++r) objs[(size_t)r] = info[(size_t)r * 4];
    return KAO_OK;
}
int session_restart_best(kao_session *s, int i, int restart, uint16_t *out) {
    HIP_TRY(hipSetDevice(s->device));
    const TopicDev &d = s->pts[(size_t)i].d;
    if (restart < 0 || restart >= d.n_restarts) return fail(KAO_ERR_INVALID, "bad restart");
    HIP_TRY(hipMemcpyAsync(out, s->d_best + d.best_off + (uint64_t)restart * d.P * d.RF, (size_t)d.P * d.RF * 2, hipMemcpyDeviceToHost, s->stream));
    HIP_TRY(hipStreamSynchronize(s->stream));
    return KAO_OK;
}
int session_adopt_external(kao_session *s, int i, const uint16_t *assign, int64_t objective, uint64_t *key_out) {
    HIP_TRY(hipSetDevice(s->device));
    const TopicDev &d = s->pts[(size_t)i].d;
    const uint64_t key = ((uint64_t)((int64_t)kObjCap - objective) << 20) | (uint64_t)kExternalRestart;
    HIP_TRY(hipStreamSynchronize(s->stream));
    HIP_TRY(hipMemcpyAsync(s->d_win_assign + d.win_off, assign, (size_t)d.P * d.RF * 2, hipMemcpyHostToDevice, s->stream));
    HIP_TRY(hipMemcpyAsync(s->d_keys + i, &key, 8, hipMemcpyHostToDevice, s->stream));
    HIP_TRY(hipStreamSynchronize(s->stream));
    *key_out = key;
    return KAO_OK;
}

}
```

### kafka_assignment_optimizer_amd/solver.py

```python
from __future__ import annotations

import ctypes as C
from dataclasses import dataclass
from typing import List, Optional, Sequence

import numpy as np

from . import _ffi
from .model import BOUND_KEYS, Topic

STATUS_NAMES = {0: "OPTIMAL_PROVEN", 1: "FEASIBLE_BOUND_GAP", 2: "NO_FEASIBLE", 3: "TIME_LIMIT", 4: "INFEASIBLE_PROVEN"}


class KaoError(RuntimeError):
    def __init__(self, code: int, where: str):
        lib = _ffi.load()
        detail = lib.kao_last_error().decode(errors="replace")
        super().__init__(f"{where}: {lib.kao_strerror(code).decode()} ({code}) {detail}")
        self.code = code


def _check(rc: int, where: str):
    if rc != 0:
        raise KaoError(rc, where)


def library_path() -> str:
    return _ffi.LIB_PATH


def init(device: int = 0):
    _check(_ffi.load().kao_init(int(device)), "kao_init")


def device_name() -> str:
    buf = C.create_string_buffer(256)
    _check(_ffi.load().kao_device_name(buf, 256), "kao_device_name")
    return buf.value.decode()


class _CTopics:

    def __init__(self, topics: Sequence[Topic]):
        self.keep = []
        self.arr = (_ffi.KaoTopic * len(topics))()
        for i, t in enumerate(topics):
            s = self.arr[i]
            rack = np.ascontiguousarray(t.rack_of, dtype=np.uint8)
            cur = np.ascontiguousarray(t.current, dtype=np.uint16)
            self.keep += [rack, cur]
            s.n_brokers, s.n_racks, s.n_partitions = t.n_brokers, int(t.n_racks), int(t.n_partitions)
            s.rf, s.rf_cur = int(t.rf), int(cur.shape[1])
            s.rack_of = rack.ctypes.data_as(C.POINTER(C.c_uint8))
            s.current = cur.ctypes.data_as(C.POINTER(C.c_uint16))
            for a in range(2):
                for b in range(2):
                    s.w[a][b] = int(t.weights[a][b])
            for k in BOUND_KEYS:
                v = t.bounds_override.get(k, -1) if t.bounds_override else -1
                setattr(s, k, -1 if v is None else int(v))
            for name in ("broker_w", "broker_wl"):
                v = getattr(t, name, None)
                if v is not None:
                    arr = np.ascontiguousarray(v, dtype=np.int32)
                    if arr.shape != (t.n_brokers,):
                        raise ValueError(f"{name}: one weight per broker expected")
                    self.keep.append(arr)
                    setattr(s, name, arr.ctypes.data_as(C.POINTER(C.c_int32)))

    def ptr(self, i: int = 0):
        return C.byref(self.arr[i]) if i else self.arr


def derive_bounds(topic: Topic) -> dict:
    ct = _CTopics([topic])
    out = (C.c_int32 * 8)()
    _check(_ffi.load().kao_derive_bounds(ct.arr, out), "kao_derive_bounds")
    return dict(zip(BOUND_KEYS, [int(v) for v in out]))


def upper_bound(topic: Topic) -> int:
    ct = _CTopics([topic])
    ub = C.c_int64()
    _check(_ffi.load().kao_upper_bound(ct.arr, C.byref(ub)), "kao_upper_bound")
    return int(ub.value)


def check_infeasible(topic: Topic) -> str:
    ct = _CTopics([topic])
    buf = C.create_string_buffer(256)
    rc = _ffi.load().kao_check_infeasible(ct.arr, buf, 256)
    if rc < 0:
        raise KaoError(rc, "kao_check_infeasible")
    return buf.value.decode() if rc == 1 else ""


def evaluate(topic: Topic, assign) -> tuple:
    ct = _CTopics([topic])
    a = np.ascontiguousarray(assign, dtype=np.uint16).reshape(-1)
    if a.size != topic.n_partitions * topic.rf:
        raise ValueError("assignment must have P*rf entries")
    obj = C.c_int64()
    viol = (C.c_int32 * 8)()
    _check(_ffi.load().kao_evaluate(ct.arr, a.ctypes.data_as(C.POINTER(C.c_uint16)), C.byref(obj), viol),
           "kao_evaluate")
    return int(obj.value), np.array(list(viol), dtype=np.int64)


def evaluate_batch(topic: Topic, candidates) -> tuple:
    ct = _CTopics([topic])
    c = np.ascontiguousarray(candidates, dtype=np.uint16).reshape(-1, topic.n_partitions * topic.rf)
    n = c.shape[0]
    obj = np.zeros(n, dtype=np.int32)
    viol = np.zeros((n, 8), dtype=np.int32)
    _check(_ffi.load().kao_evaluate_batch(ct.arr, c.ctypes.data_as(C.POINTER(C.c_uint16)), n,
                                          obj.ctypes.data_as(C.POINTER(C.c_int32)),
                                          viol.ctypes.data_as(C.POINTER(C.c_int32))), "kao_evaluate_batch")
    return obj, viol


def canonicalize(topic: Topic, assign) -> np.ndarray:
    ct = _CTopics([topic])
    a = np.ascontiguousarray(assign, dtype=np.uint16).reshape(-1).copy()
    _check(_ffi.load().kao_canonicalize(ct.arr, a.ctypes.data_as(C.POINTER(C.c_uint16))), "kao_canonicalize")
    return a.reshape(topic.n_partitions, topic.rf)


def improve_cycles(topic: Topic, assign, max_rounds: int = 0) -> tuple:
    ct = _CTopics([topic])
    a = np.ascontiguousarray(assign, dtype=np.uint16).reshape(-1).copy()
    if a.size != topic.n_partitions * topic.rf:
        raise ValueError("assignment must have P*rf entries")
    obj = C.c_int64()
    st = (C.c_int32 * 8)()
    _check(_ffi.load().kao_improve_cycles(ct.arr, a.ctypes.data_as(C.POINTER(C.c_uint16)), int(max_rounds), C.byref(obj), st),
           "kao_improve_cycles")
    names = ("rounds", "improving_rounds", "realisations", "improving", "candidates", "merged", "objective_before", "objective_after")
    return a.reshape(topic.n_partitions, topic.rf), int(obj.value), dict(zip(names, (int(v) for v in st)))


def cycle_matrices(topic: Topic, assign, layer: int, level: int) -> tuple:
    ct = _CTopics([topic])
    a = np.ascontiguousarray(assign, dtype=np.uint16).reshape(-1)
    n = len(topic.broker_ids) + int(topic.n_racks) + 1
    dist = np.zeros((n, n), dtype=np.int32)
    mid = np.zeros((n, n), dtype=np.int32)
    slot = np.zeros((n, n), dtype=np.uint32)
    _check(_ffi.load().kao_cycle_matrices(ct.arr, a.ctypes.data_as(C.POINTER(C.c_uint16)), layer, level,
                                          dist.ctypes.data_as(C.POINTER(C.c_int32)), mid.ctypes.data_as(C.POINTER(C.c_int32)),
                                          slot.ctypes.data_as(C.POINTER(C.c_uint32))), "kao_cycle_matrices")
    return dist, mid, slot


def cycle_square_plan(n: int) -> tuple:
    out = (C.c_int32 * 3)()
    _check(_ffi.load().kao_cycle_square_plan(int(n), out), "kao_cycle_square_plan")
    return int(out[0]), int(out[1]), int(out[2])


def cycle_seeds(topic: Topic, assign) -> np.ndarray:
    ct = _CTopics([topic])
    a = np.ascontiguousarray(assign, dtype=np.uint16).reshape(-1)
    ncfg = C.c_int32()
    _check(_ffi.load().kao_cycle_seeds(ct.arr, a.ctypes.data_as(C.POINTER(C.c_uint16)), None, C.byref(ncfg)), "kao_cycle_seeds")
    tab = np.zeros((topic.n_partitions, ncfg.value, 2), dtype=np.int32)
    _check(_ffi.load().kao_cycle_seeds(ct.arr, a.ctypes.data_as(C.POINTER(C.c_uint16)), tab.ctypes.data_as(C.POINTER(C.c_int32)), C.byref(ncfg)),
           "kao_cycle_seeds")
    return tab


def cycle_pair_edges(topic: Topic, assign, gmin: int = -2):
    ct = _CTopics([topic])
    a = np.ascontiguousarray(assign, dtype=np.uint16).reshape(-1)
    B = topic.n_brokers
    cost = np.zeros((B, B), dtype=np.int32)
    st = (C.c_int64 * 4)()
    _check(_ffi.load().kao_cycle_pair_edges(ct.arr, a.ctypes.data_as(C.POINTER(C.c_uint16)), int(gmin), cost.ctypes.data_as(C.POINTER(C.c_int32)), st),
           "kao_cycle_pair_edges")
    return cost, dict(half_moves=int(st[0]), pairs=int(st[1]), edges=int(st[2]), closed_improving=int(st[3]))


class EvalPlan:

    def __init__(self, topic: Topic):
        self.topic = topic
        self._ct = _CTopics([topic])
        self._h = C.c_void_p()
        _check(_ffi.load().kao_eval_plan_create(self._ct.arr, C.byref(self._h)), "kao_eval_plan_create")

    def run(self, d_candidates: int, n: int, d_objective: int, d_violations: int = 0, d_best_key: int = 0):
        _check(_ffi.load().kao_eval_plan_run(self._h, C.c_void_p(d_candidates), int(n), C.c_void_p(d_objective),
                                             C.c_void_p(d_violations or None), C.c_void_p(d_best_key or None)),
               "kao_eval_plan_run")

    def sync(self) -> float:
        ms = C.c_double()
        _check(_ffi.load().kao_eval_plan_sync(self._h, C.byref(ms)), "kao_eval_plan_sync")
        return float(ms.value)

    def close(self):
        if self._h:
            _ffi.load().kao_eval_plan_destroy(self._h)
            self._h = C.c_void_p()

    def __del__(self):
        try:
            self.close()
        except Exception:
            pass


@dataclass
class Result:
    status: str
    objective: int
    upper_bound: int
    violations: np.ndarray
    assignment: np.ndarray
    best_restart: int
    seconds_to_best: float


def _make_opts(**kw) -> _ffi.KaoOpts:
    o = _ffi.KaoOpts()
    for k, v in kw.items():
        if not hasattr(o, k):
            raise TypeError(f"unknown option {k}")
        setattr(o, k, v)
    return o


def _results_buffers(topics: Sequence[Topic]):
    res = (_ffi.KaoResult * len(topics))()
    bufs = []
    for i, t in enumerate(topics):
        b = np.full(t.n_partitions * t.rf, 0xFFFF, dtype=np.uint16)
        bufs.append(b)
        res[i].assignment = b.ctypes.data_as(C.POINTER(C.c_uint16))
    return res, bufs


def _unpack(topics, res, bufs) -> List[Result]:
    out = []
    for i, t in enumerate(topics):
        r = res[i]
        out.append(Result(STATUS_NAMES.get(r.status, str(r.status)), int(r.objective), int(r.upper_bound),
                          np.array(list(r.violations), dtype=np.int64), bufs[i].reshape(t.n_partitions, t.rf).copy(),
                          int(r.best_restart), float(r.seconds_to_best)))
    return out


class Session:

    def __init__(self, topics: Sequence[Topic], **opts):
        self.topics = list(topics)
        self._ct = _CTopics(self.topics)
        self._opts = _make_opts(**opts)
        self._h = C.c_void_p()
        _check(_ffi.load().kao_session_create(self._ct.arr, len(self.topics), C.byref(self._opts), C.byref(self._h)),
               "kao_session_create")

    def step(self, n: int = 1):
        lib = _ffi.load()
        for _ in range(n):
            _check(lib.kao_session_step(self._h), "kao_session_step")

    def sync(self):
        _check(_ffi.load().kao_session_sync(self._h), "kao_session_sync")

    def new_generation(self):
        _check(_ffi.load().kao_session_new_generation(self._h), "kao_session_new_generation")

    def best(self) -> List[Result]:
        res, bufs = _results_buffers(self.topics)
        _check(_ffi.load().kao_session_best(self._h, res), "kao_session_best")
        return _unpack(self.topics, res, bufs)

    def device_keys_ptr(self) -> int:
        p = C.c_void_p()
        _check(_ffi.load().kao_session_device_keys(self._h, C.byref(p)), "kao_session_device_keys")
        return int(p.value)

    def best_keys(self) -> np.ndarray:
        keys = np.zeros(len(self.topics), dtype=np.uint64)
        _check(_ffi.load().kao_session_best_keys(self._h, keys.ctypes.data_as(C.POINTER(C.c_uint64))),
               "kao_session_best_keys")
        return keys

    def stats(self) -> dict:
        st = _ffi.KaoStats()
        _check(_ffi.load().kao_session_stats(self._h, C.byref(st)), "kao_session_stats")
        return {k: getattr(st, k) for k, _ in _ffi.KaoStats._fields_}

    def small_launches(self) -> int:
        n = C.c_int64(0)
        _check(_ffi.load().kao_session_small_launches(self._h, C.byref(n)), "kao_session_small_launches")
        return int(n.value)

    def restart_state(self, topic: int, restart: int) -> dict:
        t = self.topics[topic]
        n = t.n_partitions * t.rf
        fin = np.zeros(n, dtype=np.uint16)
        best = np.zeros(n, dtype=np.uint16)
        info = (C.c_int32 * 4)()
        _check(_ffi.load().kao_session_restart_state(self._h, topic, restart, fin.ctypes.data_as(C.POINTER(C.c_uint16)),
                                                     best.ctypes.data_as(C.POINTER(C.c_uint16)), info),
               "kao_session_restart_state")
        return dict(final=fin.reshape(t.n_partitions, t.rf), best=best.reshape(t.n_partitions, t.rf),
                    best_obj=int(info[0]), V=int(info[1]), obj=int(info[2]), n_accept=int(info[3]))

    def bound_step(self, targets: Sequence[int], iters: int = 512):
        tg = np.ascontiguousarray(targets, dtype=np.int64)
        if tg.shape != (len(self.topics),):
            raise ValueError("one target per topic")
        _check(_ffi.load().kao_session_bound_step(self._h, tg.ctypes.data_as(C.POINTER(C.c_int64)), int(iters)),
               "kao_session_bound_step")

    def set_prices(self, topic: int, a, l, g):
        t = self.topics[topic]
        a = np.ascontiguousarray(a, dtype=np.int32); l = np.ascontiguousarray(l, dtype=np.int32); g = np.ascontiguousarray(g, dtype=np.int32)
        if a.shape != (t.n_brokers,) or l.shape != (t.n_brokers,) or g.shape[0] < t.n_racks:
            raise ValueError("a[n_brokers], l[n_brokers], g[n_racks] expected")
        p32 = C.POINTER(C.c_int32)
        _check(_ffi.load().kao_session_set_prices(self._h, topic, a.ctypes.data_as(p32), l.ctypes.data_as(p32), g.ctypes.data_as(p32)),
               "kao_session_set_prices")

    def prices(self, topic: int) -> tuple:
        t = self.topics[topic]
        a = np.zeros(t.n_brokers, dtype=np.int32); l = np.zeros(t.n_brokers, dtype=np.int32); g = np.zeros(t.n_racks, dtype=np.int32)
        p32 = C.POINTER(C.c_int32)
        _check(_ffi.load().kao_session_prices(self._h, topic, a.ctypes.data_as(p32), l.ctypes.data_as(p32), g.ctypes.data_as(p32)),
               "kao_session_prices")
        return a, l, g

    def adopt_prices(self):
        _check(_ffi.load().kao_session_adopt_prices(self._h), "kao_session_adopt_prices")

    def bounds(self) -> dict:
        n = len(self.topics)
        ub = np.zeros(n, dtype=np.int64)
        fl = np.zeros(n, dtype=np.int32)
        it = np.zeros(n, dtype=np.int32)
        _check(_ffi.load().kao_session_bounds(self._h, ub.ctypes.data_as(C.POINTER(C.c_int64)),
                                              fl.ctypes.data_as(C.POINTER(C.c_int32)), it.ctypes.data_as(C.POINTER(C.c_int32))),
               "kao_session_bounds")
        return dict(upper_bound=ub, flags=fl, iters=it)

    def set_dual_state(self, topic: int, a, l, g):
        a, l, g = (np.ascontiguousarray(v, dtype=np.int32) for v in (a, l, g))
        p32 = C.POINTER(C.c_int32)
        _check(_ffi.load().kao_session_set_dual_state(self._h, topic, a.ctypes.data_as(p32), l.ctypes.data_as(p32), g.ctypes.data_as(p32)),
               "kao_session_set_dual_state")

    def dual_state(self, topic: int) -> dict:
        t = self.topics[topic]
        a = np.zeros(t.n_brokers, dtype=np.int32)
        l = np.zeros(t.n_brokers, dtype=np.int32)
        g = np.zeros(t.n_racks, dtype=np.int32)
        best = C.c_int64()
        p32 = C.POINTER(C.c_int32)
        _check(_ffi.load().kao_session_dual_state(self._h, topic, a.ctypes.data_as(p32), l.ctypes.data_as(p32),
                                                  g.ctypes.data_as(p32), C.byref(best)), "kao_session_dual_state")
        return dict(a=a, l=l, g=g, best_dual=int(best.value))

    def close(self):
        if self._h:
            _ffi.load().kao_session_destroy(self._h)
            self._h = C.c_void_p()

    def __enter__(self):
        return self

    def __exit__(self, *exc):
        self.close()

    def __del__(self):
        try:
            self.close()
        except Exception:
            pass


def dual_bound(topic: Topic, target: int, iters: int = 512, launches: int = 1) -> dict:
    ct = _CTopics([topic])
    bound, best = C.c_int64(), C.c_int64()
    itn, fl = C.c_int32(), C.c_int32()
    mult = np.zeros(2 * topic.n_brokers + topic.n_racks, dtype=np.int32)
    _check(_ffi.load().kao_dual_bound(ct.ptr(0), int(target), int(iters), int(launches), C.byref(bound), C.byref(best),
                                      C.byref(itn), C.byref(fl), mult.ctypes.data_as(C.POINTER(C.c_int32))), "kao_dual_bound")
    B = topic.n_brokers
    return dict(bound=int(bound.value), best_dual=int(best.value), iters=int(itn.value), flags=int(fl.value),
                a=mult[:B].copy(), l=mult[B:2 * B].copy(), g=mult[2 * B:].copy())


def lp_bound(topic: Topic, tol: float = 0.0, max_iters: int = 0) -> dict:
    ct = _CTopics([topic])
    bound, best = C.c_int64(), C.c_int64()
    B = topic.n_brokers
    mult = np.zeros(2 * B + topic.n_racks, dtype=np.int32)
    st = np.zeros(8)
    _check(_ffi.load().kao_lp_bound(ct.ptr(0), float(tol), int(max_iters), C.byref(bound), C.byref(best),
                                    mult.ctypes.data_as(C.POINTER(C.c_int32)), st.ctypes.data_as(C.POINTER(C.c_double))), "kao_lp_bound")
    return dict(bound=int(bound.value), best_dual=int(best.value), a=mult[:B].copy(), l=mult[B:2 * B].copy(), g=mult[2 * B:].copy(),
                iterations=int(st[0]), primal=float(st[1]), dual=float(st[2]), status=int(st[3]), mu=float(st[4]), pinf=float(st[5]),
                dinf=float(st[6]), ms=float(st[7]))


def lp_round(topic: Topic, pert: float = 0.0, salt: int = 0, tol: float = 0.0, max_iters: int = 0, fallback=None) -> dict:
    ct = _CTopics([topic])
    n = topic.n_partitions * topic.rf
    a = np.zeros(n, dtype=np.uint16) if fallback is None else np.ascontiguousarray(np.asarray(fallback).reshape(-1), dtype=np.uint16).copy()
    if a.shape != (n,):
        raise ValueError("fallback: [P, rf] expected")
    obj = C.c_int64()
    viol = (C.c_int32 * 8)()
    st = np.zeros(8)
    _check(_ffi.load().kao_lp_round(ct.ptr(0), float(pert), int(salt) & 0xFFFFFFFF, float(tol), int(max_iters), 0 if fallback is None else 1,
                                    a.ctypes.data_as(C.POINTER(C.c_uint16)), C.byref(obj), viol, st.ctypes.data_as(C.POINTER(C.c_double))), "kao_lp_round")
    return dict(assignment=a.reshape(topic.n_partitions, topic.rf), objective=int(obj.value), violations=[int(v) for v in viol],
                iterations=int(st[0]), status=int(st[1]), fractional=int(st[2]), over_inflow=int(st[3]), from_fallback=int(st[4]),
                ms_lp=float(st[5]), ms_round=float(st[6]), pert=float(st[7]))


def lp_round_host(topic: Topic, q, zq, fallback=None) -> dict:
    ct = _CTopics([topic])
    n = topic.n_partitions * topic.rf
    q = np.ascontiguousarray(q, dtype=np.uint8); zq = np.ascontiguousarray(zq, dtype=np.int32)
    a = np.zeros(n, dtype=np.uint16) if fallback is None else np.ascontiguousarray(np.asarray(fallback).reshape(-1), dtype=np.uint16).copy()
    rep = (C.c_int32 * 4)()
    _check(_ffi.load().kao_lp_round_host(ct.ptr(0), q.ctypes.data_as(C.POINTER(C.c_uint8)), zq.ctypes.data_as(C.POINTER(C.c_int32)),
                                         0 if fallback is None else 1, a.ctypes.data_as(C.POINTER(C.c_uint16)), rep), "kao_lp_round_host")
    return dict(assignment=a.reshape(topic.n_partitions, topic.rf), fractional=int(rep[0]), over_inflow=int(rep[1]), unplaced=int(rep[2]), from_fallback=int(rep[3]))


def lp_repair_host(topic: Topic, assignment) -> np.ndarray:
    ct = _CTopics([topic])
    a = np.ascontiguousarray(np.asarray(assignment).reshape(-1), dtype=np.uint16).copy()
    rep = (C.c_int32 * 4)()
    _check(_ffi.load().kao_lp_round_host(ct.ptr(0), None, None, 2, a.ctypes.data_as(C.POINTER(C.c_uint16)), rep), "kao_lp_round_host")
    return a.reshape(topic.n_partitions, topic.rf)


def lp_trace(topic: Topic, tol: float = 0.0, max_iters: int = 80) -> dict:
    ct = _CTopics([topic])
    B = topic.n_brokers
    mult = np.zeros(2 * B + topic.n_racks, dtype=np.int32)
    st = np.zeros(8)
    max_iters = int(max_iters) if int(max_iters) > 0 else 80
    tr = np.zeros(5 * (max_iters + 2))
    pd = C.POINTER(C.c_double)
    _check(_ffi.load().kao_lp_trace(ct.ptr(0), float(tol), int(max_iters), tr.ctypes.data_as(pd), st.ctypes.data_as(pd),
                                    mult.ctypes.data_as(C.POINTER(C.c_int32))), "kao_lp_trace")
    it = int(st[0])
    return dict(a=mult[:B].copy(), l=mult[B:2 * B].copy(), g=mult[2 * B:].copy(), iterations=it, primal=float(st[1]), dual=float(st[2]),
                status=int(st[3]), ms=float(st[7]), trace=tr[:5 * (it + 1)].reshape(-1, 5))


def lp_sharded(topic: Topic, devices: Sequence[int], pert: float = 0.0, salt: int = 0, tol: float = 0.0, max_iters: int = 0) -> dict:
    ct = _CTopics([topic])
    dv = np.asarray(list(devices), dtype=np.int32)
    A = np.full((topic.n_partitions, topic.rf), 0xFFFF, dtype=np.uint16)
    bound = C.c_int64(0); obj = C.c_int64(0)
    viol = np.zeros(8, dtype=np.int32); st = np.zeros(8)
    _check(_ffi.load().kao_lp_sharded_test(ct.ptr(0), dv.ctypes.data_as(C.POINTER(C.c_int32)), len(dv), float(pert), int(salt), float(tol), int(max_iters),
                                           C.byref(bound), A.ctypes.data_as(C.POINTER(C.c_uint16)), C.byref(obj), viol.ctypes.data_as(C.POINTER(C.c_int32)),
                                           st.ctypes.data_as(C.POINTER(C.c_double))), "kao_lp_sharded_test")
    return dict(bound=int(bound.value), assignment=A, objective=int(obj.value), violations=viol.tolist(), iterations=int(st[0]), status=int(st[1]),
                fractional=int(st[2]), collectives=int(st[3]), dual=float(st[4]), ms_lp=float(st[5]), ms_rest=float(st[6]), pert=float(st[7]))


def dense_spd_test(A: np.ndarray, rhs: Optional[np.ndarray] = None) -> dict:
    A = np.ascontiguousarray(A, dtype=np.float64)
    n = A.shape[0]
    assert A.shape == (n, n)
    f = np.zeros((n, n)); li = np.zeros((n // 64, 64, 64)); x = np.zeros(n); ms = np.zeros(2)
    pd = C.POINTER(C.c_double)
    r = None if rhs is None else np.ascontiguousarray(rhs, dtype=np.float64)
    _check(_ffi.load().kao_dense_spd_test(A.ctypes.data_as(pd), n, None if r is None else r.ctypes.data_as(pd), f.ctypes.data_as(pd),
                                          li.ctypes.data_as(pd), x.ctypes.data_as(pd), ms.ctypes.data_as(pd)), "kao_dense_spd_test")
    return dict(factor=f, linv=li, x=x, ms_factor=float(ms[0]), ms_solve=float(ms[1]))


def decode_key(key: int) -> tuple:
    key = int(key)
    return key >> 44, 0xFFFFFF - ((key >> 20) & 0xFFFFFF), key & 0xFFFFF


def solve(topics: Sequence[Topic], target_objective: Optional[Sequence[int]] = None, **opts) -> List[Result]:
    topics = list(topics)
    ct = _CTopics(topics)
    opts.setdefault("stop_at_bound", 1)
    o = _make_opts(**opts)
    if target_objective is not None:
        tgt = (C.c_int64 * len(topics))(*[int(v) for v in target_objective])
        o.target_objective = tgt
    res, bufs = _results_buffers(topics)
    _check(_ffi.load().kao_solve(ct.arr, len(topics), C.byref(o), res), "kao_solve")
    return _unpack(topics, res, bufs)


def solve_multi(topics: Sequence[Topic], devices: Sequence[int], target_objective: Optional[Sequence[int]] = None, **opts) -> List[Result]:
    topics = list(topics)
    ct = _CTopics(topics)
    opts.setdefault("stop_at_bound", 1)
    o = _make_opts(**opts)
    if target_objective is not None:
        tgt = (C.c_int64 * len(topics))(*[int(v) for v in target_objective])
        o.target_objective = tgt
    dev = (C.c_int32 * len(devices))(*[int(d) for d in devices])
    res, bufs = _results_buffers(topics)
    _check(_ffi.load().kao_solve_multi(ct.arr, len(topics), dev, len(devices), C.byref(o), res), "kao_solve_multi")
    return _unpack(topics, res, bufs)


def solve_capped(topics: Sequence[Topic], replica_cap: Sequence[int], devices: Optional[Sequence[int]] = None, max_rounds: int = 0, **opts):
    topics = list(topics)
    ct = _CTopics(topics)
    o = _make_opts(**opts)
    cap = np.ascontiguousarray(replica_cap, dtype=np.int32)
    if cap.shape != (topics[0].n_brokers,):
        raise ValueError("one cap per broker expected")
    dev = (C.c_int32 * len(devices))(*[int(d) for d in devices]) if devices else None
    res, bufs = _results_buffers(topics)
    lb = C.c_int64()
    _check(_ffi.load().kao_solve_capped(ct.arr, len(topics), cap.ctypes.data_as(C.POINTER(C.c_int32)), dev, len(devices) if devices else 0,
                                        C.byref(o), int(max_rounds), res, C.byref(lb)), "kao_solve_capped")
    out = _unpack(topics, res, bufs)
    return out, (None if lb.value == (1 << 63) - 1 else int(lb.value))


def rccl_selftest(devices: Sequence[int]) -> None:
    dev = (C.c_int32 * len(devices))(*[int(d) for d in devices])
    _check(_ffi.load().kao_rccl_selftest(dev, len(devices)), "kao_rccl_selftest")


def rccl_loopback_counts() -> tuple:
    out = (C.c_uint64 * 2)()
    _check(_ffi.load().kao_rccl_loopback_counts(out), "kao_rccl_loopback_counts")
    return int(out[0]), int(out[1])


def last_solve_timing() -> dict:
    out = (C.c_double * 16)()
    _check(_ffi.load().kao_last_solve_timing(out), "kao_last_solve_timing")
    return dict(session_ready=out[0], time_to_best=out[1], results_read_back=out[2], returned=out[3], launches=int(out[4]),
                delta_candidates=int(out[5]), bound_launches=int(out[6]), elite_exchanges=int(out[7]), bound_iters=int(out[8]),
                cx_calls=int(out[9]), cx_gains=int(out[10]), search_iters=int(out[11]), generations=int(out[12]), cx_further_starts=int(out[13]),
                lp_solves=int(out[14]), lp_iters=int(out[15]))


def last_solve_lp() -> dict:
    out = (C.c_double * 8)()
    _check(_ffi.load().kao_last_solve_lp(out), "kao_last_solve_lp")
    return dict(solves=int(out[0]), iterations=int(out[1]), rounded=int(out[2]), adopted=int(out[3]), fractional_partitions=int(out[4]))


def last_solve_profile() -> dict:
    out = (C.c_double * 8)()
    _check(_ffi.load().kao_last_solve_profile(out), "kao_last_solve_profile")
    return dict(ms_search=out[0], ms_eval=out[1], search_launches=int(out[2]), restarts=int(out[3]), search_bytes_algo=int(out[4]),
                delta_candidates=int(out[5]), lds_bytes_search=int(out[6]), blocks_search=int(out[7]))
```

Measured before the change: 922.2 billion.

## Split search restarts into iteration chunks chained across blocks for tail balancing

Adds a chunked search kernel that hands out tickets from a host-built schedule. Each restart's iterations are split into sequential chunks run by different blocks, which chain through progress words, carry the RNG state between chunks, and poll with sleeps until the previous chunk finishes. The goal is to fill idle CUs during the tail of a launch when there are more restart blocks than resident slots. The cost is spin-wait polling, extra global state traffic between chunks, a deadlock-guard error path, and more kernel variants.

```diff
diff --git a/include/kao.h b/include/kao.h
--- a/include/kao.h
+++ b/include/kao.h
@@ -127,6 +127,8 @@
 int kao_session_device_keys(kao_session *s, void **d_keys);
 int kao_session_stats(kao_session *s, kao_stats *out);
 int kao_session_small_launches(kao_session *s, int64_t *out);
+int kao_session_chunked_launches(kao_session *s, int64_t *out);
+int kao_search_chunk_plan(int32_t entries, int32_t resident, int32_t iters, int32_t forced, int32_t *out, int32_t cap);
 int kao_session_bound_step(kao_session *s, const int64_t *target, int32_t iters);
 int kao_session_set_prices(kao_session *s, int32_t topic, const int32_t *a, const int32_t *l, const int32_t *g);
 int kao_session_adopt_prices(kao_session *s);
diff --git a/kafka_assignment_optimizer_amd/__init__.py b/kafka_assignment_optimizer_amd/__init__.py
--- a/kafka_assignment_optimizer_amd/__init__.py
+++ b/kafka_assignment_optimizer_amd/__init__.py
@@ -1,5 +1,5 @@
 from .model import DEFAULT_WEIGHTS, NONE, Topic, assignment_to_json, topics_from_json
 from .solver import (EvalPlan, KaoError, Result, Session, canonicalize, check_infeasible, derive_bounds, device_name, dual_bound, evaluate,
-                     cycle_matrices, cycle_pair_edges, cycle_seeds, cycle_square_plan, dense_spd_test, evaluate_batch, improve_cycles, init, last_solve_lp, last_solve_profile, last_solve_timing, library_path, lp_bound, lp_repair_host, lp_round, lp_round_host, lp_sharded, lp_trace, rccl_loopback_counts, rccl_selftest, solve, solve_capped, solve_multi, upper_bound)
+                     cycle_matrices, cycle_pair_edges, cycle_seeds, cycle_square_plan, dense_spd_test, evaluate_batch, improve_cycles, init, last_solve_lp, last_solve_profile, last_solve_timing, library_path, lp_bound, lp_repair_host, lp_round, lp_round_host, lp_sharded, lp_trace, rccl_loopback_counts, rccl_selftest, search_chunk_plan, solve, solve_capped, solve_multi, upper_bound)
 
 __version__ = "0.1.0"
diff --git a/kafka_assignment_optimizer_amd/_ffi.py b/kafka_assignment_optimizer_amd/_ffi.py
--- a/kafka_assignment_optimizer_amd/_ffi.py
+++ b/kafka_assignment_optimizer_amd/_ffi.py
@@ -68,6 +68,8 @@
     "kao_session_device_keys": (C.c_int, [C.c_void_p, _P(C.c_void_p)]),
     "kao_session_stats": (C.c_int, [C.c_void_p, _P(KaoStats)]),
     "kao_session_small_launches": (C.c_int, [C.c_void_p, _P(C.c_int64)]),
+    "kao_session_chunked_launches": (C.c_int, [C.c_void_p, _P(C.c_int64)]),
+    "kao_search_chunk_plan": (C.c_int, [C.c_int32, C.c_int32, C.c_int32, C.c_int32, _P(C.c_int32), C.c_int32]),
     "kao_session_restart_state": (C.c_int, [C.c_void_p, C.c_int32, C.c_int32, _P(C.c_uint16), _P(C.c_uint16),
                                             _P(C.c_int32)]),
     "kao_session_bound_step": (C.c_int, [C.c_void_p, _P(C.c_int64), C.c_int32]),
diff --git a/kafka_assignment_optimizer_amd/csrc/kao_host.h b/kafka_assignment_optimizer_amd/csrc/kao_host.h
--- a/kafka_assignment_optimizer_amd/csrc/kao_host.h
+++ b/kafka_assignment_optimizer_amd/csrc/kao_host.h
@@ -176,6 +176,8 @@
         bool cur_in_lds = true;
         bool eval_coop = false;
         int smap_off = 0, smap_n = 0, emap_off = 0, emap_n = 0;
+        int chunk_tickets = 0, chunk_n = 0, sched_off = 0, chunk_iters = 0;
+        bool chunk_priced = false;
     };
     std::vector<LaunchGroup> groups;
     int blocks_search = 0, blocks_eval = 0;
@@ -237,6 +239,15 @@
     uint64_t search_rf3_launches = 0;
     uint64_t search_small_launches = 0;
     bool small_on = true;
+    int chunks_forced = 0;
+    bool can_chunk = false;
+    int4 *d_sched = nullptr;
+    uint32_t *d_chunk_ctl = nullptr;
+    uint32_t *d_chunk_progress = nullptr;
+    uint32_t *d_chunk_rng = nullptr;
+    uint32_t chunk_serial = 0;
+    uint64_t search_chunked_launches = 0;
+    int32_t *h_chunk_err = nullptr;
 };
 
 namespace kao {
diff --git a/kafka_assignment_optimizer_amd/csrc/kao_internal.h b/kafka_assignment_optimizer_amd/csrc/kao_internal.h
--- a/kafka_assignment_optimizer_amd/csrc/kao_internal.h
+++ b/kafka_assignment_optimizer_amd/csrc/kao_internal.h
@@ -71,6 +71,8 @@
     int32_t scan2_max;
     int32_t cur_global;
     int32_t elite;
+    int32_t chunks;
+    uint32_t serial;
 };
 
 struct SearchPools {
@@ -88,7 +90,17 @@
     const uint16_t *int_pool;
     const uint16_t *elite_assign;
     const unsigned long long *elite_key;
-};
+    uint32_t *chunk_ticket;
+    uint32_t *chunk_progress;
+    uint32_t *chunk_rng;
+    const int4 *chunk_sched;
+};
+constexpr int kChunkMax = 64;
+constexpr uint32_t kChunkPoison = 255u;
+constexpr int kChunkAuto = 4;
+constexpr int kChunkTailPct = 100;
+constexpr int kChunkMinRounds = 2;
+constexpr int kChunkMinIters = 64;
 
 struct EvalPools {
     const TopicDev *topics;
@@ -142,6 +154,9 @@
 bool search_small_cost(int lam_min, int lam_max, int obj_scale, int w_abs_max, bool priced);
 bool search_band_tabs(int rep_lo, int rep_hi, int lead_lo, int lead_hi);
 void launch_search(const SearchPools &pools, const SearchParams &prm, int n_blocks, int waves, bool global_a, bool priced, int nw, void *stream, int team = 0, int rft = 0, bool small = false);
+inline bool search_chunk_eligible(bool global_a, bool cur_global, int team) { return !global_a && !cur_global && team == 0; }
+int search_resident_blocks(int waves, bool priced, int nw, bool wide, int rft, bool small, size_t lds);
+int search_chunk_plan(int entries, int resident, int iters, int forced, int32_t *out);
 bool launch_init(const SearchPools &pools, const SearchParams &prm, int n_blocks, int per_block, bool priced, int nw, int waves, void *stream);
 void launch_eval(const EvalPools &pools, int n_blocks, int ne, void *stream);
 void launch_gather(const TopicDev *topics, int n_topics, const unsigned long long *keys, const uint16_t *best_pool,
diff --git a/kafka_assignment_optimizer_amd/csrc/kao_search.hip b/kafka_assignment_optimizer_amd/csrc/kao_search.hip
--- a/kafka_assignment_optimizer_amd/csrc/kao_search.hip
+++ b/kafka_assignment_optimizer_amd/csrc/kao_search.hip
@@ -1,10 +1,39 @@
 #include "kao_search_dev.h"
 
+#include <map>
+#include <mutex>
+#include <tuple>
+
 namespace kao {
 
-template <bool kGlobalA, bool kPriced, int NW, bool kWide, bool kTeam, bool kCurG = false, int RFT = 0, bool kSmall = false>
-__device__ __forceinline__ void search_body(unsigned char *smem, const SearchPools &pl, const SearchParams &prm) {
+struct SearchPiece {
+    uint32_t entry;
+    int32_t init, elite;
+    uint32_t first, n;
+    bool later;
+    uint32_t ticket;
+};
+__device__ __forceinline__ void chunk_pass(uint32_t ticket);
+template <class T> __device__ __forceinline__ T late_kernarg(size_t off) {
+    auto p = (const __attribute__((address_space(4))) unsigned char *)__builtin_amdgcn_kernarg_segment_ptr();
+    asm volatile("" : "+s"(p));
+    return *reinterpret_cast<const __attribute__((address_space(4))) T *>(p + off);
+}
+static_assert(sizeof(SearchPools) % alignof(SearchParams) == 0, "late_kernarg: SearchParams follows SearchPools without padding");
+constexpr size_t kArgPrm = sizeof(SearchPools);
+__device__ __forceinline__ int4 sched_record(const int4 *sched, uint32_t ticket) {
+    auto p = (const __attribute__((address_space(4))) int *)sched + 4 * (size_t)ticket;
+    return make_int4(p[0], p[1], p[2], p[3]);
+}
+__device__ __forceinline__ SearchPiece whole_launch(const SearchParams &prm) { return SearchPiece{blockIdx.x, prm.init, prm.elite, 0u, prm.iters, false, 0u}; }
+
+template <bool kGlobalA, bool kPriced, int NW, bool kWide, bool kTeam, bool kCurG = false, int RFT = 0, bool kSmall = false, bool kChunked = false>
+__device__ __forceinline__ void search_body(unsigned char *smem, const SearchPools &pl, const SearchParams &prm, const SearchPiece pc) {
+    static_assert(!kChunked || (!kGlobalA && !kTeam && !kCurG), "chunked launches: LDS-resident topics, one wavefront per restart");
     static_assert(!kTeam || kGlobalA, "teams run topics that live in global memory");
+    constexpr bool kCanChunk = kChunked;
+    const uint32_t pc_entry = kChunked ? pc.entry : blockIdx.x;
+    const int32_t pc_init = kChunked ? pc.init : prm.init, pc_elite = kChunked ? pc.elite : prm.elite;
     static_assert(!kCurG || !kGlobalA, "kCurG: the working assignment is in LDS");
     static_assert(RFT == 0 || (RFT == 3 && NW == 4 && !kGlobalA && !kTeam), "RFT = 3: LDS-resident topics of four words per partition");
     static_assert(!kSmall || (RFT == 3 && !kPriced && !kCurG), "kSmall: the unpriced RF-3 instantiation");
@@ -13,7 +42,10 @@
     const int wave = __builtin_amdgcn_readfirstlane(threadIdx.x >> 6);
     const int n_waves = kTeam ? __builtin_amdgcn_readfirstlane((int)(blockDim.x >> 6)) : 1;
     const int tid = kTeam ? (int)threadIdx.x : lane, nthr = kTeam ? (int)blockDim.x : 64;
-    const int2 bm = pl.block_map[blockIdx.x];
+    using MapPtr = std::conditional_t<kCanChunk, const __attribute__((address_space(4))) int *, const int *>;
+    int2 bm;
+    if constexpr (kChunked) bm = make_int2(((MapPtr)pl.block_map)[2 * pc_entry], ((MapPtr)pl.block_map)[2 * pc_entry + 1]);
+    else bm = pl.block_map[pc_entry];
     const TopicDev *TD = pl.topics + bm.x;
 
     TopicRegs T = topic_regs<RFT>(TD);
@@ -79,7 +111,10 @@
     __syncthreads();
 
     const int rho = bm.y + (kTeam ? 0 : wave);
-    if (rho >= TD->n_restarts) return;
+    if (rho >= TD->n_restarts) {
+        if constexpr (kCanChunk) chunk_pass(pc.ticket);
+        return;
+    }
     const int g = TD->restart_base + rho;
     unsigned char *state_packed = pl.state_pool + TD->state_off + (uint64_t)rho * T.P * (NW * 2);
     if (kGlobalA) L.A = reinterpret_cast<Part<NW> *>(pl.state_pool + TD->state_off) + (uint64_t)rho * T.P;
@@ -90,8 +125,8 @@
     const int S = prm.obj_scale;
 
     int best_obj, accepted;
-    if (prm.init) {
-        if (prm.init == 1)
+    if (pc_init) {
+        if (pc_init == 1)
         for (int p = tid; p < T.P; p += nthr) {
             Part<NW> c = CUR[p];
 #pragma unroll
@@ -103,8 +138,9 @@
     } else {
         best_obj = pl.restart_info[g * 4 + 0];
         accepted = pl.restart_info[g * 4 + 3];
+        if constexpr (kCanChunk) { best_obj = __builtin_amdgcn_readfirstlane(best_obj); accepted = __builtin_amdgcn_readfirstlane(accepted); }
         bool reseed = false;
-        if (prm.elite) {
+        if (pc_elite) {
             const unsigned long long ek = pl.elite_key[bm.x];
             const int e_obj = (int)kObjCap - (int)((ek >> 20) & 0xFFFFFFull);
             reseed = ek != ~0ull && (ek >> 44) == 0 && (int)(ek & 0xFFFFFull) != rho && best_obj < e_obj &&
@@ -132,7 +168,7 @@
     if (lane == 0) L.RT[krt - 1] = 0;
     if (kTeam) __syncthreads();
 
-    if (prm.init == 1) {
+    if (pc_init == 1) {
         constexpr bool kFillWeights = RFT != 3;
         const uint32_t *HL = pl.cur_pool + TD->hole_off;
         const FillTabs F{L.W, XR, L.K, L.RT, PR, PG, hbw ? BW : nullptr};
@@ -179,6 +215,10 @@
     if (kTeam) __syncthreads();
 
     uint32_t rng = fmix32(slo ^ fmix32(shi + (uint32_t)rho * 0x9E3779B1u + prm.launch * 0x85EBCA77u + (uint32_t)tid * 0xC2B2AE3Du));
+    if constexpr (kCanChunk) {
+        if (pc.later) rng = pl.chunk_rng[(size_t)g * 64 + lane];
+        pl.chunk_rng[(size_t)g * 64 + lane] = pc.ticket;
+    }
 
     const int plog = TD->period_log2 + (rho & 3);
     const uint32_t pmask = (1u << plog) - 1u;
@@ -193,7 +233,7 @@
     const bool x_windowed = x_rounds_full > 8;
 
     int lam_lo = prm.lam_min, lam_hi = prm.lam_max;
-    uint32_t n_iters = prm.iters, it_base = prm.launch * prm.iters;
+    uint32_t n_iters = kChunked ? pc.n : prm.iters, it_base = prm.launch * prm.iters + (kChunked ? pc.first : 0u);
     constexpr uint32_t kLpScanTwo = 1u << 29;
     uint32_t loop_pack = TD->P * TD->RF <= prm.scan2_max ? kLpScanTwo : 0u;
     if (kSmall) loop_pack |= ((uint32_t)prm.lam_min & 0xFFFu) | (((uint32_t)prm.lam_max & 0xFFFu) << 12) | (((uint32_t)plog & 31u) << 24);
@@ -974,15 +1014,68 @@
     int V2, obj2;
     T = topic_regs<RFT>(TD);
     full_cost<NW, kTeam>(T, L, CUR, RSZ, tid, nthr, V2, obj2, hbw ? BW : nullptr, TS, wave, n_waves);
-    if ((V2 != V || obj2 != obj) && tid == 0) atomicAdd(pl.drift, 1);
+    if ((V2 != V || obj2 != obj) && tid == 0) atomicAdd(kChunked ? late_kernarg<int32_t *>(offsetof(SearchPools, drift)) : pl.drift, 1);
     if (!kGlobalA)
         for (int p = lane; p < T.P; p += 64) store_packed<NW>(state_packed, p, L.A[p]);
     if (tid == 0) {
-        pl.restart_info[g * 4 + 0] = best_obj;
-        pl.restart_info[g * 4 + 1] = V2;
-        pl.restart_info[g * 4 + 2] = obj2;
-        pl.restart_info[g * 4 + 3] = accepted;
-    }
+        int32_t *info = (kChunked ? late_kernarg<int32_t *>(offsetof(SearchPools, restart_info)) : pl.restart_info) + g * 4;
+        info[0] = best_obj;
+        info[1] = V2;
+        info[2] = obj2;
+        info[3] = accepted;
+    }
+    if constexpr (kCanChunk) {
+        uint32_t *words = late_kernarg<uint32_t *>(offsetof(SearchPools, chunk_rng)) + (size_t)g * 64 + lane;
+        const uint32_t ticket = (uint32_t)__builtin_amdgcn_readfirstlane((int)*words);
+        *words = rng;
+        chunk_pass(ticket);
+    }
+}
+
+constexpr uint32_t kChunkPolls = 1u << 22;
+__device__ __forceinline__ bool chunk_take(unsigned char *smem, const SearchPools &pl, const SearchParams &prm, SearchPiece &pc, uint32_t &ticket) {
+    uint32_t *bc = reinterpret_cast<uint32_t *>(smem);
+    if (threadIdx.x == 0) {
+        const uint32_t t = atomicAdd(pl.chunk_ticket, 1u);
+        if (t + 1u == gridDim.x) __hip_atomic_store(pl.chunk_ticket, 0u, __ATOMIC_RELAXED, __HIP_MEMORY_SCOPE_AGENT);
+        const int4 sc = pl.chunk_sched[t];
+        const uint32_t c = (uint32_t)sc.y & 0xFFu, nc = (uint32_t)sc.y >> 8;
+        uint32_t ok = 1u;
+        if (c > 0u) {
+            uint32_t *word = pl.chunk_progress + sc.x;
+            const uint32_t want = prm.serial * 256u + c, gone = prm.serial * 256u + kChunkPoison;
+            for (uint32_t n = 0;; ++n) {
+                const uint32_t v = __hip_atomic_load(word, __ATOMIC_ACQUIRE, __HIP_MEMORY_SCOPE_AGENT);
+                if (v == want) break;
+                if (v == gone || n >= kChunkPolls) { ok = 0u; break; }
+                __builtin_amdgcn_s_sleep(16);
+            }
+            if (!ok) {
+                atomicAdd(pl.drift + 1, 1);
+                if (c + 1u < nc) __hip_atomic_store(word, gone, __ATOMIC_RELEASE, __HIP_MEMORY_SCOPE_AGENT);
+            }
+        }
+        bc[0] = t; bc[1] = ok;
+    }
+    __syncthreads();
+    ticket = (uint32_t)__builtin_amdgcn_readfirstlane((int)bc[0]);
+    const bool ok = __builtin_amdgcn_readfirstlane((int)bc[1]) != 0;
+    __syncthreads();
+    __builtin_amdgcn_fence(__ATOMIC_ACQUIRE, "agent");
+    const int4 sc = sched_record(pl.chunk_sched, ticket);
+    const bool later = ((uint32_t)sc.y & 0xFFu) != 0u;
+    pc = SearchPiece{(uint32_t)sc.x, later ? 0 : prm.init, later ? 0 : prm.elite, (uint32_t)sc.z, (uint32_t)sc.w, later, ticket};
+    return ok;
+}
+__device__ __forceinline__ void chunk_pass(uint32_t ticket) {
+    const int4 sc = sched_record(late_kernarg<const int4 *>(offsetof(SearchPools, chunk_sched)), ticket);
+    const uint32_t c = (uint32_t)sc.y & 0xFFu, nc = (uint32_t)sc.y >> 8;
+    if (c + 1u >= nc) return;
+    __builtin_amdgcn_fence(__ATOMIC_RELEASE, "agent");
+    __syncthreads();
+    if (threadIdx.x == 0)
+        __hip_atomic_store(late_kernarg<uint32_t *>(offsetof(SearchPools, chunk_progress)) + sc.x,
+                           late_kernarg<uint32_t>(kArgPrm + offsetof(SearchParams, serial)) * 256u + c + 1u, __ATOMIC_RELEASE, __HIP_MEMORY_SCOPE_AGENT);
 }
 
 #ifndef KAO_WPE_SMALL
@@ -995,17 +1088,28 @@
 template <bool kGlobalA, bool kPriced, int NW, bool kWide, int RFT = 0, bool kSmall = false>
 __global__ __launch_bounds__(256) __attribute__((amdgpu_waves_per_eu(search_min_waves<kGlobalA, kPriced, NW, kWide>(), 8))) void k_search(SearchPools pl, SearchParams prm) {
     extern __shared__ __attribute__((aligned(16))) unsigned char smem[];
-    search_body<kGlobalA, kPriced, NW, kWide, false, false, RFT, kSmall>(smem, pl, prm);
-}
+    search_body<kGlobalA, kPriced, NW, kWide, false, false, RFT, kSmall>(smem, pl, prm, whole_launch(prm));
+}
+template <bool kPriced, int NW, bool kWide, int RFT = 0, bool kSmall = false>
+__global__ __launch_bounds__(256) __attribute__((amdgpu_waves_per_eu(search_min_waves<false, kPriced, NW, kWide>(), 8))) void k_search_chunked(SearchPools pl, SearchParams prm) {
+    extern __shared__ __attribute__((aligned(16))) unsigned char smem[];
+    SearchPiece pc;
+    uint32_t ticket;
+    if (!chunk_take(smem, pl, prm, pc, ticket)) return;
+    search_body<false, kPriced, NW, kWide, false, false, RFT, kSmall, true>(smem, pl, prm, pc);
+}
+static_assert(std::is_same_v<decltype(&k_search_chunked<false, 4, false, 3, true>), void (*)(SearchPools, SearchParams)> &&
+              std::is_same_v<decltype(&k_search_chunked<true, 8, true>), void (*)(SearchPools, SearchParams)>,
+              "late_kernarg reads k_search_chunked's arguments by offset: (SearchPools, SearchParams) by value, in that order, nothing else");
 template <bool kPriced, int NW>
 __global__ __launch_bounds__(256) void k_search_curg(SearchPools pl, SearchParams prm) {
     extern __shared__ __attribute__((aligned(16))) unsigned char smem[];
-    search_body<false, kPriced, NW, true, false, true>(smem, pl, prm);
+    search_body<false, kPriced, NW, true, false, true>(smem, pl, prm, whole_launch(prm));
 }
 template <bool kPriced, int NW>
 __global__ __launch_bounds__(NW == 8 ? 256 : 512) void k_team(SearchPools pl, SearchParams prm) {
     extern __shared__ __attribute__((aligned(16))) unsigned char smem[];
-    search_body<true, kPriced, NW, true, true>(smem, pl, prm);
+    search_body<true, kPriced, NW, true, true>(smem, pl, prm, whole_launch(prm));
 }
 
 constexpr int kInitWaves = 16;
@@ -1186,29 +1290,59 @@
     return 8 * (int64_t)lam_max + 4 * (int64_t)obj_scale * (int64_t)w_abs_max <= (int64_t)kSmallCostMax;
 }
 
+using SearchKernel = void (*)(SearchPools, SearchParams);
+template <SearchKernel kKernel> using KernelConst = std::integral_constant<SearchKernel, kKernel>;
+template <class F>
+static void with_search_kernel(bool global_a, bool curg, int team, bool priced, int nw, bool wide, int rft, bool small, bool chunked, F f) {
+    chunked = chunked && search_chunk_eligible(global_a, curg, team);
+    if (rft == 3 && search_rf3_eligible(global_a, curg, priced, nw, team)) {
+        if (chunked) {
+            if (small) { if (wide) f(KernelConst<k_search_chunked<false, 4, true, 3, true>>{}); else f(KernelConst<k_search_chunked<false, 4, false, 3, true>>{}); }
+            else if (wide) f(KernelConst<k_search_chunked<false, 4, true, 3>>{});
+            else f(KernelConst<k_search_chunked<false, 4, false, 3>>{});
+        }
+        else if (small) { if (wide) f(KernelConst<k_search<false, false, 4, true, 3, true>>{}); else f(KernelConst<k_search<false, false, 4, false, 3, true>>{}); }
+        else if (wide) f(KernelConst<k_search<false, false, 4, true, 3>>{});
+        else f(KernelConst<k_search<false, false, 4, false, 3>>{});
+        return;
+    }
+    with_flags(priced, nw == 8, [&](auto p, auto k8) {
+        constexpr bool kPriced = decltype(p)::value;
+        constexpr int NW = decltype(k8)::value ? 8 : 4;
+        if (curg) f(KernelConst<k_search_curg<kPriced, NW>>{});
+        else if (team > 0) f(KernelConst<k_team<kPriced, NW>>{});
+        else if (global_a) f(KernelConst<k_search<true, kPriced, NW, true>>{});
+        else if (chunked) { if (wide) f(KernelConst<k_search_chunked<kPriced, NW, true>>{}); else f(KernelConst<k_search_chunked<kPriced, NW, false>>{}); }
+        else if (wide) f(KernelConst<k_search<false, kPriced, NW, true>>{});
+        else f(KernelConst<k_search<false, kPriced, NW, false>>{});
+    });
+}
+
 void launch_search(const SearchPools &pools, const SearchParams &prm, int n_blocks, int waves, bool global_a, bool priced, int nw, void *stream, int team, int rft, bool small) {
     const bool curg = prm.cur_global != 0 && !global_a, wide = prm.wide != 0;
     const size_t lds = search_lds_bytes(prm.maxP, prm.maxBx, waves, global_a, priced, nw, prm.bw != 0, prm.maxR, team, curg);
     hipStream_t st = static_cast<hipStream_t>(stream);
     const dim3 grid(n_blocks), block(64 * (team > 0 && !curg ? team : waves));
-    if (rft == 3 && search_rf3_eligible(global_a, curg, priced, nw, team)) {
-        if (small) {
-            if (wide) launch_lds<k_search<false, false, 4, true, 3, true>>(grid, block, lds, st, pools, prm);
-            else launch_lds<k_search<false, false, 4, false, 3, true>>(grid, block, lds, st, pools, prm);
-        }
-        else if (wide) launch_lds<k_search<false, false, 4, true, 3>>(grid, block, lds, st, pools, prm);
-        else launch_lds<k_search<false, false, 4, false, 3>>(grid, block, lds, st, pools, prm);
-        return;
-    }
-    with_flags(priced, nw == 8, [&](auto p, auto k8) {
-        constexpr bool kPriced = decltype(p)::value;
-        constexpr int NW = decltype(k8)::value ? 8 : 4;
-        if (curg) launch_lds<k_search_curg<kPriced, NW>>(grid, block, lds, st, pools, prm);
-        else if (team > 0) launch_lds<k_team<kPriced, NW>>(grid, block, lds, st, pools, prm);
-        else if (global_a) launch_lds<k_search<true, kPriced, NW, true>>(grid, block, lds, st, pools, prm);
-        else if (wide) launch_lds<k_search<false, kPriced, NW, true>>(grid, block, lds, st, pools, prm);
-        else launch_lds<k_search<false, kPriced, NW, false>>(grid, block, lds, st, pools, prm);
+    with_search_kernel(global_a, curg, team, priced, nw, wide, rft, small, prm.chunks != 0, [&](auto k) {
+        launch_lds<decltype(k)::value>(grid, block, lds, st, pools, prm);
     });
+}
+
+int search_resident_blocks(int waves, bool priced, int nw, bool wide, int rft, bool small, size_t lds) {
+    static std::mutex mu;
+    static std::map<std::tuple<const void *, int, size_t, int>, int> known;
+    int n = 0, dev = 0;
+    (void)hipGetDevice(&dev);
+    with_search_kernel(false, false, 0, priced, nw, wide, rft, small, true, [&](auto k) {
+        const void *fn = reinterpret_cast<const void *>(decltype(k)::value);
+        const auto key = std::make_tuple(fn, 64 * waves, lds, dev);
+        std::lock_guard<std::mutex> lock(mu);
+        const auto it = known.find(key);
+        if (it != known.end()) { n = it->second; return; }
+        if (hipOccupancyMaxActiveBlocksPerMultiprocessor(&n, fn, 64 * waves, lds) != hipSuccess) { (void)hipGetLastError(); n = 0; return; }
+        known[key] = n;
+    });
+    return n;
 }
 
 bool launch_init(const SearchPools &pools, const SearchParams &prm, int n_blocks, int per_block, bool priced, int nw, int waves, void *stream) {
diff --git a/kafka_assignment_optimizer_amd/csrc/kao_session.cpp b/kafka_assignment_optimizer_amd/csrc/kao_session.cpp
--- a/kafka_assignment_optimizer_amd/csrc/kao_session.cpp
+++ b/kafka_assignment_optimizer_amd/csrc/kao_session.cpp
@@ -5,6 +5,7 @@
 namespace {
 
 constexpr int kEvRing = 32;
+constexpr const char *kChunkGaveUp = "K-search: a chunk gave up waiting for the chunk before it";
 
 template <typename Item>
 std::vector<Item> xcd_order(const std::vector<Item> &items, const std::vector<int> &topic_of) {
@@ -92,6 +93,7 @@
     std::vector<int4> emap;
     std::vector<uint32_t> cur_pool, bw_pool, bwd_pool; std::vector<uint16_t> ext_pool, curd_pool, int_pool; std::vector<int32_t> rsz_pool;
     std::vector<uint8_t> rackof_pool;
+    std::vector<int4> sched;
     uint64_t state_bytes = 0, best_u16 = 0, win_u16 = 0, dual_i32 = 0, price_i32 = 0, wide_slices = 0;
 };
 template <typename T>
@@ -263,6 +265,81 @@
     return rc;
 }
 
+bool group_small(const kao_session &s, const kao_session::LaunchGroup &g) {
+    const bool rf3_runs = g.rf3 && search_rf3_eligible(g.global_a, g.cur_global, s.priced, g.nw, g.team);
+    return rf3_runs && s.small_on && g.band_tabs && search_small_cost(s.opts.lam_min, s.opts.lam_max, s.opts.obj_scale, g.w_abs_max, s.priced);
+}
+
+}
+
+namespace kao {
+int search_chunk_plan(int entries, int resident, int iters, int forced, int32_t *out) {
+    if (entries < 1) return 0;
+    iters = std::max(iters, 0);
+    int C = 1, K = entries;
+    if (forced >= 2) C = std::min(forced, kChunkMax);
+    else if (forced == 0 && entries >= kChunkMinRounds * (int64_t)std::max(resident, 1)) {
+        C = kChunkAuto;
+        while (C > 1 && iters / C < kChunkMinIters) C /= 2;
+        K = (int)std::min<int64_t>(entries, std::max<int64_t>(1, (int64_t)std::max(resident, 1) * kChunkTailPct / 100));
+    }
+    C = std::max(1, std::min(C, iters));
+    if (C == 1) K = entries;
+    const int whole = entries - K;
+    if (out) {
+        for (int e = 0; e < whole; ++e) { int32_t *o = out + 4 * (size_t)e; o[0] = e; o[1] = 0; o[2] = 0; o[3] = iters; }
+        for (int c = 0; c < C; ++c) {
+            const int first = c * (iters / C) + std::min(c, iters % C), n = iters / C + (c < iters % C ? 1 : 0);
+            for (int e = 0; e < K; ++e) {
+                int32_t *o = out + 4 * ((size_t)whole + (size_t)c * K + e);
+                o[0] = whole + e; o[1] = c; o[2] = first; o[3] = n;
+            }
+        }
+    }
+    return whole + C * K;
+}
+}
+
+extern "C" int kao_search_chunk_plan(int32_t entries, int32_t resident, int32_t iters, int32_t forced, int32_t *out, int32_t cap) {
+    if (entries < 1 || resident < 0 || iters < 0 || forced < 0) return fail(KAO_ERR_INVALID, "kao_search_chunk_plan: bad argument");
+    const int n = kao::search_chunk_plan(entries, resident, iters, forced, nullptr);
+    if (out && cap >= n) kao::search_chunk_plan(entries, resident, iters, forced, out);
+    return n;
+}
+
+namespace {
+
+void plan_chunks(kao_session &s, int n_cu, SessionPlan &pl) {
+    s.chunks_forced = (int)std::min<int64_t>(std::max<int64_t>(env_int("KAO_SEARCH_CHUNKS", 0), 0), kChunkMax);
+    if (s.chunks_forced == 1) return;
+    for (kao_session::LaunchGroup &g : s.groups) {
+        if (!search_chunk_eligible(g.global_a, g.cur_global, g.team)) continue;
+        if (s.chunks_forced == 0 && !(group_small(s, g) && !g.wide)) continue;
+        if (s.chunks_forced == 0 && (g.smap_n <= std::max(n_cu, 1) || s.opts.iters_per_launch < 2 * kChunkMinIters)) continue;
+        const size_t lds = search_lds_bytes(g.maxP, g.maxBx, g.waves, false, s.priced, g.nw, s.any_bw, g.maxR, 0, false);
+        const int per_cu = search_resident_blocks(g.waves, s.priced, g.nw, g.wide, g.rf3 ? 3 : 0, group_small(s, g), lds);
+        const int resident = per_cu > 0 ? per_cu * std::max(n_cu, 1) : INT32_MAX;
+        const int iters = s.opts.iters_per_launch;
+        const int tickets = search_chunk_plan(g.smap_n, resident, iters, s.chunks_forced, nullptr);
+        if (tickets <= g.smap_n) continue;
+        std::vector<int32_t> plan((size_t)tickets * 4);
+        search_chunk_plan(g.smap_n, resident, iters, s.chunks_forced, plan.data());
+        g.chunk_tickets = tickets;
+        g.chunk_n = 1;
+        for (int t = 0; t < tickets; ++t) g.chunk_n = std::max(g.chunk_n, plan[(size_t)t * 4 + 1] + 1);
+        g.chunk_iters = iters;
+        g.chunk_priced = s.priced;
+        g.sched_off = (int)pl.sched.size();
+        std::vector<int> per_entry((size_t)g.smap_n, 0);
+        for (int t = 0; t < tickets; ++t) per_entry[(size_t)plan[(size_t)t * 4]]++;
+        for (int t = 0; t < tickets; ++t) {
+            const int32_t *r = &plan[(size_t)t * 4];
+            pl.sched.push_back(make_int4(r[0], r[1] | (per_entry[(size_t)r[0]] << 8), r[2], r[3]));
+        }
+        s.can_chunk = true;
+    }
+}
+
 struct ArenaLayout {
     struct Sec { void *slot; size_t off, bytes; const void *src; };
     std::vector<Sec> secs;
@@ -295,6 +372,7 @@
     a.add(s.d_int, pl.int_pool);
     a.add(s.d_bw, pl.bw_pool);
     a.add(s.d_bwd, pl.bwd_pool);
+    if (s.can_chunk) a.add(s.d_sched, pl.sched);
     return a;
 }
 
@@ -323,6 +401,11 @@
     a.add(s.d_dual_rb, s.dual_rb_bytes);
     a.add(s.d_price, 2 * s.price_half_i32 * 4);
     a.add(s.d_keys_glob, n_topics * 8);
+    if (s.can_chunk) {
+        a.add(s.d_chunk_ctl, 256);
+        a.add(s.d_chunk_progress, (size_t)s.blocks_search * 4);
+        a.add(s.d_chunk_rng, n_restarts * 256);
+    }
     return a;
 }
 
@@ -339,6 +422,7 @@
     if (s->ev_bound1) (void)hipEventDestroy(s->ev_bound1);
     if (s->ev_search) (void)hipEventDestroy(s->ev_search);
     if (s->stream_bound) (void)hipStreamDestroy(s->stream_bound);
+    if (s->h_chunk_err) (void)hipHostFree(s->h_chunk_err);
     arena_put(s->arena_ro, s->arena_ro_bytes, s->device);
     arena_put(s->arena_rw, s->arena_rw_bytes, s->device);
     for (hipEvent_t e : s->ev) (void)hipEventDestroy(e);
@@ -361,6 +445,7 @@
     if ((rc = resolve_opts(topics, n_topics, opts_in, n_cu, total_b, s->opts))) return rc;
     SessionPlan pl;
     if ((rc = plan_session(*s, topics, n_cu, pl))) return rc;
+    plan_chunks(*s, n_cu, pl);
 
     const ArenaLayout ro = layout_ro(*s, pl), rw = layout_rw(*s, pl);
     if ((rc = arena_get(ro.total, &s->arena_ro, &s->arena_ro_bytes))) return rc;
@@ -382,6 +467,14 @@
     hipError_t e3 = hipMemsetAsync(s->d_readback, 0xFF, (size_t)n_topics * 8, s->stream);
     hipError_t e4 = hipMemsetAsync(s->d_drift, 0, 16, s->stream);
     if (e4 == hipSuccess) e4 = hipMemsetAsync(s->d_price, 0, price_b ? price_b : 4, s->stream);
+    if (s->can_chunk && e4 == hipSuccess) {
+        e4 = hipHostMalloc(reinterpret_cast<void **>(&s->h_chunk_err), 16);
+        if (e4 == hipSuccess) *s->h_chunk_err = 0; else s->h_chunk_err = nullptr;
+    }
+    if (s->can_chunk && e4 == hipSuccess) {
+        e4 = hipMemsetAsync(s->d_chunk_ctl, 0, 256, s->stream);
+        if (e4 == hipSuccess) e4 = hipMemsetAsync(s->d_chunk_progress, 0, (size_t)s->blocks_search * 4, s->stream);
+    }
     hipError_t e5 = hipStreamSynchronize(s->stream);
     if (e1 != hipSuccess || e2 != hipSuccess || e3 != hipSuccess || e4 != hipSuccess || e5 != hipSuccess) return fail(KAO_ERR_HIP, "session upload failed");
     if (s->opts.profile) {
@@ -430,8 +523,16 @@
         }
         const int rft = g.rf3 ? 3 : 0;
         const bool rf3_runs = rft && search_rf3_eligible(g.global_a, g.cur_global, s->priced, g.nw, g.team);
-        const bool small = rf3_runs && s->small_on && g.band_tabs && search_small_cost(gp.lam_min, gp.lam_max, gp.obj_scale, g.w_abs_max, s->priced);
-        launch_search(sp, gp, g.smap_n, g.waves, g.global_a, s->priced, g.nw, s->stream, g.team, rft, small);
+        const bool small = group_small(*s, g);
+        int n_blocks = g.smap_n;
+        if (g.chunk_tickets && (int)gp.iters == g.chunk_iters && s->priced == g.chunk_priced) {
+            gp.chunks = g.chunk_n; gp.serial = ++s->chunk_serial;
+            sp.chunk_ticket = s->d_chunk_ctl; sp.chunk_progress = s->d_chunk_progress + g.smap_off; sp.chunk_rng = s->d_chunk_rng;
+            sp.chunk_sched = s->d_sched + g.sched_off;
+            n_blocks = g.chunk_tickets;
+            s->search_chunked_launches++;
+        }
+        launch_search(sp, gp, n_blocks, g.waves, g.global_a, s->priced, g.nw, s->stream, g.team, rft, small);
         if (rf3_runs) s->search_rf3_launches++;
         if (small) s->search_small_launches++;
         HIP_TRY(hipGetLastError());
@@ -470,7 +571,9 @@
 int kao_session_sync(kao_session *s) {
     if (!s) return fail(KAO_ERR_INVALID, "null session");
     HIP_TRY(hipSetDevice(s->device));
+    if (s->h_chunk_err) HIP_TRY(hipMemcpyAsync(s->h_chunk_err, s->d_drift + 1, 4, hipMemcpyDeviceToHost, s->stream));
     HIP_TRY(hipStreamSynchronize(s->stream));
+    if (s->h_chunk_err && *s->h_chunk_err) return fail(KAO_ERR_HIP, kChunkGaveUp);
     if (s->opts.profile) return session_drain_events(s);
     return KAO_OK;
 }
@@ -478,6 +581,15 @@
 int kao_session_best_keys(kao_session *s, uint64_t *keys) {
     if (!s || !keys) return fail(KAO_ERR_INVALID, "null argument");
     HIP_TRY(hipSetDevice(s->device));
+    if (s->h_chunk_err) {
+        const size_t nk = (size_t)s->n_topics * 8;
+        HIP_TRY(hipMemcpyAsync(s->h_readback.data(), s->d_keys, nk + 8, hipMemcpyDeviceToHost, s->stream));
+        HIP_TRY(hipStreamSynchronize(s->stream));
+        std::memcpy(keys, s->h_readback.data(), nk);
+        std::memcpy(s->h_chunk_err, s->h_readback.data() + nk + 4, 4);
+        if (*s->h_chunk_err) return fail(KAO_ERR_HIP, kChunkGaveUp);
+        return KAO_OK;
+    }
     HIP_TRY(hipMemcpyAsync(keys, s->d_keys, (size_t)s->n_topics * 8, hipMemcpyDeviceToHost, s->stream));
     HIP_TRY(hipStreamSynchronize(s->stream));
     return KAO_OK;
@@ -541,6 +653,12 @@
     return KAO_OK;
 }
 
+int kao_session_chunked_launches(kao_session *s, int64_t *out) {
+    if (!s || !out) return fail(KAO_ERR_INVALID, "null argument");
+    *out = (int64_t)s->search_chunked_launches;
+    return KAO_OK;
+}
+
 int kao_session_small_launches(kao_session *s, int64_t *out) {
     if (!s || !out) return fail(KAO_ERR_INVALID, "null argument");
     *out = (int64_t)s->search_small_launches;
diff --git a/kafka_assignment_optimizer_amd/solver.py b/kafka_assignment_optimizer_amd/solver.py
--- a/kafka_assignment_optimizer_amd/solver.py
+++ b/kafka_assignment_optimizer_amd/solver.py
@@ -158,6 +158,16 @@
     return int(out[0]), int(out[1]), int(out[2])
 
 
+def search_chunk_plan(entries: int, resident: int, iters: int, forced: int = 0) -> np.ndarray:
+    lib = _ffi.load()
+    n = lib.kao_search_chunk_plan(int(entries), int(resident), int(iters), int(forced), None, 0)
+    _check(min(n, 0), "kao_search_chunk_plan")
+    out = np.zeros((n, 4), dtype=np.int32)
+    n2 = lib.kao_search_chunk_plan(int(entries), int(resident), int(iters), int(forced), out.ctypes.data_as(C.POINTER(C.c_int32)), n)
+    _check(min(n2, 0), "kao_search_chunk_plan")
+    return out
+
+
 def cycle_seeds(topic: Topic, assign) -> np.ndarray:
     ct = _CTopics([topic])
     a = np.ascontiguousarray(assign, dtype=np.uint16).reshape(-1)
@@ -295,6 +305,11 @@
     def small_launches(self) -> int:
         n = C.c_int64(0)
         _check(_ffi.load().kao_session_small_launches(self._h, C.byref(n)), "kao_session_small_launches")
+        return int(n.value)
+
+    def chunked_launches(self) -> int:
+        n = C.c_int64(0)
+        _check(_ffi.load().kao_session_chunked_launches(self._h, C.byref(n)), "kao_session_chunked_launches")
         return int(n.value)
 
     def restart_state(self, topic: int, restart: int) -> dict:
```

After: 963.9 billion, median of 6. 1.05x the previous value.
